# mourisl/T1K

Hardware: AMD Instinct MI355X
Metric: genotyped reads/sec (end-to-end genotyper stage, 2x150 bp HLA) (higher is better)
Workload: dtype u64

## Files before the change

### include/t1k_gpu.h

```cpp
#ifndef T1K_GPU_H
#define T1K_GPU_H

#include <stddef.h>
#include <stdint.h>

#ifdef __cplusplus
extern "C" {
#endif

typedef enum {
  T1K_OK = 0,
  T1K_ERR_ARG = -1,
  T1K_ERR_DEVICE = -2,
  T1K_ERR_CAPACITY = -3,
  T1K_ERR_IO = -4,
  T1K_ERR_STATE = -5,
  T1K_ERR_INTERNAL = -6,
  T1K_ERR_COMMITTED = -7
} t1k_status;

typedef struct t1k_ctx t1k_ctx;
typedef struct t1k_job t1k_job;
typedef struct t1k_rowset t1k_rowset;
typedef struct t1k_comm t1k_comm;

typedef struct {
  int32_t kmer_length;
  int32_t radius;
  int32_t hit_len_required;
  double ref_seq_similarity;
  int32_t relax_intron_align;
  int32_t max_assign_cnt;
  int32_t max_read_len;
  int32_t workgroups;
  int64_t group_cap;
  int64_t cand_cap;
  int64_t ovl_cap;
  int64_t row_cap;
  int32_t n_base_code;
  int32_t store_chunk_mb;
} t1k_params;

void t1k_params_default(t1k_params *p);

int t1k_ctx_create(int device, const t1k_params *params, t1k_ctx **out);
void t1k_ctx_destroy(t1k_ctx *ctx);
const char *t1k_last_error(const t1k_ctx *ctx);
int t1k_device_count(void);
int t1k_device_memory(int device, uint64_t *freeBytes, uint64_t *totalBytes);

int t1k_ref_upload(t1k_ctx *ctx, const char *seqs, const uint64_t *offsets, const uint8_t *exon, uint32_t nAlleles);

int t1k_reads_upload(t1k_ctx *ctx, const char *seqs, const uint64_t *offsets, const uint32_t *weights, uint32_t nReadEnds);
int t1k_reads_upload_begin(t1k_ctx *ctx, uint32_t nReadEnds, uint64_t textBytes, int maxReadLen);
int t1k_reads_upload_piece(t1k_ctx *ctx, int what, const void *src, uint64_t byteOffset, uint64_t bytes, int slot);
int t1k_reads_upload_wait(t1k_ctx *ctx, int slot);
int t1k_reads_upload_end(t1k_ctx *ctx);

int t1k_reads_dedupe(t1k_ctx *ctx, uint32_t *distinctOf, uint32_t *nDistinct);

typedef struct {
  int32_t seq_idx, read_start, read_end, seq_start, seq_end, strand;
  int32_t match_cnt, left_clip, right_clip, relaxed_match_cnt;
  double similarity;
} t1k_overlap;

int t1k_assign_batch(t1k_ctx *ctx);
int t1k_assign_range(t1k_ctx *ctx, uint64_t first, uint32_t count);
int t1k_overlaps_download(t1k_ctx *ctx, uint32_t *counts, t1k_overlap *ovl, uint64_t cap, uint64_t *total);

int t1k_overlaps_upload(t1k_ctx *ctx, const uint32_t *counts, const t1k_overlap *ovl);
void t1k_pair_limits(uint32_t out[4]);
uint32_t t1k_pair_direct_cap(void);

typedef struct {
  int32_t allele_idx, start, end;
  float weight, qual, adjust_weight;
} t1k_row_entry;

int t1k_pair_batch(t1k_ctx *ctx, const uint32_t *end1, const uint32_t *end2, const uint8_t *hasN, uint32_t nFragments);
int t1k_rows_download(t1k_ctx *ctx, uint32_t *rowCounts, uint8_t *fragAssigned, t1k_row_entry *rows, uint64_t cap, uint64_t *total);

typedef struct {
  int32_t allele, start, end;
  float weight, adjust_weight;
} t1k_group_entry;
int t1k_rowset_create(t1k_ctx *owner, uint64_t nFragments, const uint8_t *whitelist , t1k_rowset **out);
int t1k_rowset_trim(t1k_rowset *rs, uint64_t n_fragments);
void t1k_rowset_destroy(t1k_rowset *rs);
int t1k_rowset_set_raw(t1k_rowset *rs, int raw);
int t1k_rowset_device_bytes(t1k_rowset *rs, uint64_t *bytes, uint64_t *rowEntries);
const char *t1k_rowset_last_error(const t1k_rowset *rs);
int t1k_pair_into(t1k_ctx *ctx, t1k_rowset *rs, const uint32_t *end1, const uint32_t *end2, const uint8_t *hasN, uint32_t nFragments, uint64_t fragBase);
int t1k_rowset_coalesce(t1k_rowset *rs, uint64_t *nGroups, uint64_t *nEntries, uint64_t *assignedFragments);
int t1k_rowset_coalesce_sized(t1k_rowset *rs, uint64_t *nGroups, uint64_t *nEntries, uint64_t *assignedFragments, void (*sized)(uint64_t nGroups, uint64_t nEntries, void *user), void *user);
int t1k_rowset_groups_download(t1k_rowset *rs, uint64_t *groupPtr, t1k_group_entry *entries, uint32_t *firstFragment);
int t1k_rowset_assigned_download(t1k_rowset *rs, uint8_t *fragAssigned);
int t1k_rowset_assigned_range(t1k_rowset *rs, uint64_t first, uint64_t count, uint8_t *fragAssigned);
int t1k_rowset_rows_download(t1k_rowset *rs, uint64_t first, uint32_t count, uint32_t *rowCounts, t1k_row_entry *rows, uint64_t cap, uint64_t *total);
void t1k_coalesce_limits(uint32_t out[3]);

typedef struct t1k_comm_group t1k_comm_group;
int t1k_comm_unique_id(void *id128);
t1k_comm_group *t1k_comm_group_create(int nRanks);
void t1k_comm_group_destroy(t1k_comm_group *g);
int t1k_comm_init(t1k_ctx *ctx, int nRanks, int rank, const void *id128, t1k_comm_group *group, int transport , t1k_comm **out);
int t1k_comm_bind(t1k_comm *c, t1k_ctx *ctx);
int t1k_comm_abort(t1k_comm *c);
void t1k_comm_destroy(t1k_comm *c);
const char *t1k_comm_last_error(const t1k_comm *c);
int t1k_comm_rank(const t1k_comm *c);
int t1k_comm_size(const t1k_comm *c);
int t1k_comm_is_rccl(const t1k_comm *c);
int t1k_comm_allreduce(t1k_comm *c, void *dev, uint64_t count, int kind);
int t1k_comm_allgather_u64(t1k_comm *c, const uint64_t *mine, uint32_t k, uint64_t *all);
int t1k_comm_alltoallv(t1k_comm *c, const void *sendbuf, const uint64_t *sendOff, void *recvbuf, const uint64_t *recvOff);
int t1k_comm_allgatherv(t1k_comm *c, const void *mine, const uint64_t *bytes, const uint64_t *displ, void *out);
int t1k_comm_allgatherv_host(t1k_comm *c, void *host, const uint64_t *bytes, const uint64_t *displ, uint64_t total);
int t1k_rowset_exchange(t1k_rowset *rs, t1k_comm *comm, uint64_t fragBase);
int t1k_rowset_groups_gather(t1k_rowset *rs, t1k_comm *comm, uint64_t *totalGroups, uint64_t *totalEntries, uint64_t *totalAssigned);
int t1k_rowset_groups_download_all(t1k_rowset *rs, uint32_t *sizes, t1k_group_entry *entries, uint32_t *firstFragment);
int t1k_em_shard(t1k_ctx *ctx, uint32_t rowBegin, uint32_t rowEnd, t1k_comm *comm);

int t1k_coverage_get(t1k_ctx *ctx, int32_t *out, uint64_t cap);
int t1k_coverage_reset(t1k_ctx *ctx);
int t1k_missing_coverage(t1k_ctx *ctx, int32_t *missing);
typedef struct t1k_readset t1k_readset;
int t1k_ctx_set_coverage_mode(t1k_ctx *ctx, int deferred);
int t1k_readset_detach(t1k_ctx *reader, t1k_readset **out);
int t1k_readset_take_store(t1k_readset *rs, t1k_ctx *pipe, int slot);
uint64_t t1k_readset_bytes(const t1k_readset *rs);
uint32_t t1k_readset_size(const t1k_readset *rs);
const char *t1k_readset_last_error(const t1k_readset *rs);
void t1k_readset_destroy(t1k_readset *rs);
int t1k_coverage_selected(t1k_ctx *ctx, t1k_readset *rs, const uint8_t *selected, uint64_t *nRecords);
typedef struct t1k_xwin t1k_xwin;
int t1k_xwin_create(t1k_ctx *owner, uint64_t maxReadEnds, uint32_t maxWindows, t1k_xwin **out);
void t1k_xwin_destroy(t1k_xwin *x);
const char *t1k_xwin_last_error(const t1k_xwin *x);
int t1k_xwin_link(t1k_xwin *x, t1k_ctx *reader, uint32_t window, uint32_t *nExternal);
int t1k_xwin_resolve(t1k_xwin *x, t1k_ctx *ctx, uint32_t window);

int t1k_ref_share(t1k_ctx *dst, const t1k_ctx *src);
uint64_t t1k_pool_release(void);
void *t1k_pinned_alloc(uint64_t bytes);
void t1k_pinned_free(void *p);
int t1k_reads_share(t1k_ctx *dst, const t1k_ctx *src);
int t1k_reads_attach(t1k_ctx *dst, const t1k_ctx *src, int storeSlot, int resetStore);
int t1k_coverage_absorb(t1k_ctx *dst, t1k_ctx *src);

int t1k_extract_batch(t1k_ctx *ctx, uint32_t endsPerFragment, uint8_t *good, uint64_t *stats);

int t1k_align_count_batch(t1k_ctx *ctx, const char *text, const uint32_t *tOff, const char *pat, const uint32_t *pOff, const uint32_t *len, uint32_t nJobs,
                          int32_t *nMatch);
int t1k_gap_count_batch(t1k_ctx *ctx, const char *text, const uint32_t *tOff, const uint32_t *tLen, const char *pat, const uint32_t *pOff,
                        const uint32_t *pLen, uint32_t nJobs, int32_t *nMatch);
int t1k_align_batch(t1k_ctx *ctx, const char *text, const uint32_t *tOff, const uint32_t *tLen, const char *pat, const uint32_t *pOff,
                    const uint32_t *pLen, uint32_t nJobs, int32_t *score, int32_t *nMatch, int32_t *nMismatch, int32_t *nIndel, int8_t *ops,
                    const uint32_t *opsOff, uint32_t *nOps);

typedef void (*t1k_allreduce_fn)(void *dev_f64, uint64_t n, void *user);
int t1k_em_setup(t1k_ctx *ctx, const uint64_t *rowPtr, const uint32_t *ecIdx, const double *count, const int32_t *ecLen, uint32_t nGroups,
                 uint32_t nEc, t1k_allreduce_fn allreduce, void *user);
int t1k_em_update(t1k_ctx *ctx, const double *x0, double *x1, double *ecReadCount, double *diff);
void t1k_em_limits(uint32_t out[2]);

int t1k_barcode_em(t1k_ctx *ctx, uint32_t nBarcodes, const uint64_t *bcAllelePtr, const uint32_t *bcAllele, const uint64_t *bcGroupPtr,
                   const double *groupCount, const uint64_t *groupEntryPtr, const uint32_t *entryLocal, const double *rho, uint32_t nAlleles,
                   double alpha, double tol, int32_t maxIter, double *nOut, int32_t *itersOut, double *kernelMs);

typedef struct {
  uint64_t distinct;
  uint64_t keys;
  uint64_t corrected;
  uint64_t split;
  uint64_t no_umi;
  double kernel_ms;
} t1k_umi_stats;
int t1k_umi_collapse(t1k_ctx *ctx, uint32_t nFrag, const uint32_t *fragRow, const uint64_t *fragUmi, const uint64_t *listPtr, const uint32_t *listAllele,
                     uint32_t nRows, const uint32_t *alleleGene, uint32_t nAlleles, uint32_t nGenes, int32_t mismatch, uint32_t *fragMol, uint32_t *nMol,
                     uint32_t *molRow, uint32_t *molFrags, uint64_t *molListPtr, uint32_t *molList, double *frac, int32_t *uniq, t1k_umi_stats *stats);

typedef struct {
  uint32_t allele, seq_start;
  uint64_t read_at, ops_at;
  uint32_t n_ops, w_all, w_uniq, reserved;
} t1k_pileup_aln;
int t1k_pileup_begin(t1k_ctx *ctx, uint32_t nAlleles, const uint64_t *alleleOff );
int t1k_pileup_add(t1k_ctx *ctx, const t1k_pileup_aln *aln, uint32_t n, const char *text, uint64_t textBytes, const int8_t *ops, uint64_t opsBytes,
                   double *kernelMs);
int t1k_pileup_get(t1k_ctx *ctx, int32_t *counts );
int t1k_pileup_end(t1k_ctx *ctx);

int t1k_sitepile_begin(t1k_ctx *ctx, uint32_t nAlleles, const uint64_t *alleleOff , uint64_t nSites, const uint32_t *siteAllele, const uint32_t *sitePos,
                       uint64_t nBarcodes);
int t1k_sitepile_add(t1k_ctx *ctx, const t1k_pileup_aln *aln, uint32_t n, const uint64_t *bookPtr , const uint32_t *book, const char *text, uint64_t textBytes,
                     const int8_t *ops, uint64_t opsBytes, double *kernelMs);
int t1k_sitepile_get(t1k_ctx *ctx, uint64_t *keys, int32_t *counts, uint64_t cap, uint64_t *nRuns);
int t1k_sitepile_stats(t1k_ctx *ctx, uint64_t *keysEmitted, uint64_t *folds, double *foldMs);
int t1k_sitepile_end(t1k_ctx *ctx);

int t1k_phase_begin(t1k_ctx *ctx, uint32_t nAlleles, const uint64_t *alleleOff , uint64_t nSites, const uint32_t *siteAllele, const uint32_t *sitePos);
int t1k_phase_add(t1k_ctx *ctx, const t1k_pileup_aln *aln, uint32_t n, uint32_t nBook, const uint32_t *bookRec , const uint8_t *bookUniq ,
                  const char *text, uint64_t textBytes, const int8_t *ops, uint64_t opsBytes, double *kernelMs);
int t1k_phase_get(t1k_ctx *ctx, uint64_t *keys, int32_t *counts, uint64_t cap, uint64_t *nRuns);
int t1k_phase_stats(t1k_ctx *ctx, uint64_t *observations, uint64_t *bookings, uint64_t *keysEmitted, uint64_t *discordant, uint64_t *folds, double *foldMs);
int t1k_phase_end(t1k_ctx *ctx);

typedef struct { uint32_t read_len, clip_front, strand; } t1k_support_rec;
typedef struct { uint32_t flags, t_start, t_end; } t1k_support_book;
int t1k_support_begin(t1k_ctx *ctx, uint32_t nAlleles, const uint64_t *alleleOff , uint64_t nSites, const uint32_t *siteAllele, const uint32_t *sitePos);
int t1k_support_add(t1k_ctx *ctx, const t1k_pileup_aln *aln, uint32_t n, const t1k_support_rec *rec , const uint64_t *bookPtr ,
                    const t1k_support_book *book, const char *text, uint64_t textBytes, const int8_t *ops, uint64_t opsBytes, double *kernelMs);
int t1k_support_get(t1k_ctx *ctx, uint64_t *keys, int32_t *counts, uint64_t cap, uint64_t *nRuns);
int t1k_support_stats(t1k_ctx *ctx, uint64_t *keysEmitted, uint64_t *folds, double *foldMs);
int t1k_support_end(t1k_ctx *ctx);

int t1k_indel_begin(t1k_ctx *ctx, uint32_t nAlleles, const uint64_t *alleleOff , const char *alleleText );
int t1k_indel_add(t1k_ctx *ctx, const t1k_pileup_aln *aln, uint32_t n, const uint8_t *strand , const uint64_t *bookPtr , const uint8_t *bookUniq,
                  const char *text, uint64_t textBytes, const int8_t *ops, uint64_t opsBytes, double *kernelMs);
int t1k_indel_get(t1k_ctx *ctx, uint64_t *keys, int32_t *counts, uint64_t cap, uint64_t *nRuns);
int t1k_indel_stats(t1k_ctx *ctx, uint64_t *events, uint64_t *shifted, uint64_t *edgeDelBooked, uint64_t *edgeInsBooked, uint64_t *keysEmitted, uint64_t *folds, double *foldMs);
int t1k_indel_end(t1k_ctx *ctx);

int t1k_cigar_batch(t1k_ctx *ctx, const t1k_pileup_aln *aln, uint32_t n, const uint32_t *clip ,
                    const int8_t *ops, uint64_t opsBytes, uint32_t nAlleles, const uint64_t *alleleOff , const char *alleleText ,
                    uint64_t *cigarPtr , char *cigar, uint64_t cigarCap, uint64_t *mdPtr , char *md, uint64_t mdCap,
                    uint32_t *nm , uint32_t *refSpan , double *kernelMs );

typedef struct {
  uint64_t read_ends, lookups, postings, hits, groups, candidates, extended, near_best, dp_calls, rows, batches;
  double ms_seed, ms_chain, ms_extend, ms_select, ms_fullalign, ms_pair, ms_em, ms_total;
  uint64_t read_ends_total, pair_overlaps, dp_cells;
  double ms_load, ms_device, ms_coalesce, ms_write;
} t1k_stats;
int t1k_stats_get(t1k_ctx *ctx, t1k_stats *out);

enum { T1K_ROUTE_GENERAL_LANE = 0,
       T1K_ROUTE_WAVE_SMALL = 1,
       T1K_ROUTE_WAVE_LARGE = 2,
       T1K_ROUTE_BIG_BY_SIZE = 3,
       T1K_ROUTE_BIG_BY_SCRATCH = 4,
       T1K_ROUTE_KINDS = 5 };
typedef struct {
  uint64_t ranges, ranges_nw5, ranges_nw10, ranges_xlong;
  uint64_t groups, fast, slow, jobs, retry, finish, general, wave, genjobs, big, eq, band, wide, extjobs, extretry;
} t1k_route_totals;
typedef struct {
  uint32_t read_end, allele, n;
  uint8_t strand;
  uint8_t near_done, simple;
  uint8_t route;
  uint8_t nw, xlong, reserved[2];
} t1k_route_rec;
int t1k_route_report_enable(t1k_ctx *ctx, int on);
int t1k_route_report_get(t1k_ctx *ctx, t1k_route_totals *totals , t1k_route_rec *recs , uint64_t cap, uint64_t *nRecs);

double t1k_alloc_ms(t1k_ctx *ctx, uint64_t *bytes);
uint64_t t1k_ctx_mem_report(t1k_ctx *ctx, const char *tag, int print);

int t1k_genotyper_main(int argc, char **argv);
int t1k_extractor_main(int argc, char **argv);
int t1k_bam_extractor_main(int argc, char **argv);
int t1k_analyzer_main(int argc, char **argv);

typedef struct {
  t1k_params dev;
  double filter_frac, filter_cov, cross_gene_rate, squarem_min_alpha;
  int32_t allele_digit_units;
  char allele_delimiter;
  int32_t threads;
  int32_t device;
  int32_t output_read_assignment;
  int32_t batch_fragments;
} t1k_job_params;
void t1k_job_params_default(t1k_job_params *p);

int t1k_job_create(const t1k_job_params *p, const char *refFasta, t1k_job **out);
void t1k_job_destroy(t1k_job *job);
const char *t1k_job_last_error(const t1k_job *job);
int t1k_job_load_reads(t1k_job *job, const char *file1, const char *file2, const char *barcodeFile);
int t1k_job_load_reads_multi(t1k_job *job, const char *const *files1, uint32_t n1, const char *const *files2, uint32_t n2, const char *barcodeFile);
typedef struct t1k_reads t1k_reads;
int t1k_reads_open(const char *const *files1, uint32_t n1, const char *const *files2, uint32_t n2, const char *barcodeFile, int threads, t1k_reads **out);
int t1k_reads_open_stream(const char *const *files1, uint32_t n1, const char *const *files2, uint32_t n2, const char *barcodeFile, int threads, t1k_reads **out);
const char *t1k_reads_last_error(const t1k_reads *reads);
int t1k_reads_fragments(const t1k_reads *reads, uint64_t *nFragments);
void t1k_reads_close(t1k_reads *reads);
int t1k_job_attach_reads(t1k_job *job, t1k_reads *reads);
int t1k_job_set_reads(t1k_job *job, const char *seq1, const uint64_t *off1, const char *seq2, const uint64_t *off2, uint32_t nFragments);
int t1k_job_run(t1k_job *job);
int t1k_job_set_output_prefix(t1k_job *job, const char *prefix);
int t1k_job_write_outputs(t1k_job *job, const char *prefix);
int t1k_job_genotype_text(t1k_job *job, char *buf, uint64_t cap, uint64_t *needed);
int t1k_job_counts(t1k_job *job, uint64_t *fragments, uint64_t *assignedFragments, uint64_t *groups, uint64_t *ecs, int32_t *emIterations);
int t1k_job_stats(t1k_job *job, t1k_stats *out);
t1k_ctx *t1k_job_ctx(t1k_job *job);
int t1k_job_set_shard(t1k_job *job, int rank, int nRanks, t1k_comm *comm);
int t1k_job_share_reads(t1k_job *dst, t1k_job *src);
int t1k_job_run_local(t1k_job *job);
int t1k_job_finish(t1k_job *job);
int t1k_job_groups_serialize(t1k_job *job, void *buf, uint64_t cap, uint64_t *needed);
int t1k_job_groups_merge(t1k_job *job, const void *const *bufs, const uint64_t *lens, uint32_t n);
int t1k_job_coalesce_rows(t1k_job *job, const t1k_row_entry *rows, const uint32_t *rowCounts, const uint32_t *fragments, uint32_t nFragments);
int t1k_coverage_device(t1k_ctx *ctx, void **devPtr, uint64_t *count);

typedef struct {
  int32_t allele_idx;
  int32_t has_mate_pair, o1_from_r2;
  t1k_overlap o1, o2;
  uint64_t ops1, ops2;
  uint32_t n_ops1, n_ops2;
} t1k_frag_assignment;
int t1k_fragment_details(const t1k_overlap *l1, uint32_t n1, const t1k_overlap *l2, uint32_t n2, int paired, const int32_t *alleles, uint32_t nAlleles,
                         t1k_frag_assignment *out);
typedef struct {
  int32_t allele_idx, ref_pos, exon_pos;
// ... 19 lines not shown
```

### t1k_amd/capi.py

```python
import ctypes as C
import gzip
import os

import numpy as np

_HERE = os.path.dirname(os.path.abspath(__file__))


def lib_path():
    return os.environ.get("T1K_GPU_LIB") or os.path.join(_HERE, "lib", "libt1k_gpu.so")


class T1kError(RuntimeError):
    pass


class Params(C.Structure):
    _fields_ = [("kmer_length", C.c_int32), ("radius", C.c_int32), ("hit_len_required", C.c_int32),
                ("ref_seq_similarity", C.c_double), ("relax_intron_align", C.c_int32), ("max_assign_cnt", C.c_int32),
                ("max_read_len", C.c_int32), ("workgroups", C.c_int32), ("group_cap", C.c_int64),
                ("cand_cap", C.c_int64), ("ovl_cap", C.c_int64), ("row_cap", C.c_int64), ("n_base_code", C.c_int32), ("store_chunk_mb", C.c_int32)]


class JobParams(C.Structure):
    _fields_ = [("dev", Params), ("filter_frac", C.c_double), ("filter_cov", C.c_double),
                ("cross_gene_rate", C.c_double), ("squarem_min_alpha", C.c_double), ("allele_digit_units", C.c_int32),
                ("allele_delimiter", C.c_char), ("threads", C.c_int32), ("device", C.c_int32),
                ("output_read_assignment", C.c_int32), ("batch_fragments", C.c_int32)]


class Stats(C.Structure):
    _fields_ = [(n, C.c_uint64) for n in ("read_ends", "lookups", "postings", "hits", "groups", "candidates", "extended",
                                          "near_best", "dp_calls", "rows", "batches")] + \
               [(n, C.c_double) for n in ("ms_seed", "ms_chain", "ms_extend", "ms_select", "ms_fullalign", "ms_pair", "ms_em", "ms_total")] + \
               [(n, C.c_uint64) for n in ("read_ends_total", "pair_overlaps", "dp_cells")] + \
               [(n, C.c_double) for n in ("ms_load", "ms_device", "ms_coalesce", "ms_write")]

    def as_dict(self):
        return {n: getattr(self, n) for n, _ in self._fields_}


class UmiStats(C.Structure):
    _fields_ = [(n, C.c_uint64) for n in ("distinct", "keys", "corrected", "split", "no_umi")] + [("kernel_ms", C.c_double)]


OVERLAP_DTYPE = np.dtype([("seq_idx", "<i4"), ("read_start", "<i4"), ("read_end", "<i4"), ("seq_start", "<i4"),
                          ("seq_end", "<i4"), ("strand", "<i4"), ("match_cnt", "<i4"), ("left_clip", "<i4"),
                          ("right_clip", "<i4"), ("relaxed_match_cnt", "<i4"), ("similarity", "<f8")])
ROW_DTYPE = np.dtype([("allele_idx", "<i4"), ("start", "<i4"), ("end", "<i4"), ("weight", "<f4"), ("qual", "<f4"),
                      ("adjust_weight", "<f4")])
GROUP_DTYPE = np.dtype([("allele", "<i4"), ("start", "<i4"), ("end", "<i4"), ("weight", "<f4"), ("adjust_weight", "<f4")])
assert OVERLAP_DTYPE.itemsize == 48 and ROW_DTYPE.itemsize == 24 and GROUP_DTYPE.itemsize == 20
FRAG_ASG_DTYPE = np.dtype([("allele_idx", "<i4"), ("has_mate_pair", "<i4"), ("o1_from_r2", "<i4"), ("_pad", "<i4"), ("o1", OVERLAP_DTYPE), ("o2", OVERLAP_DTYPE),
                           ("ops1", "<u8"), ("ops2", "<u8"), ("n_ops1", "<u4"), ("n_ops2", "<u4")])
VARIANT_DTYPE = np.dtype([("allele_idx", "<i4"), ("ref_pos", "<i4"), ("exon_pos", "<i4"), ("ref", "S1"), ("var", "S1"), ("_pad", "S2"), ("qual", "<i4"), ("group", "<i4"),
                          ("output_group", "<i4"), ("_pad2", "<i4"), ("var_support", "<f8"), ("all_support", "<f8"), ("var_uniq_support", "<f8")])
assert FRAG_ASG_DTYPE.itemsize == 136 and VARIANT_DTYPE.itemsize == 56

PILEUP_ALN_DTYPE = np.dtype([("allele", "<u4"), ("seq_start", "<u4"), ("read_at", "<u8"), ("ops_at", "<u8"), ("n_ops", "<u4"), ("w_all", "<u4"), ("w_uniq", "<u4"),
                             ("reserved", "<u4")])
PHASE_NO_MATE = 0xFFFFFFFF
PHASE_STATES = ("A", "C", "G", "T", "N", "-")
PILEUP_COUNTERS = ("A", "C", "G", "T", "N", "del", "ins", "A_uniq", "C_uniq", "G_uniq", "T_uniq", "N_uniq", "del_uniq", "ins_uniq")
assert PILEUP_ALN_DTYPE.itemsize == 40
SUPPORT_REC_DTYPE = np.dtype([("read_len", "<u4"), ("clip_front", "<u4"), ("strand", "<u4")])
SUPPORT_BOOK_DTYPE = np.dtype([("flags", "<u4"), ("t_start", "<u4"), ("t_end", "<u4")])
SUPPORT_STATES = ("A", "C", "G", "T", "N", "-", "+")
SUPPORT_FAMILY_B = 1 << 57
assert SUPPORT_REC_DTYPE.itemsize == 12 and SUPPORT_BOOK_DTYPE.itemsize == 12
ROUTE_TOTALS = ("ranges", "ranges_nw5", "ranges_nw10", "ranges_xlong", "groups", "fast", "slow", "jobs", "retry", "finish", "general", "wave", "genjobs", "big",
                "eq", "band", "wide", "extjobs", "extretry")
ROUTE_REC_DTYPE = np.dtype([("read_end", "<u4"), ("allele", "<u4"), ("n", "<u4"), ("strand", "u1"), ("near_done", "u1"), ("simple", "u1"), ("route", "u1"),
                            ("nw", "u1"), ("xlong", "u1"), ("reserved", "u1", (2,))])
ROUTE_NAMES = ("general_lane", "wave_small", "wave_large", "big_by_size", "big_by_scratch")
assert ROUTE_REC_DTYPE.itemsize == 20
CIGAR_FILL = 0xAB

ALLREDUCE_FN = C.CFUNCTYPE(None, C.c_void_p, C.c_uint64, C.c_void_p)

_lib = None


def lib():
    global _lib
    if _lib is not None:
        return _lib
    p = lib_path()
    if not os.path.exists(p):
        raise T1kError("%s not found: run `python -c 'import __graft_entry__ as g; g.build()'` first" % p)
    L = C.CDLL(p)
    vp, u64p, u32p, u8p, i32p = C.c_void_p, C.POINTER(C.c_uint64), C.POINTER(C.c_uint32), C.POINTER(C.c_uint8), C.POINTER(C.c_int32)
    L.t1k_params_default.argtypes = [C.POINTER(Params)]
    L.t1k_ctx_create.argtypes = [C.c_int, C.POINTER(Params), C.POINTER(vp)]
    L.t1k_ctx_destroy.argtypes = [vp]
    L.t1k_last_error.argtypes = [vp]
    L.t1k_last_error.restype = C.c_char_p
    L.t1k_device_count.restype = C.c_int
    L.t1k_ref_upload.argtypes = [vp, C.c_char_p, vp, vp, C.c_uint32]
    L.t1k_reads_upload.argtypes = [vp, C.c_char_p, vp, vp, C.c_uint32]
    L.t1k_assign_batch.argtypes = [vp]
    L.t1k_assign_range.argtypes = [vp, C.c_uint64, C.c_uint32]
    L.t1k_overlaps_download.argtypes = [vp, vp, vp, C.c_uint64, u64p]
    L.t1k_pair_batch.argtypes = [vp, vp, vp, vp, C.c_uint32]
    L.t1k_rows_download.argtypes = [vp, vp, vp, vp, C.c_uint64, u64p]
    L.t1k_coverage_get.argtypes = [vp, vp, C.c_uint64]
    L.t1k_coverage_reset.argtypes = [vp]
    L.t1k_missing_coverage.argtypes = [vp, vp]
    L.t1k_coverage_absorb.argtypes = [vp, vp]
    L.t1k_align_batch.argtypes = [vp, C.c_char_p, vp, vp, C.c_char_p, vp, vp, C.c_uint32, vp, vp, vp, vp, vp, vp, vp]
    L.t1k_align_count_batch.argtypes = [vp, C.c_char_p, vp, C.c_char_p, vp, vp, C.c_uint32, vp]
    L.t1k_gap_count_batch.argtypes = [vp, C.c_char_p, vp, vp, C.c_char_p, vp, vp, C.c_uint32, vp]
    L.t1k_em_setup.argtypes = [vp, vp, vp, vp, vp, C.c_uint32, C.c_uint32, ALLREDUCE_FN, vp]
    L.t1k_em_update.argtypes = [vp, vp, vp, vp, vp]
    L.t1k_em_shard.argtypes = [vp, C.c_uint32, C.c_uint32, vp]
    L.t1k_em_limits.argtypes = [vp]
    L.t1k_em_limits.restype = None
    L.t1k_barcode_em.argtypes = [vp, C.c_uint32, vp, vp, vp, vp, vp, vp, vp, C.c_uint32, C.c_double, C.c_double, C.c_int32, vp, vp, C.POINTER(C.c_double)]
    L.t1k_umi_collapse.argtypes = [vp, C.c_uint32, vp, vp, vp, vp, C.c_uint32, vp, C.c_uint32, C.c_uint32, C.c_int32, vp, C.POINTER(C.c_uint32), vp, vp, vp, vp, vp, vp,
                                   C.POINTER(UmiStats)]
# ... 4 lines not shown
    L.t1k_sitepile_begin.argtypes = [vp, C.c_uint32, vp, C.c_uint64, vp, vp, C.c_uint64]
    L.t1k_sitepile_add.argtypes = [vp, vp, C.c_uint32, vp, vp, vp, C.c_uint64, vp, C.c_uint64, C.POINTER(C.c_double)]
    L.t1k_sitepile_get.argtypes = [vp, vp, vp, C.c_uint64, u64p]
    L.t1k_sitepile_stats.argtypes = [vp, u64p, u64p, C.POINTER(C.c_double)]
    L.t1k_sitepile_end.argtypes = [vp]
    L.t1k_support_begin.argtypes = [vp, C.c_uint32, vp, C.c_uint64, vp, vp]
    L.t1k_support_add.argtypes = [vp, vp, C.c_uint32, vp, vp, vp, vp, C.c_uint64, vp, C.c_uint64, C.POINTER(C.c_double)]
    L.t1k_support_get.argtypes = [vp, vp, vp, C.c_uint64, u64p]
    L.t1k_support_stats.argtypes = [vp, u64p, u64p, C.POINTER(C.c_double)]
    L.t1k_support_end.argtypes = [vp]
    L.t1k_indel_begin.argtypes = [vp, C.c_uint32, vp, vp]
    L.t1k_indel_add.argtypes = [vp, vp, C.c_uint32, vp, vp, vp, vp, C.c_uint64, vp, C.c_uint64, C.POINTER(C.c_double)]
    L.t1k_indel_get.argtypes = [vp, vp, vp, C.c_uint64, u64p]
    L.t1k_indel_stats.argtypes = [vp, u64p, u64p, u64p, u64p, u64p, u64p, C.POINTER(C.c_double)]
    L.t1k_indel_end.argtypes = [vp]
    L.t1k_phase_begin.argtypes = [vp, C.c_uint32, vp, C.c_uint64, vp, vp]
    L.t1k_phase_add.argtypes = [vp, vp, C.c_uint32, C.c_uint32, vp, vp, vp, C.c_uint64, vp, C.c_uint64, C.POINTER(C.c_double)]
    L.t1k_phase_get.argtypes = [vp, vp, vp, C.c_uint64, u64p]
    L.t1k_phase_stats.argtypes = [vp, u64p, u64p, u64p, u64p, u64p, C.POINTER(C.c_double)]
    L.t1k_phase_end.argtypes = [vp]
    L.t1k_cigar_batch.argtypes = [vp, vp, C.c_uint32, vp, vp, C.c_uint64, C.c_uint32, vp, vp, vp, vp, C.c_uint64, vp, vp, C.c_uint64, vp, vp, C.POINTER(C.c_double)]
    L.t1k_extract_batch.argtypes = [vp, C.c_uint32, vp, vp]
    L.t1k_extractor_main.argtypes = [C.c_int, C.POINTER(C.c_char_p)]
    L.t1k_stats_get.argtypes = [vp, C.POINTER(Stats)]
    L.t1k_route_report_enable.argtypes = [vp, C.c_int]
    L.t1k_route_report_get.argtypes = [vp, vp, vp, C.c_uint64, u64p]
    L.t1k_genotyper_main.argtypes = [C.c_int, C.POINTER(C.c_char_p)]
    L.t1k_job_params_default.argtypes = [C.POINTER(JobParams)]
    L.t1k_job_create.argtypes = [C.POINTER(JobParams), C.c_char_p, C.POINTER(vp)]
    L.t1k_job_destroy.argtypes = [vp]
    L.t1k_job_last_error.argtypes = [vp]
    L.t1k_job_last_error.restype = C.c_char_p
    L.t1k_job_load_reads.argtypes = [vp, C.c_char_p, C.c_char_p, C.c_char_p]
    L.t1k_job_set_reads.argtypes = [vp, C.c_char_p, vp, C.c_char_p, vp, C.c_uint32]
    L.t1k_job_run.argtypes = [vp]
    L.t1k_job_write_outputs.argtypes = [vp, C.c_char_p]
    L.t1k_pool_release.restype = C.c_uint64
    L.t1k_pool_release.argtypes = []
    L.t1k_job_load_reads_multi.argtypes = [vp, C.POINTER(C.c_char_p), C.c_uint32, C.POINTER(C.c_char_p), C.c_uint32, C.c_char_p]
    L.t1k_reads_open.argtypes = [C.POINTER(C.c_char_p), C.c_uint32, C.POINTER(C.c_char_p), C.c_uint32, C.c_char_p, C.c_int, C.POINTER(vp)]
    L.t1k_reads_open_stream.argtypes = [C.POINTER(C.c_char_p), C.c_uint32, C.POINTER(C.c_char_p), C.c_uint32, C.c_char_p, C.c_int, C.POINTER(vp)]
    L.t1k_reads_last_error.argtypes = [vp]
    L.t1k_reads_last_error.restype = C.c_char_p
    L.t1k_reads_fragments.argtypes = [vp, u64p]
    L.t1k_reads_close.argtypes = [vp]
    L.t1k_reads_close.restype = None
    L.t1k_job_attach_reads.argtypes = [vp, vp]
    L.t1k_job_genotype_text.argtypes = [vp, C.c_char_p, C.c_uint64, u64p]
    L.t1k_job_counts.argtypes = [vp, u64p, u64p, u64p, u64p, i32p]
    L.t1k_job_stats.argtypes = [vp, C.POINTER(Stats)]
    L.t1k_job_ctx.argtypes = [vp]
    L.t1k_job_ctx.restype = vp
    L.t1k_job_run_local.argtypes = [vp]
    L.t1k_job_finish.argtypes = [vp]
    L.t1k_job_groups_serialize.argtypes = [vp, vp, C.c_uint64, u64p]
    L.t1k_reads_dedupe.argtypes = [vp, vp, u32p]
    L.t1k_job_groups_merge.argtypes = [vp, vp, vp, C.c_uint32]
    L.t1k_job_coalesce_rows.argtypes = [vp, vp, vp, vp, C.c_uint32]
    L.t1k_variants_call.argtypes = [vp, vp, C.c_int32, C.c_uint32, vp, vp, vp, vp, vp, vp, vp, C.POINTER(vp)]
    L.t1k_fragment_details.argtypes = [vp, C.c_uint32, vp, C.c_uint32, C.c_int, vp, C.c_uint32, vp]
    L.t1k_variants_count.argtypes = [vp]
    L.t1k_variants_count.restype = C.c_uint32
    L.t1k_variants_get.argtypes = [vp, vp]
    L.t1k_variants_vcf.argtypes = [vp, vp, C.c_uint64, u64p]
    L.t1k_variants_adjust.argtypes = [vp, vp, C.c_uint32, vp, C.c_char_p, C.c_uint32, C.c_char_p, C.c_uint32, vp]
    L.t1k_variants_destroy.argtypes = [vp]
    L.t1k_job_set_shard.argtypes = [vp, C.c_int, C.c_int, vp]
    L.t1k_job_share_reads.argtypes = [vp, vp]
    L.t1k_job_ctx.restype = vp
    L.t1k_job_ctx.argtypes = [vp]
    L.t1k_comm_unique_id.argtypes = [vp]
    L.t1k_comm_init.argtypes = [vp, C.c_int, C.c_int, vp, vp, C.c_int, C.POINTER(vp)]
    L.t1k_comm_bind.argtypes = [vp, vp]
    L.t1k_comm_destroy.argtypes = [vp]
    L.t1k_comm_last_error.restype = C.c_char_p
    L.t1k_comm_last_error.argtypes = [vp]
    L.t1k_comm_is_rccl.argtypes = [vp]
    L.t1k_comm_group_create.restype = vp
    L.t1k_comm_group_create.argtypes = [C.c_int]
    L.t1k_comm_group_destroy.argtypes = [vp]
    L.t1k_coverage_device.argtypes = [vp, C.POINTER(vp), u64p]
    L.t1k_device_memory.argtypes = [C.c_int, u64p, u64p]
    L.t1k_ctx_set_coverage_mode.argtypes = [vp, C.c_int]
    L.t1k_readset_detach.argtypes = [vp, C.POINTER(vp)]
    L.t1k_readset_take_store.argtypes = [vp, vp, C.c_int]
    L.t1k_readset_bytes.argtypes = [vp]
    L.t1k_readset_bytes.restype = C.c_uint64
    L.t1k_readset_size.argtypes = [vp]
    L.t1k_readset_size.restype = C.c_uint32
    L.t1k_readset_destroy.argtypes = [vp]
    L.t1k_coverage_selected.argtypes = [vp, vp, vp, u64p]
    L.t1k_overlaps_upload.argtypes = [vp, vp, vp]
    L.t1k_pair_limits.argtypes = [vp]
    L.t1k_pair_limits.restype = None
    L.t1k_pair_direct_cap.argtypes = []
    L.t1k_pair_direct_cap.restype = C.c_uint32
    L.t1k_rowset_create.argtypes = [vp, C.c_uint64, vp, C.POINTER(vp)]
    L.t1k_rowset_destroy.argtypes = [vp]
    L.t1k_rowset_destroy.restype = None
    L.t1k_rowset_set_raw.argtypes = [vp, C.c_int]
    L.t1k_rowset_last_error.argtypes = [vp]
    L.t1k_rowset_last_error.restype = C.c_char_p
    L.t1k_pair_into.argtypes = [vp, vp, vp, vp, vp, C.c_uint32, C.c_uint64]
    L.t1k_rowset_rows_download.argtypes = [vp, C.c_uint64, C.c_uint32, vp, vp, C.c_uint64, u64p]
    L.t1k_rowset_assigned_range.argtypes = [vp, C.c_uint64, C.c_uint64, vp]
    L.t1k_rowset_coalesce.argtypes = [vp, u64p, u64p, u64p]
    L.t1k_rowset_groups_download.argtypes = [vp, vp, vp, vp]
    L.t1k_rowset_device_bytes.argtypes = [vp, u64p, u64p]
    L.t1k_coalesce_limits.argtypes = [vp]
    L.t1k_coalesce_limits.restype = None
    L.t1k_rowset_exchange.argtypes = [vp, vp, C.c_uint64]
    L.t1k_rowset_groups_gather.argtypes = [vp, vp, u64p, u64p, u64p]
    L.t1k_rowset_groups_download_all.argtypes = [vp, vp, vp, vp]
    L.t1k_comm_abort.argtypes = [vp]
    L.t1k_ref_share.argtypes = [vp, vp]
    _lib = L
    return L


def _ptr(a):
    return a.ctypes.data_as(C.c_void_p) if a is not None else None


def _concat(seqs):
    offs = np.zeros(len(seqs) + 1, dtype=np.uint64)
    if len(seqs):
        offs[1:] = np.cumsum([len(s) for s in seqs], dtype=np.uint64)
    blob = "".join(seqs).encode("ascii")
    return blob, offs


class Context:

    def __init__(self, device=0, **kw):
        L = lib()
        p = Params()
        L.t1k_params_default(C.byref(p))
        for k, v in kw.items():
            setattr(p, k, v)
        self.params = p
        h = C.c_void_p()
        rc = L.t1k_ctx_create(device, C.byref(p), C.byref(h))
        if rc != 0:
            raise T1kError("t1k_ctx_create failed (%d): no usable GPU / bad parameters" % rc)
        self.h = h
        self.n_read_ends = 0
        self.allele_len = None

    def _check(self, rc, what):
        if rc != 0:
            raise T1kError("%s failed (%d): %s" % (what, rc, lib().t1k_last_error(self.h).decode()))

    def close(self):
        if self.h:
            lib().t1k_ctx_destroy(self.h)
            self.h = None

    def __del__(self):
        try:
            self.close()
        except Exception:
            pass

    def ref_upload(self, seqs, exon_masks=None):
        blob, offs = _concat(seqs)
        ex = None
        if exon_masks is not None:
            ex = np.concatenate([np.asarray(m, dtype=np.uint8) for m in exon_masks]) if len(seqs) else np.zeros(0, np.uint8)
        self.allele_len = np.array([len(s) for s in seqs], dtype=np.int64)
        self._check(lib().t1k_ref_upload(self.h, blob, _ptr(offs), _ptr(ex), len(seqs)), "t1k_ref_upload")

    def ref_share(self, src):
        self.allele_len = src.allele_len
        self._check(lib().t1k_ref_share(self.h, src.h), "t1k_ref_share")

    def reads_upload(self, seqs, weights=None):
        blob, offs = _concat(seqs)
        w = None if weights is None else np.asarray(weights, dtype=np.uint32)
        self.n_read_ends = len(seqs)
        self._check(lib().t1k_reads_upload(self.h, blob, _ptr(offs), _ptr(w), len(seqs)), "t1k_reads_upload")

    def reads_dedupe(self):
        out = np.zeros(self.n_read_ends, dtype=np.uint32)
        nd = C.c_uint32()
        self._check(lib().t1k_reads_dedupe(self.h, _ptr(out), C.byref(nd)), "t1k_reads_dedupe")
        self.n_uploaded, self.n_read_ends = self.n_read_ends, nd.value
        return out

    def assign(self):
        self._check(lib().t1k_assign_batch(self.h), "t1k_assign_batch")

    def extract(self, ends_per_fragment=1):
        good = np.zeros(self.n_read_ends // ends_per_fragment, dtype=np.uint8)
        st = np.zeros(8, dtype=np.uint64)
        self._check(lib().t1k_extract_batch(self.h, ends_per_fragment, _ptr(good), _ptr(st)), "t1k_extract_batch")
        return good, dict(zip(("read_ends", "lookups", "postings", "read_ends_with_hits", "read_ends_chained", "screen_ns", "main_ns", "big_shape"), (int(x) for x in st)))

    def overlaps(self):
        n = self.n_read_ends
        counts = np.zeros(n, dtype=np.uint32)
        tot = C.c_uint64()
        self._check(lib().t1k_overlaps_download(self.h, _ptr(counts), None, 0, C.byref(tot)), "t1k_overlaps_download")
        out = np.zeros(tot.value, dtype=OVERLAP_DTYPE)
        self._check(lib().t1k_overlaps_download(self.h, _ptr(counts), _ptr(out), tot.value, C.byref(tot)), "t1k_overlaps_download")
        return counts, out

    def overlaps_upload(self, counts, ovl):
        c = np.ascontiguousarray(counts, dtype=np.uint32)
        o = np.ascontiguousarray(ovl, dtype=OVERLAP_DTYPE)
        assert len(c) == self.n_read_ends and int(c.sum()) == len(o)
        self._check(lib().t1k_overlaps_upload(self.h, _ptr(c), _ptr(o)), "t1k_overlaps_upload")

    def pair(self, end1, end2, has_n):
        e1 = np.asarray(end1, dtype=np.uint32)
        e2 = None if end2 is None else np.asarray(end2, dtype=np.uint32)
        hn = np.asarray(has_n, dtype=np.uint8)
        self.n_fragments = len(e1)
        self._check(lib().t1k_pair_batch(self.h, _ptr(e1), _ptr(e2), _ptr(hn), len(e1)), "t1k_pair_batch")

    def rows(self):
        n = self.n_fragments
        counts = np.zeros(n, dtype=np.uint32)
        assigned = np.zeros(n, dtype=np.uint8)
        tot = C.c_uint64()
        self._check(lib().t1k_rows_download(self.h, _ptr(counts), _ptr(assigned), None, 0, C.byref(tot)), "t1k_rows_download")
        out = np.zeros(tot.value, dtype=ROW_DTYPE)
        self._check(lib().t1k_rows_download(self.h, _ptr(counts), _ptr(assigned), _ptr(out), tot.value, C.byref(tot)), "t1k_rows_download")
        return counts, assigned, out

    def coverage(self):
        tot = int(self.allele_len.sum())
        out = np.zeros(tot, dtype=np.int32)
        self._check(lib().t1k_coverage_get(self.h, _ptr(out), tot), "t1k_coverage_get")
        return out

    def set_coverage_mode(self, deferred):
        self._check(lib().t1k_ctx_set_coverage_mode(self.h, 1 if deferred else 0), "t1k_ctx_set_coverage_mode")

    def detach_readset(self, slot=0):
        h = C.c_void_p()
        self._check(lib().t1k_readset_detach(self.h, C.byref(h)), "t1k_readset_detach")
        rs = Readset(h)
        self._check(lib().t1k_readset_take_store(rs.h, self.h, slot), "t1k_readset_take_store")
        return rs

    def coverage_selected(self, readset, selected):
        sel = np.ascontiguousarray(selected, dtype=np.uint8)
        n = C.c_uint64()
        self._check(lib().t1k_coverage_selected(self.h, readset.h, _ptr(sel), C.byref(n)), "t1k_coverage_selected")
        return n.value

    def coverage_reset(self):
        self._check(lib().t1k_coverage_reset(self.h), "t1k_coverage_reset")

    def missing_coverage(self):
        out = np.zeros(len(self.allele_len), dtype=np.int32)
        self._check(lib().t1k_missing_coverage(self.h, _ptr(out)), "t1k_missing_coverage")
        return out

    def stats(self):
        s = Stats()
        lib().t1k_stats_get(self.h, C.byref(s))
        return s.as_dict()

    def route_report_enable(self, on=True):
        self._check(lib().t1k_route_report_enable(self.h, 1 if on else 0), "t1k_route_report_enable")

    def route_report(self):
        n = C.c_uint64()
        self._check(lib().t1k_route_report_get(self.h, None, None, 0, C.byref(n)), "t1k_route_report_get")
        tot = np.zeros(len(ROUTE_TOTALS), np.uint64)
        recs = np.zeros(n.value, ROUTE_REC_DTYPE)
        self._check(lib().t1k_route_report_get(self.h, _ptr(tot), _ptr(recs), n.value, C.byref(n)), "t1k_route_report_get")
        return dict(zip(ROUTE_TOTALS, (int(x) for x in tot))), recs

    def align_batch(self, texts, pats, want_ops=True):
        n = len(texts)
        tb, toff = _concat(texts)
        pb, poff = _concat(pats)
        tlen = np.array([len(t) for t in texts], dtype=np.uint32)
        plen = np.array([len(p) for p in pats], dtype=np.uint32)
        toff32, poff32 = toff[:-1].astype(np.uint32), poff[:-1].astype(np.uint32)
        score = np.zeros(n, np.int32); nm = np.zeros(n, np.int32); nx = np.zeros(n, np.int32); ni = np.zeros(n, np.int32)
        ops_off = np.zeros(n, np.uint32)
        if n:
            ops_off[1:] = np.cumsum((tlen + plen + 2)[:-1], dtype=np.uint64).astype(np.uint32)
        ops = np.zeros(int((tlen + plen + 2).sum()) + 8, np.int8)
        nops = np.zeros(n, np.uint32)
        self._check(lib().t1k_align_batch(self.h, tb, _ptr(toff32), _ptr(tlen), pb, _ptr(poff32), _ptr(plen), n, _ptr(score), _ptr(nm),
                                          _ptr(nx), _ptr(ni), _ptr(ops) if want_ops else None, _ptr(ops_off), _ptr(nops)), "t1k_align_batch")
        op_list = [ops[ops_off[i]:ops_off[i] + nops[i]].copy() for i in range(n)] if want_ops else None
        return score, nm, nx, ni, op_list

    def align_count_batch(self, texts, pats):
        n = len(texts)
        tb, toff = _concat(texts)
        pb, poff = _concat(pats)
        ln = np.array([len(t) for t in texts], dtype=np.uint32)
        out = np.zeros(n, np.int32)
        self._check(lib().t1k_align_count_batch(self.h, tb, _ptr(toff[:-1].astype(np.uint32)), pb, _ptr(poff[:-1].astype(np.uint32)), _ptr(ln), n,
                                                _ptr(out)), "t1k_align_count_batch")
        return out

    def gap_count_batch(self, texts, pats, lead=""):
        n = len(texts)
        tb, toff = _concat([lead] + list(texts))
        pb, poff = _concat(pats)
        tlen = np.array([len(t) for t in texts], dtype=np.uint32)
        plen = np.array([len(p) for p in pats], dtype=np.uint32)
        out = np.zeros(n, np.int32)
        self._check(lib().t1k_gap_count_batch(self.h, tb, _ptr(toff[1:-1].astype(np.uint32)), _ptr(tlen), pb, _ptr(poff[:-1].astype(np.uint32)), _ptr(plen), n,
                                              _ptr(out)), "t1k_gap_count_batch")
        return out

    def em_setup(self, row_ptr, ec_idx, count, ec_len, allreduce=None, raw=False):
        self._em_keep = (np.ascontiguousarray(row_ptr, np.uint64), np.ascontiguousarray(ec_idx, np.uint32), np.ascontiguousarray(count, np.float64),
                         np.ascontiguousarray(ec_len, np.int32))
        rp, ei, ct, el = self._em_keep
        assert len(rp) == len(ct) + 1 and int(rp[-1]) == len(ei)
        self._em_cb = ALLREDUCE_FN(allreduce) if allreduce else C.cast(None, ALLREDUCE_FN)
        self._em_nec = len(el)
# ... 860 lines not shown
```

### t1k_amd/csrc/host/job.cpp

```cpp
#include "job_internal.h"

extern "C" {


void t1k_job_params_default(t1k_job_params *p) {
  memset(p, 0, sizeof(*p));
  t1k_params_default(&p->dev);
  p->filter_frac = 0.15;
  p->filter_cov = 1.0;
  p->cross_gene_rate = 0.04;
  p->squarem_min_alpha = 0;
  p->allele_digit_units = -1;
  p->allele_delimiter = 0;
  p->threads = 1;
  p->device = 0;
  p->output_read_assignment = 0;
  p->batch_fragments = 0;
}

int t1k_job_create(const t1k_job_params *p, const char *refFasta, t1k_job **out) { return jobCreate(p, refFasta, nullptr, out); }

}
namespace t1k {
int jobCreate(const t1k_job_params *p, const char *refFasta, const std::set<std::string> *selected, t1k_job **out) {
// ... 411 lines not shown
  const bool traceTasks = getenv("T1K_DEBUG_TASKS") != nullptr;
  auto prepare = [&] {
    struct Raw {
      void *p = nullptr; size_t cap = 0; bool pinned = false;
      ~Raw() { drop(); }
      void drop() { if (pinned) t1k_pinned_free(p); else free(p); p = nullptr; cap = 0; }
      void *need(size_t bytes) {
        if (bytes <= cap) return p;
        drop();
        static const bool noPin = getenv("T1K_NO_PINNED_TEXT") != nullptr;
        p = noPin ? nullptr : t1k_pinned_alloc(bytes);
        pinned = p != nullptr;
        if (!p) p = malloc(bytes);
        cap = p ? bytes : 0;
        return p;
      }
    } offs[2], stage;
    auto windowSize = [&](uint32_t w) -> uint64_t {
      uint64_t size = firstWindow;
      if (w > 0) {
        const Window &prev = win[w - 1];
        const double tp = prev.msPrep / std::max<double>(1, prev.f1 - prev.f0);
        double tg = 0;
        for (uint32_t v = w; v-- > 0;)
          if (win[v].done && win[v].tDone > win[v].tReady) { tg = (win[v].tDone - win[v].tReady) / std::max<double>(1, win[v].f1 - win[v].f0); break; }
        uint64_t waiting = 0;
        for (uint32_t v = sh.oldest; v < w; ++v) waiting += win[v].f1 - win[v].f0;
        double factor = fixedGrowth > 0 ? fixedGrowth : (tg > 0 && tp > 0 ? 0.85 * tg / tp : 6.0);
        factor = std::min(16.0, std::max(1.0, factor));
        size = (uint64_t)(factor * (double)std::max<uint64_t>(waiting, firstWindow / 2));
        size = std::min<uint64_t>(windowFrags, std::max<uint64_t>(size, firstWindow));
      }
      return size;
    };
    uint64_t fNext = 0;
    uint64_t have = F;
    bool ended = !gzStream;
    for (uint32_t w = 0; gzStream ? true : fNext < F; ++w) {
      if (gzStream) {
        const uint64_t least = fNext + (w == 0 ? firstWindow : std::max<uint32_t>(16384u, firstWindow / 4));
        for (;;) {
          const int st = in.streamState();
          have = in.streamAvail();
          if (st < 0) { std::string e; (void)job->in->streamFinish(e); fail(T1K_ERR_IO, e.empty() ? "cannot read the .gz input" : e); return; }
          if (st == 1) { have = in.streamAvail(); ended = true; break; }
          bool idle;
          uint64_t want;
          { std::lock_guard<std::mutex> g(sh.m); if (sh.err != T1K_OK) return; idle = sh.oldest >= sh.created; want = fNext + windowSize(w); }
          if (w + 8 >= maxWindows) { std::this_thread::sleep_for(std::chrono::milliseconds(1)); continue; }
          if (have >= want || (have >= least && idle)) break;
          std::this_thread::sleep_for(std::chrono::microseconds(300));
        }
        if (ended && fNext >= have) {
          std::lock_guard<std::mutex> g(sh.m);
          sh.allCreated = true;
          sh.cv.notify_all();
          break;
        }
      }
      {
        std::unique_lock<std::mutex> lk(sh.m);
        sh.cv.wait(lk, [&] { return sh.err != T1K_OK || w < 2 || win[w - 2].done; });
        if (sh.err != T1K_OK) return;
        if (gzStream && !ended) { const int st = in.streamState(); have = in.streamAvail(); if (st == 1) { have = in.streamAvail(); ended = true; } }
        const uint64_t size = windowSize(w);
        Window N;
        N.f0 = (uint32_t)fNext; N.f1 = (uint32_t)std::min<uint64_t>(have, fNext + size);
        if (ended && (have - N.f1 < size / 4 || w + 1 >= maxWindows)) N.f1 = (uint32_t)have;
        N.slot = (int)(w & 1);
        N.touched.assign(P, 0);
        if (!eagerFromNowOn) {
          const double perFrag = archivedFrags ? 1.25 * (double)archivedNeed / (double)archivedFrags : 0.0;
          const uint64_t slack = (uint64_t)P * (uint64_t)std::max(1, job->prm.dev.store_chunk_mb) << 20;
          auto estimate = [&](const Window &X) { return archivedFrags ? (uint64_t)(perFrag * (double)(X.f1 - X.f0)) + slack : 0ull; };
          uint64_t open = 0;
          for (uint32_t v = sh.oldest; v < w; ++v)
            if (win[v].deferred && !win[v].done) open += estimate(win[v]);
          bool fits = archivedBytes + open + estimate(N) <= archiveBudget;
          static const char *testHeadroom = getenv("T1K_TEST_ARCHIVE_HEADROOM_MB");
          if (fits && sh.pairedFrags >= (testHeadroom ? 1u : 65536u) && !getenv("T1K_ARCHIVE_GB")) {
            uint64_t freeNow = 0, totalNow = 0, rowsNow = 0, entriesNow = 0;
            if (t1k_device_memory(job->prm.device, &freeNow, &totalNow) == T1K_OK && t1k_rowset_device_bytes(job->rows, &rowsNow, &entriesNow) == T1K_OK && totalNow) {
              if (testHeadroom) { const uint64_t used = totalNow - std::min(freeNow, totalNow); totalNow = used + ((uint64_t)atoll(testHeadroom) << 20); freeNow = totalNow - used; }
              const double projectedRows = (double)entriesNow / (double)sh.pairedFrags * (double)F * sizeof(t1k_row_entry) * 1.1 + 32.0 * (double)F + std::min(4e9, 0.015 * (double)totalNow);
              const uint64_t usedNow = totalNow - std::min(freeNow, totalNow);
              const uint64_t other = usedNow > archivedBytes + rowsNow ? usedNow - archivedBytes - rowsNow : 0;
              const double coalesceWork = 48.0 * (double)F + std::min(8e9, 0.03 * (double)totalNow);
              const double transient = perFrag * (double)std::min<uint64_t>(windowFrags, F - N.f1);
              static const double reserve = [] { const char *e = getenv("T1K_ARCHIVE_RESERVE_GB"); return e ? atof(e) * 1073741824.0 : -1.0; }();
              const double keepFree = reserve >= 0 ? reserve : std::max(8e9, 0.04 * (double)totalNow);
              fits = (double)other + (double)(archivedBytes + open + estimate(N)) + std::max(projectedRows, (double)rowsNow) + coalesceWork + transient + keepFree <= (double)totalNow;
              if (getenv("T1K_DEBUG_ARCHIVE"))
                fprintf(stderr, "[t1k job] window %u (%u fragments): %llu row entries in the chunks, %llu fragments paired, stats.rows %llu, rows %.1f GB, kept %.1f + open %.1f + this %.1f GB, other %.1f GB, transient %.1f GB -> %s\n",
                        w, N.f1 - N.f0, (unsigned long long)entriesNow, (unsigned long long)sh.pairedFrags, (unsigned long long)job->stats.rows, rowsNow / 1e9, archivedBytes / 1e9, open / 1e9,
                        estimate(N) / 1e9, other / 1e9, transient / 1e9, fits ? "kept" : "not kept");
              if (!fits && getenv("T1K_DEBUG_PHASES"))
                fprintf(stderr, "[t1k job] window %u: read sets are not kept from here on: %.1f GB of rows projected for the job (%.1f GB so far), %.1f GB kept, %.1f GB other, device %.1f GB\n",
                        w, projectedRows / 1e9, rowsNow / 1e9, archivedBytes / 1e9, other / 1e9, totalNow / 1e9);
            }
          }
          if (fits) N.deferred = true;
          else eagerFromNowOn = true;
        }
        fNext = N.f1;
        win.push_back(std::move(N));
        sh.created = w + 1;
        if (ended && fNext >= have) sh.allCreated = true;
      }
      Window &W = win[w];
      const double t0 = nowMs();
      const uint32_t nf = W.f1 - W.f0, ne = nf * per;
      uint64_t *off = (uint64_t *)offs[W.slot].need(((size_t)ne + 1) * 8);
      if (!off) { fail(T1K_ERR_DEVICE, "window preparation: out of host memory"); return; }
      W.hasN.resize(nf);
      std::vector<uint64_t> pieceBytes(T + 2, 0);
      std::vector<uint32_t> pieceMax(T + 1, 0);
      auto setAside = [&](uint32_t r) {
        if (!dropLong) return false;
        for (uint32_t m = 0; m < per; ++m) if (in.side[m].seqL[r] > lenLimit) return true;
        return false;
      };
      parallelRanges(nf, T, [&](int t, size_t b, size_t e) {
        uint64_t run = 0, aside = 0;
        uint32_t mx = 0;
        for (size_t i = b; i < e; ++i) {
          const uint32_t r = in.frag[fBeg - inBase + W.f0 + i];
          const bool skip = setAside(r);
          aside += skip ? 1 : 0;
          for (uint32_t m = 0; m < per; ++m) {
            const uint32_t len = skip ? 0 : in.side[m].seqL[r];
            off[i * per + m] = run; run += len; mx = std::max(mx, len);
          }
        }
        pieceBytes[t + 1] = run; pieceMax[t] = mx;
        if (aside) droppedFragments += aside;
      });
      for (int t = 0; t < T; ++t) pieceBytes[t + 1] += pieceBytes[t];
      const uint64_t total = pieceBytes[T];
      uint32_t maxLen = 0;
      for (int t = 0; t < T; ++t) maxLen = std::max(maxLen, pieceMax[t]);
      if (gzStream && maxLen > lenLimit) {
        fail(T1K_ERR_ARG, "a read of " + std::to_string(maxLen) + " bases is longer than this build handles (" + std::to_string(job->prm.dev.max_read_len) +
                              "); T1K_LONG_READS=drop sets the fragments of such reads aside instead of stopping");
        return;
      }
      parallelRanges(nf, T, [&](int t, size_t b, size_t e) {
        const uint64_t carry = pieceBytes[t];
        for (size_t i = b; i < e; ++i)
          for (uint32_t m = 0; m < per; ++m) off[i * per + m] += carry;
      });
      off[ne] = total;
      static const size_t slotBytes = [] { const char *e = getenv("T1K_STAGE_MB"); return (size_t)std::max(1, e ? atoi(e) : 96) << 20; }();
      const int nSlots = 3;
      char *ring = (char *)stage.need(nSlots * slotBytes);
      if (!ring) { fail(T1K_ERR_DEVICE, "window preparation: out of host memory"); return; }
      t1k_ctx *rd = job->reader[W.slot];
      int r = t1k_reads_upload_begin(rd, ne, total, (int)maxLen);
      if (r == T1K_OK) r = t1k_reads_upload_piece(rd, 1, off, 0, ((uint64_t)ne + 1) * 8, 3);
      double msGather = 0;
      uint32_t nPieces = 0;
      for (size_t i0 = 0; i0 < nf && r == T1K_OK; ++nPieces) {
        const uint64_t base = off[i0 * per];
        size_t lo = i0 + 1, hi = nf;
        while (lo < hi) {
          const size_t mid = lo + (hi - lo + 1) / 2;
          if (off[mid * per] - base <= slotBytes) lo = mid; else hi = mid - 1;
        }
// ... 48 lines not shown
          }
        });
        for (uint32_t q = 1; q < W.nPair; ++q) W.pairNeed[q] = std::max(W.pairNeed[q], W.pairNeed[q - 1]);
        for (uint32_t q = 0; q < W.nPair; ++q) W.pairNeed[q] = std::min(W.pairNeed[q], W.nAssign);
      }
      if (traceTasks) fprintf(stderr, "[t1k task] prep window %u: %.1f .. %.1f ms (text %.1f ms, upload %.1f, resize %.1f, dedupe %.1f, pairing needs %.1f)\n", w, t0 - tStart, nowMs() - tStart, tText - t0, tUp - tText, tRes - tUp, tDd - tRes, nowMs() - tDd);
      {
        std::lock_guard<std::mutex> g(sh.m);
        job->distinctReadEnds += W.nDistinct - W.nExternal;
        job->stats.read_ends -= W.nExternal;
        msPrep += nowMs() - t0;
        W.msPrep = nowMs() - t0; W.tReady = nowMs();
        W.ready = true;
      }
      sh.cv.notify_all();
    }
  };
  std::function<int(t1k_ctx *, Window &, uint32_t, uint32_t, std::string &)> assignRange = [&](t1k_ctx *ctx, Window &Wn, uint32_t b0, uint32_t nb, std::string &msg) -> int {
    int r = t1k_assign_range(ctx, b0, nb);
    if (r == T1K_ERR_CAPACITY && nb > 64) {
      if ((r = assignRange(ctx, Wn, b0, nb / 2, msg)) != T1K_OK) return r;
      return assignRange(ctx, Wn, b0 + nb / 2, nb - nb / 2, msg);
    }
    if (r != T1K_OK) { msg = t1k_last_error(ctx); return r; }
    t1k_stats st;
    t1k_stats_get(ctx, &st);
    if (traceTasks) fprintf(stderr, "[t1k task]   range of %u read-ends at %u: kernels by HIP events: seed %.1f chain %.1f extend %.1f select %.1f align+truncate %.1f ms\n", nb, b0, st.ms_seed, st.ms_chain, st.ms_extend, st.ms_select, st.ms_fullalign);
    std::lock_guard<std::mutex> g(sh.m);
    Wn.ovlRecords += st.extended;
    job->stats.read_ends += st.read_ends; job->stats.lookups += st.lookups; job->stats.postings += st.postings; job->stats.hits += st.hits;
    job->stats.groups += st.groups; job->stats.candidates += st.candidates; job->stats.extended += st.extended; job->stats.near_best += st.near_best;
    job->stats.dp_calls += st.dp_calls; job->stats.ms_chain += st.ms_chain; job->stats.ms_extend += st.ms_extend; job->stats.ms_select += st.ms_select;
    job->stats.ms_fullalign += st.ms_fullalign; job->stats.ms_seed += st.ms_seed; job->stats.batches += 1; job->stats.dp_cells += st.dp_cells;
    return T1K_OK;
  };
  auto worker = [&](int pi) {
    t1k_ctx *ctx = pipes[pi];
    int attached = -1;
    std::vector<uint32_t> e1, e2;
    for (;;) {
      uint32_t w = 0, item = 0;
      int kind = -1;
      {
        std::unique_lock<std::mutex> lk(sh.m);
        for (;;) {
          if (sh.err != T1K_OK) return;
          if (sh.allCreated && sh.oldest >= sh.created) return;
          for (w = sh.oldest; w < sh.created && w < sh.oldest + 2 && win[w].ready && kind < 0; ++w) {
            Window &W = win[w];
            if (W.nextPair < W.nPair && W.assignPrefix >= W.pairNeed[W.nextPair]) {
              if (W.linked) { kind = 1; item = W.nextPair++; }
              else if (!W.linking) {
                bool srcDone = true;
                for (uint32_t v = sh.oldest; v < w; ++v) srcDone = srcDone && win[v].ready && win[v].doneAssign == win[v].nAssign;
                if (srcDone) { kind = 2; W.linking = true; }
              }
            }
            if (kind < 0 && W.nextAssign < W.nAssign) { kind = 0; item = W.nextAssign++; }
            if (kind >= 0) break;
          }
          if (kind >= 0) break;
          sh.cv.wait(lk);
        }
      }
      Window &W = win[w];
      int r = T1K_OK;
      std::string msg;
      const double tTask = nowMs();
      if (kind == 2) {
        r = t1k_xwin_resolve(xw.x, ctx, w);
        if (r != T1K_OK) { fail(r, t1k_xwin_last_error(xw.x)); return; }
        if (traceTasks) fprintf(stderr, "[t1k task] pipe %d window %u: %u read-ends linked to earlier windows: %.1f .. %.1f ms\n", pi, w, W.nExternal, tTask - tStart, nowMs() - tStart);
        { std::lock_guard<std::mutex> g(sh.m); W.linked = true; }
        sh.cv.notify_all();
        continue;
      }
      if (attached != (int)w) {
        r = t1k_reads_attach(ctx, job->reader[W.slot], W.slot, W.touched[pi] ? 0 : 1);
        if (r != T1K_OK) msg = t1k_last_error(ctx);
        W.touched[pi] = 1;
        attached = (int)w;
      }
      if (r == T1K_OK) (void)t1k_ctx_set_coverage_mode(ctx, (W.deferred || job->analyzer) ? 1 : 0);
      if (r == T1K_OK && kind == 0) {
        const uint32_t b0 = item * W.assignBatch, nb = std::min(W.assignBatch, W.nDistinct - b0);
        r = assignRange(ctx, W, b0, nb, msg);
      } else if (r == T1K_OK) {
        const uint32_t q0 = item * W.pairBatch, nq = std::min(W.pairBatch, (W.f1 - W.f0) - q0);
        e1.resize(nq); e2.resize(nq);
        for (uint32_t i = 0; i < nq; ++i) { e1[i] = W.distinctOf[(size_t)(q0 + i) * per]; if (per == 2) e2[i] = W.distinctOf[(size_t)(q0 + i) * per + 1]; }
        r = t1k_pair_into(ctx, job->rows, e1.data(), per == 2 ? e2.data() : nullptr, W.hasN.data() + q0, nq, (uint64_t)W.f0 + q0);
        if (r != T1K_OK) msg = t1k_last_error(ctx);
        else {
          t1k_stats st;
          t1k_stats_get(ctx, &st);
          std::lock_guard<std::mutex> g(sh.m);
          job->stats.ms_pair += st.ms_pair; job->stats.pair_overlaps += st.pair_overlaps; job->stats.rows += st.rows;
          sh.pairedFrags += nq;
        }
      }
      if (r != T1K_OK) { fail(r, msg); return; }
      if (traceTasks) fprintf(stderr, "[t1k task] pipe %d window %u %s %u: %.1f .. %.1f ms\n", pi, w, kind == 0 ? "assign" : "pair", item, tTask - tStart, nowMs() - tStart);
      {
        std::lock_guard<std::mutex> g(sh.m);
        if (kind == 0) {
          ++W.doneAssign; W.assignDone[item] = 1;
          while (W.assignPrefix < W.nAssign && W.assignDone[W.assignPrefix]) ++W.assignPrefix;
        } else { ++W.donePair; W.pairDone[item] = 1; }
        if (W.doneAssign == W.nAssign && W.donePair == W.nPair) {
          if (W.deferred) {
            t1k_readset *rs = nullptr;
            if (t1k_readset_detach(job->reader[W.slot], &rs) == T1K_OK) {
              for (int q = 0; q < P; ++q)
                if (W.touched[q]) (void)t1k_readset_take_store(rs, pipes[q], W.slot);
              archivedBytes += t1k_readset_bytes(rs); archivedFrags += W.f1 - W.f0;
              archivedNeed += W.ovlRecords * 16 + (uint64_t)W.nDistinct * 220;
              job->archive.push_back(rs);
            } else if (sh.err == T1K_OK) { sh.err = T1K_ERR_INTERNAL; sh.errMsg = std::string("keeping the window's read set: ") + t1k_last_error(job->reader[W.slot]); }
          }
          W.done = true; W.tDone = nowMs();
          if (traceTasks) fprintf(stderr, "[t1k task] window %u done: fragments %u .. %u, %u distinct read-ends (%u of them assigned by earlier windows), %u + %u ranges, ready at %.1f ms, done at %.1f ms%s\n", w, W.f0, W.f1,
                                  W.nDistinct, W.nExternal, W.nAssign, W.nPair, W.tReady - tStart, W.tDone - tStart, W.deferred ? ", read set kept" : "");
          std::vector<uint32_t>().swap(W.distinctOf);
          while (sh.oldest < sh.created && win[sh.oldest].done) ++sh.oldest;
        }
      }
      sh.cv.notify_all();
    }
  };
  job->streamDone = 0;
  const bool streaming = !job->outPrefix.empty() && job->nRanks == 1 && !in.sharded && !job->analyzer && F > 0 && !getenv("T1K_NO_STREAM_OUTPUT");
  bool loopEnded = false;
  auto follow = [&] {
    if (!streamOpen(job, job->outPrefix)) { fail(T1K_ERR_IO, job->err); return; }
    for (uint32_t w = 0;; ++w) {
      {
        std::unique_lock<std::mutex> lk(sh.m);
        sh.cv.wait(lk, [&] { return sh.err != T1K_OK || loopEnded || w < sh.created || sh.allCreated; });
        if (sh.err != T1K_OK || w >= sh.created) return;
      }
      Window &W = win[w];
      uint32_t next = 0;
      for (;;) {
        uint32_t upto = next;
        {
          std::unique_lock<std::mutex> lk(sh.m);
          sh.cv.wait(lk, [&] { return sh.err != T1K_OK || loopEnded || (W.ready && (next >= W.nPair || W.pairDone[next])); });
          if (sh.err != T1K_OK) return;
          if (!W.ready) return;
          while (upto < W.nPair && W.pairDone[upto]) ++upto;
          if (upto == next && next < W.nPair) return;
        }
        if (upto == next) break;
        const uint32_t fLo = W.f0 + next * W.pairBatch, fHi = (uint32_t)std::min<uint64_t>(W.f1, (uint64_t)W.f0 + (uint64_t)upto * W.pairBatch);
        int r = t1k_rowset_assigned_range(job->rows, fLo, fHi - fLo, job->fragAssigned.data() + fBeg + fLo);
        if (r != T1K_OK) { fail(r, t1k_rowset_last_error(job->rows)); return; }
        if (!streamAppend(job, fLo, fHi, true)) { fail(T1K_ERR_IO, job->err); return; }
        job->streamDone = fHi;
        if (!job->prm.output_read_assignment && fHi > fLo) job->in->release(in.frag[fLo], (size_t)in.frag[fHi - 1] + 1);
        next = upto;
      }
    }
  };
  {
    std::thread prep(prepare);
    std::thread writer;
    if (streaming) writer = std::thread(follow);
    std::vector<std::thread> others;
    for (int i = 1; i < P; ++i) others.emplace_back(worker, i);
    worker(0);
    for (auto &t : others) t.join();
    { std::lock_guard<std::mutex> g(sh.m); if (sh.err == T1K_OK && (!sh.allCreated || sh.oldest < sh.created) && F > 0) { sh.err = T1K_ERR_INTERNAL; sh.errMsg = "window loop ended early"; } loopEnded = true; }
    sh.cv.notify_all();
    prep.join();
    if (writer.joinable()) writer.join();
  }
  if (sh.err != T1K_OK) { streamClose(job, true); return jobFail(job, sh.err, sh.errMsg); }
  if (gzStream) {
    if (!job->in->streamFinish(job->err)) { streamClose(job, true); return jobFail(job, T1K_ERR_IO, job->err); }
    F = (uint32_t)in.nFrag();
// ... 64 lines not shown
      if (!job->assignText.empty()) memcpy(&all[displ[job->rank]], job->assignText.data(), job->assignText.size());
      if ((rc = t1k_comm_allgatherv_host(job->comm, total ? &all[0] : nullptr, sizes.data(), displ.data(), total)) != T1K_OK) return jobFail(job, rc, t1k_comm_last_error(job->comm));
      job->assignText.swap(all);
    }
  }
  uint64_t G = 0, N = 0, assigned = 0;
  static_assert(sizeof(GroupEntry) == sizeof(t1k_group_entry), "group entry layouts differ");
  const double tEx0 = nowMs();
  if (getenv("T1K_DEBUG_ARCHIVE")) {
    uint64_t b = 0, e = 0;
    if (t1k_rowset_device_bytes(job->rows, &b, &e) == T1K_OK)
      fprintf(stderr, "[t1k job] after the loop: %llu row entries in the chunks (%.1f GB allocated for rows), %llu fragments paired, stats.rows %llu\n",
              (unsigned long long)e, b / 1e9, (unsigned long long)sh.pairedFrags, (unsigned long long)job->stats.rows);
  }
  if (sharded && (rc = t1k_rowset_exchange(job->rows, job->comm, fBeg)) != T1K_OK) return jobFail(job, rc, t1k_rowset_last_error(job->rows));
  const double tEx1 = nowMs();
  struct Sizer { Genotyper *gt; int T; bool on; } sizer{&gt, T, !sharded};
  auto sizeTables = [](uint64_t g, uint64_t n, void *u) {
    Sizer &z = *(Sizer *)u;
    if (!z.on) return;
    z.gt->groupPtr.assign(g + 1, 0);
    z.gt->groupEnt.resize(n);
    z.gt->groupFirst.resize(g);
    parallelRanges(n * sizeof(GroupEntry) / 4096 + 1, z.T, [&](int, size_t b, size_t e) {
      volatile char *base = (volatile char *)z.gt->groupEnt.data();
      const size_t bytes = n * sizeof(GroupEntry);
      for (size_t pg = b; pg < e; ++pg) if (pg * 4096 < bytes) base[pg * 4096] = 0;
    });
  };
  if ((rc = t1k_rowset_coalesce_sized(job->rows, &G, &N, &assigned, sizeTables, &sizer)) != T1K_OK) return jobFail(job, rc, t1k_rowset_last_error(job->rows));
  const double tCo = nowMs();
  if (!sharded) {
    if (gt.groupPtr.size() != G + 1) { gt.groupPtr.assign(G + 1, 0); gt.groupEnt.resize(N); gt.groupFirst.resize(G); }
    const double tRes = nowMs();
    if ((rc = t1k_rowset_groups_download(job->rows, gt.groupPtr.data(), (t1k_group_entry *)gt.groupEnt.data(), gt.groupFirst.data())) != T1K_OK)
      return jobFail(job, rc, t1k_rowset_last_error(job->rows));
    const double tDl = nowMs();
    if ((rc = t1k_rowset_assigned_download(job->rows, job->fragAssigned.data())) != T1K_OK) return jobFail(job, rc, t1k_rowset_last_error(job->rows));
    if (getenv("T1K_DEBUG_PHASES"))
      fprintf(stderr, "[t1k job] after the loop: coverage of the pipelines + coalescing on the device %.1f ms, host tables sized %.1f ms, groups downloaded %.1f ms, flags %.1f ms\n",
              tCo - tDev, tRes - tCo, tDl - tRes, nowMs() - tDl);
  } else {
    const uint64_t Gl = G, Nl = N;
    if ((rc = t1k_rowset_groups_gather(job->rows, job->comm, &G, &N, &assigned)) != T1K_OK) return jobFail(job, rc, t1k_rowset_last_error(job->rows));
    std::vector<uint32_t> sizes(G), first(G);
    GroupVec ents;
    ents.resize(N);
    parallelRanges(N * sizeof(GroupEntry) / 4096 + 1, T, [&](int, size_t b, size_t e) {
      volatile char *base = (volatile char *)ents.data();
      const size_t bytes = N * sizeof(GroupEntry);
      for (size_t pg = b; pg < e; ++pg) if (pg * 4096 < bytes) base[pg * 4096] = 0;
    });
    if ((rc = t1k_rowset_groups_download_all(job->rows, sizes.data(), (t1k_group_entry *)ents.data(), first.data())) != T1K_OK)
      return jobFail(job, rc, t1k_rowset_last_error(job->rows));
    const double tGa = nowMs();
    gt.setGroupsMerged(sizes, ents, first);
    if (getenv("T1K_DEBUG_PHASES"))
      fprintf(stderr, "[t1k job] rank %d of %d after the loop (waits for the slowest rank included): rows to their pattern owners %.1f ms, coalescing of the owned patterns %.1f ms "
                      "(%llu groups, %llu entries on this rank), group tables gathered + downloaded %.1f ms (%llu groups, %llu entries in all), merged by first fragment %.1f ms\n",
              job->rank, job->nRanks, tEx1 - tEx0, tCo - tEx1, (unsigned long long)Gl, (unsigned long long)Nl, tGa - tCo,
              (unsigned long long)G, (unsigned long long)N, nowMs() - tGa);
    if ((rc = t1k_rowset_assigned_download(job->rows, job->fragAssigned.data() + fBeg)) != T1K_OK) return jobFail(job, rc, t1k_rowset_last_error(job->rows));
    if (!in.sharded) {
      std::vector<uint64_t> bytes(job->nRanks), displ(job->nRanks);
      for (int r = 0; r < job->nRanks; ++r) { displ[r] = (uint64_t)Fall * r / job->nRanks; bytes[r] = (uint64_t)Fall * (r + 1) / job->nRanks - displ[r]; }
      if ((rc = t1k_comm_allgatherv_host(job->comm, job->fragAssigned.data(), bytes.data(), displ.data(), Fall)) != T1K_OK) return jobFail(job, rc, t1k_comm_last_error(job->comm));
    }
  }
  gt.assignedFragments = assigned;
  job->stats.read_ends_total = job->readEnds;
  t1k_rowset_destroy(job->rows);
  job->rows = nullptr;
  job->msDevice = tDev - tStart; job->msCoalesce = nowMs() - tDev; job->msHost = 0;
  job->stats.ms_load = job->msLoad; job->stats.ms_device = job->msDevice; job->stats.ms_coalesce = job->msCoalesce;
  if (getenv("T1K_DEBUG_PHASES")) {
    double ms = 0; uint64_t by = 0, b1 = 0;
    for (t1k_ctx *c : pipes) { ms += t1k_alloc_ms(c, &b1); by += b1; }
    for (t1k_ctx *c : job->reader) { ms += t1k_alloc_ms(c, &b1); by += b1; }
    fprintf(stderr, "[t1k job] device memory: %.1f GB allocated by the contexts in %.1f ms of hipMalloc (summed over threads)\n", by / 1073741824.0, ms);
  }
  if (getenv("T1K_DEBUG_PHASES"))
    fprintf(stderr, "[t1k job] %u windows, %llu read-ends -> %llu distinct; window preparation %.1f ms (overlapped), device loop %.1f ms, coalesce + download %.1f ms (%llu groups, %llu entries)\n",
            sh.created, (unsigned long long)job->readEnds, (unsigned long long)job->distinctReadEnds, msPrep, job->msDevice, job->msCoalesce, (unsigned long long)G, (unsigned long long)N);
  if (getenv("T1K_DEBUG_PHASES") && job->covDeferred)
    fprintf(stderr, "[t1k job] coverage deferred to selection: read sets of %zu of %u windows kept (%.2f GB of device memory)\n", job->archive.size(), sh.created, archivedBytes / 1073741824.0);
  job->localDone = true;
  return T1K_OK;
}

int t1k_job_run_local(t1k_job *job) {
  int rc = runLocalOnce(job);
  if (rc != T1K_OK && job && job->in && job->in->streamGaveUp.load() && job->nRanks == 1) {
    fprintf(stderr, "[t1k] %s -- the read files are opened whole and the job starts over\n", job->err.c_str());
    std::unique_ptr<ReadInput> whole(new ReadInput());
    const std::vector<std::string> f1 = job->in->streamFiles1, f2 = job->in->streamFiles2;
    const std::string bc = job->in->streamBarcodeFile;
    const bool drop = job->in->dropInflatedText;
    job->in.reset();
    const double t0 = nowMs();
    std::string err;
    if (!whole->open(f1, f2, bc, hostThreads(job), err)) return jobFail(job, T1K_ERR_IO, err);
    whole->dropInflatedText = drop;
    job->in = std::move(whole);
    job->ran = false; job->localDone = false;
    job->msLoad = nowMs() - t0;
    rc = runLocalOnce(job);
  }
  return rc;
}


}
```

### t1k_amd/csrc/t1k_capi.hip

```cpp
#include <sys/mman.h>
#include <map>
#include <mutex>
#include <unordered_map>
#include <algorithm>
#include <memory>
#include <thread>
#include <chrono>
#include <cstring>
#include <cstdio>
#include <cstdlib>
#include "t1k_dev.h"
#include "t1k_launch.h"

namespace {
struct DevPool {
  std::mutex m;
  std::map<int, std::multimap<size_t, void *>> freeBlocks;
  std::unordered_map<void *, std::pair<size_t, int>> live;
  size_t pooled = 0;
};
DevPool &devPool() { static DevPool *p = new DevPool(); return *p; }
}

hipError_t t1k_dev_malloc(void **out, size_t bytes) {
// ... 180 lines not shown
  if (g >= nOvl) return;
  T1kOvlP p;
  if (!t1k_ovl_pack(work[g], p)) atomicOr(&counters[2], 1024ull);
  store[g] = p;
}
static void t1k_launch_publish_lists(t1k_ctx *ctx, unsigned long long *listPtr, uint32_t *listCount, const T1kOvl *work, T1kOvlP *store, uint64_t nOvl,
                                     const uint32_t *ovlStart, const uint32_t *ovlCount, uint32_t n, unsigned long long *counters, const uint8_t *skip) {
  if (nOvl) hipLaunchKernelGGL(k_pack_overlaps, dim3((unsigned)((nOvl + 255) / 256)), dim3(256), 0, ctx->stream, work, store, nOvl, counters);
  if (n) hipLaunchKernelGGL(k_publish_lists, dim3((n + 255) / 256), dim3(256), 0, ctx->stream, listPtr, listCount, store, ovlStart, ovlCount, n, skip);
}


extern "C" {

void t1k_params_default(t1k_params *p) {
  memset(p, 0, sizeof(*p));
  p->kmer_length = 11;
  p->radius = 10;
  p->hit_len_required = 31;
  p->ref_seq_similarity = 0.8;
  p->relax_intron_align = 0;
  p->max_assign_cnt = 2000;
  p->max_read_len = T1K_LONG_READ_LEN;
  p->workgroups = 2048;
  p->n_base_code = 3;
  p->store_chunk_mb = 1536;
  p->group_cap = 160ll << 20;
  p->cand_cap = 128ll << 20;
  p->ovl_cap = 96ll << 20;
  p->row_cap = 48ll << 20;
}

int t1k_device_count(void) {
  int n = 0;
  if (hipGetDeviceCount(&n) != hipSuccess) return 0;
  return n;
}

int t1k_ctx_create(int device, const t1k_params *params, t1k_ctx **out) {
  if (!out) return T1K_ERR_ARG;
  *out = nullptr;
  int n = 0;
  if (hipGetDeviceCount(&n) != hipSuccess || n <= 0 || device < 0 || device >= n) return T1K_ERR_DEVICE;
  if (hipSetDevice(device) != hipSuccess) return T1K_ERR_DEVICE;
  t1k_ctx *ctx = new t1k_ctx();
  ctx->device = device;
  if (params) ctx->prm = *params; else t1k_params_default(&ctx->prm);
  t1k_params d;
  t1k_params_default(&d);
  if (ctx->prm.kmer_length <= 0) ctx->prm.kmer_length = d.kmer_length;
  if (ctx->prm.radius <= 0) ctx->prm.radius = d.radius;
  if (ctx->prm.hit_len_required <= 0) ctx->prm.hit_len_required = d.hit_len_required;
  if (ctx->prm.max_assign_cnt == 0) ctx->prm.max_assign_cnt = d.max_assign_cnt;
  if (ctx->prm.max_read_len <= 0) ctx->prm.max_read_len = d.max_read_len;
  if (ctx->prm.workgroups <= 0) ctx->prm.workgroups = d.workgroups;
  if (ctx->prm.group_cap <= 0) ctx->prm.group_cap = d.group_cap;

  if (ctx->prm.cand_cap <= 0) ctx->prm.cand_cap = d.cand_cap;
  if (ctx->prm.ovl_cap <= 0) ctx->prm.ovl_cap = d.ovl_cap;
  if (ctx->prm.row_cap <= 0) ctx->prm.row_cap = d.row_cap;
  if (ctx->prm.store_chunk_mb <= 0) ctx->prm.store_chunk_mb = d.store_chunk_mb;
  if (ctx->prm.kmer_length > 15 || ctx->prm.max_read_len > T1K_LONG_READ_LEN) { delete ctx; return T1K_ERR_ARG; }
  if (hipStreamCreate(&ctx->stream) != hipSuccess) { delete ctx; return T1K_ERR_DEVICE; }
  for (auto &e : ctx->ev) if (hipEventCreate(&e) != hipSuccess) { delete ctx; return T1K_ERR_DEVICE; }
  *out = ctx;
  return T1K_OK;
}

static void freeBuf(T1kDevBuf &b) {
  if (b.p) (void)t1k_dev_free(b.p);
  b.p = nullptr; b.bytes = 0;
}

void t1k_ctx_destroy(t1k_ctx *ctx) {
  if (ctx && ctx->emPinned) { (void)hipHostFree(ctx->emPinned); ctx->emPinned = nullptr; }
  if (ctx && ctx->countersPinned) { (void)hipHostFree(ctx->countersPinned); ctx->countersPinned = nullptr; }
  if (!ctx) return;
  (void)hipSetDevice(ctx->device);
  if (ctx->stream) (void)hipStreamSynchronize(ctx->stream);
  for (auto &b : ctx->refBufs) freeBuf(b);
  T1kDevBuf *all[] = {&ctx->bReadAscii, &ctx->bReadOffs, &ctx->bReadBases, &ctx->bReadN, &ctx->bReadLen, &ctx->bReadWeight, &ctx->bWgHits, &ctx->bWgGroups,
                      &ctx->bWgStage, &ctx->bWgBig, &ctx->bWgCache, &ctx->bLists, &ctx->bCand, &ctx->bExt, &ctx->bCandStart, &ctx->bCandCount, &ctx->bListPtr, &ctx->bListCount,
                      &ctx->bOvlWork, &ctx->bOvlUpload, &ctx->bDedupScratch, &ctx->bDedupBases, &ctx->bDedupN, &ctx->bDedupLen, &ctx->bDedupWeight, &ctx->bOvlStart, &ctx->bOvlCount, &ctx->bCounters, &ctx->bSlowQueue, &ctx->bSlowScratch, &ctx->bSortScratch, &ctx->bSelClass, &ctx->bEqTrace, &ctx->bSortTmp, &ctx->bJobSort, &ctx->bEnd1, &ctx->bEnd2,
                      &ctx->bHasN, &ctx->bRows, &ctx->bRowStart, &ctx->bRowCount, &ctx->bFragAssigned, &ctx->bPairScratch, &ctx->bPairOverflow, &ctx->bPairBig, &ctx->bExtractHuge, &ctx->bEmRowPtr, &ctx->bEmEc,
                      &ctx->bEmCount, &ctx->bEmLen, &ctx->bEmX0, &ctx->bEmN, &ctx->bEmPsum, &ctx->bEmColPtr, &ctx->bEmRowOf, &ctx->bExtract, &ctx->bPileup, &ctx->bPileupIn, &ctx->spMap.buf, &ctx->spTab.keys, &ctx->spTab.vals, &ctx->spTab.work, &ctx->bSpIn,
                      &ctx->phMap.buf, &ctx->phTab.keys, &ctx->phTab.vals, &ctx->phTab.work, &ctx->bPhIn, &ctx->bPhObs, &ctx->bPhArena,
                      &ctx->supMap.buf, &ctx->supTab.keys, &ctx->supTab.vals, &ctx->supTab.work, &ctx->bSupIn,
                      &ctx->indTab.keys, &ctx->indTab.vals, &ctx->indTab.work, &ctx->bIndRef, &ctx->bIndIn};
  for (auto *b : all) freeBuf(*b);
  for (auto &slot : ctx->storeChunks)
    for (auto &b : slot) freeBuf(b);
  for (auto &b : ctx->bAlign) freeBuf(b);
  for (auto &e : ctx->ev) if (e) (void)hipEventDestroy(e);
  for (auto &e : ctx->upEv) if (e) (void)hipEventDestroy(e);
  if (ctx->stream) (void)hipStreamDestroy(ctx->stream);
  delete ctx;
}

const char *t1k_last_error(const t1k_ctx *ctx) { return ctx ? ctx->err.c_str() : "no context"; }

uint64_t t1k_ctx_mem_report(t1k_ctx *ctx, const char *tag, int print) {
  if (!ctx) return 0;
#define B(x) {#x, &ctx->x}
  const struct { const char *name; T1kDevBuf *b; } all[] = {B(bReadAscii), B(bReadOffs), B(bReadBases), B(bReadN), B(bReadLen), B(bReadWeight), B(bWgHits), B(bWgGroups),
    B(bWgStage), B(bWgBig), B(bWgCache), B(bLists), B(bCand), B(bExt), B(bCandStart), B(bCandCount), B(bListPtr), B(bListCount), B(bOvlWork), B(bOvlUpload), B(bDedupScratch), B(bDedupBases), B(bDedupN),
    B(bDedupLen), B(bDedupWeight), B(bOvlStart), B(bOvlCount), B(bCounters), B(bSlowQueue), B(bSlowScratch), B(bSortScratch), B(bSelClass), B(bEqTrace), B(bSortTmp), B(bJobSort), B(bEnd1),
    B(bEnd2), B(bHasN), B(bRows), B(bRowStart), B(bRowCount), B(bFragAssigned), B(bPairScratch), B(bPairOverflow), B(bPairBig), B(bExtractHuge), B(bEmRowPtr), B(bEmEc), B(bEmCount),
    B(bEmLen), B(bEmX0), B(bEmN), B(bEmPsum), B(bEmColPtr), B(bEmRowOf), B(bExtract), B(bPileup), B(bPileupIn), B(bSpIn), B(bPhIn), B(bPhObs), B(bPhArena), B(bSupIn), B(bIndRef), B(bIndIn),
    {"bIndKeys", &ctx->indTab.keys}, {"bIndVals", &ctx->indTab.vals}, {"bIndWork", &ctx->indTab.work},
    {"bSupSites", &ctx->supMap.buf}, {"bSupKeys", &ctx->supTab.keys}, {"bSupVals", &ctx->supTab.vals}, {"bSupWork", &ctx->supTab.work},
    {"bSpSites", &ctx->spMap.buf}, {"bSpKeys", &ctx->spTab.keys}, {"bSpVals", &ctx->spTab.vals}, {"bSpWork", &ctx->spTab.work},
    {"bPhSites", &ctx->phMap.buf}, {"bPhKeys", &ctx->phTab.keys}, {"bPhVals", &ctx->phTab.vals}, {"bPhWork", &ctx->phTab.work}};
#undef B
  uint64_t tot = 0, ref = 0, store = 0, align = 0;
  std::string line;
  for (auto &e : all) if (e.b->p) { tot += e.b->bytes; if (e.b->bytes >= (64u << 20)) { char t[96]; snprintf(t, sizeof t, " %s %.0f", e.name + 1, e.b->bytes / 1048576.0); line += t; } }
  for (auto &b : ctx->refBufs) if (b.p) ref += b.bytes;
  for (auto &slot : ctx->storeChunks) for (auto &b : slot) if (b.p) store += b.bytes;
  for (auto &b : ctx->bAlign) if (b.p) align += b.bytes;
  if (print)
    fprintf(stderr, "[t1k mem] %s: %.2f GB in named blocks + reference %.2f + overlap store %.2f + alignment phase %.2f GB; blocks of 64 MB and more (MB):%s\n", tag ? tag : "context",
            tot / 1073741824.0, ref / 1073741824.0, store / 1073741824.0, align / 1073741824.0, line.c_str());
  return tot + ref + store + align;
}

int t1k_missing_coverage(t1k_ctx *ctx, int32_t *missing) {
  if (!ctx || !ctx->ref.covDiff || !missing) return t1k_fail(ctx, T1K_ERR_STATE, "no reference");
  T1K_HIP(ctx, hipSetDevice(ctx->device));
  const uint32_t A = ctx->ref.nAlleles;
  T1kDevBuf dScratch, dMiss;
  int rc;
  const double t0 = nowMs();
  if ((rc = t1k_ensure(ctx, dScratch, (ctx->ref.totalBases + 2) * 4))) return rc;
  if ((rc = t1k_ensure(ctx, dMiss, (size_t)A * 4))) { freeBuf(dScratch); return rc; }
  const double t1 = nowMs();
  if ((rc = t1k_coverage_fold(ctx))) { freeBuf(dScratch); freeBuf(dMiss); return rc; }
  t1k_launch_missing_coverage(ctx, ctx->ref, (int32_t *)dScratch.p, (int32_t *)dMiss.p);
  hipMemcpyAsync(missing, dMiss.p, (size_t)A * 4, hipMemcpyDeviceToHost, ctx->stream);
  hipError_t e = hipStreamSynchronize(ctx->stream);
  if (getenv("T1K_DEBUG_PHASES")) fprintf(stderr, "[t1k] missing coverage: buffers %.1f ms, kernel + copy %.1f ms\n", t1 - t0, nowMs() - t1);
  freeBuf(dScratch); freeBuf(dMiss);
  if (e != hipSuccess) return t1k_fail(ctx, T1K_ERR_DEVICE, hipGetErrorString(e));
  return T1K_OK;
}
int t1k_coverage_device(t1k_ctx *ctx, void **devPtr, uint64_t *count) {
  if (!ctx || !ctx->ref.covDiff || !devPtr || !count) return t1k_fail(ctx, T1K_ERR_STATE, "no reference");
  T1K_HIP(ctx, hipSetDevice(ctx->device));
  if (int rc = t1k_coverage_fold(ctx)) return rc;
  T1K_HIP(ctx, hipStreamSynchronize(ctx->stream));
  *devPtr = ctx->ref.covDiff;
  *count = 2 * ctx->ref.covStride;
  return T1K_OK;
}

int t1k_ref_share(t1k_ctx *dst, const t1k_ctx *src) {
  if (!dst || !src || dst == src || !src->ref.bases || dst->device != src->device) return t1k_fail(dst, T1K_ERR_ARG, "t1k_ref_share: contexts do not match");
  if (dst->prm.kmer_length != src->prm.kmer_length) return t1k_fail(dst, T1K_ERR_ARG, "t1k_ref_share: different k-mer length");
  T1K_HIP(dst, hipSetDevice(dst->device));
  for (auto &b : dst->refBufs) freeBuf(b);
  dst->refBufs.clear();
  dst->ref = src->ref;
  dst->hAlleleOff = src->hAlleleOff;
  dst->hAlleleLen = src->hAlleleLen;
  T1kDevBuf cov;
  int rc;
  if ((rc = t1k_ensure(dst, cov, 3 * src->ref.covStride * sizeof(int32_t)))) return rc;
  T1K_HIP(dst, hipMemsetAsync(cov.p, 0, 3 * src->ref.covStride * sizeof(int32_t), dst->stream));
  T1K_HIP(dst, hipStreamSynchronize(dst->stream));
  dst->refBufs.push_back(cov);
  dst->ref.covDiff = (int32_t *)cov.p;
  dst->covFullLen = 0; dst->covFullDirty = false;
  return T1K_OK;
}
int t1k_reads_attach(t1k_ctx *dst, const t1k_ctx *src, int storeSlot, int resetStore) {
  if (!dst || !src || dst == src || dst->device != src->device || storeSlot < 0 || storeSlot > 1) return t1k_fail(dst, T1K_ERR_ARG, "t1k_reads_attach: contexts do not match");
  dst->reads = src->reads;
  dst->readsShared = true;
  dst->batchMaxLen = src->batchMaxLen; dst->batchFastMaxLen = src->batchFastMaxLen;
  dst->nCand = dst->nOvl = 0;
  dst->rangeCount = 0;
  dst->storeSlot = storeSlot;
  if (resetStore) { dst->storeChunk[storeSlot] = 0; dst->storeUsed[storeSlot] = 0; }
  return T1K_OK;
}
int t1k_reads_share(t1k_ctx *dst, const t1k_ctx *src) { return t1k_reads_attach(dst, src, 0, 1); }
int t1k_coverage_absorb(t1k_ctx *dst, t1k_ctx *src) {
  if (!dst || !src || !dst->ref.covDiff || !src->ref.covDiff || dst->device != src->device || dst->ref.totalBases != src->ref.totalBases)
    return t1k_fail(dst, T1K_ERR_ARG, "t1k_coverage_absorb: contexts do not match");
  T1K_HIP(dst, hipSetDevice(dst->device));
  if (int rc = t1k_coverage_fold(src)) return t1k_fail(dst, rc, "t1k_coverage_absorb: fold");
// ... 739 lines not shown
```

### t1k_amd/csrc/t1k_coalesce.hip

```cpp
#include <algorithm>
#include <thread>
#include <chrono>
#include <cstdio>
#include <cstdlib>
#include <cstring>
#include "t1k_dev.h"
#include "t1k_launch.h"

struct T1kGroupEnt { int32_t allele, start, end; float weight, adjustWeight; };

__global__ void k_co_flag(const uint32_t *rowCount, uint32_t *flag, uint32_t n) {
  const uint32_t f = blockIdx.x * blockDim.x + threadIdx.x;
  if (f < n) flag[f] = rowCount[f] ? 1u : 0u;
}
__global__ void k_co_compact(const uint32_t *flag, const uint32_t *pos, const unsigned long long *h2, uint32_t *idx, unsigned long long *key, uint32_t n) {
  const uint32_t f = blockIdx.x * blockDim.x + threadIdx.x;
  if (f < n && flag[f]) { idx[pos[f] - 1] = f; key[pos[f] - 1] = h2[f]; }
}
__global__ void k_co_gather_key(const uint32_t *idx, const unsigned long long *h, unsigned long long *key, uint32_t m) {
  const uint32_t j = blockIdx.x * blockDim.x + threadIdx.x;
  if (j < m) key[j] = h[idx[j]];
}
__global__ void k_co_mark(const uint32_t *idx, const unsigned long long *k1, const unsigned long long *h2, const unsigned long long *rowPtr, const uint32_t *rowCount,
                          uint32_t *flag, uint32_t m) {
// ... 171 lines not shown
          if (u < cnt) {
            if (e[u].x < a.x) a.x = e[u].x;
            if (e[u].y < a.y) a.y = e[u].x;
            wt += __int_as_float(e[u].z);
            aw += __int_as_float(e[u].w);
          }
        }
      }
      a.z = __float_as_int(wt); a.w = __float_as_int(aw);
      sAcc[lane] = a;
    }
    meet();
    loadRows();
    loadPtrs(min(b + 8, nBatches - 1));
    for (int t = ws + 1; t < 4; ++t) meet();
  }
  if (w == 0 && act) {
    const int4 a = sAcc[lane];
    out[groupPtr[g] + q] = T1kGroupEnt{allele, a.x, a.y, __int_as_float(a.z), __int_as_float(a.w)};
  }
}

__global__ void k_co_unsort(const unsigned long long *rowPtr, const uint32_t *rowCount, const unsigned long long *outOff, t1k_row_entry *out, uint64_t f0, uint32_t n) {
  const uint32_t i = blockIdx.x * 4 + (threadIdx.x >> 6);
  if (i >= n) return;
  const int lane = threadIdx.x & 63;
  const t1k_row_entry *r = (const t1k_row_entry *)rowPtr[f0 + i];
  const uint32_t c = rowCount[f0 + i];
  for (uint32_t q = lane; q < c; q += 64) {
    t1k_row_entry e = r[q];
    const uint32_t at = __float_as_uint(e.qual);
    e.qual = 1.0f;
    out[outOff[i] + at] = e;
  }
}

static uint32_t coLongRun() {
  static const uint32_t longRun = getenv("T1K_CO_LONG_RUN") ? (uint32_t)std::max(2 * CO_B + 2, atoi(getenv("T1K_CO_LONG_RUN"))) : (uint32_t)CO_LONG_RUN;
  return longRun;
}

static int rsFail(t1k_rowset *rs, int code, const std::string &m) { if (rs) rs->err = m; return code; }
#define RS_HIP(call) do { hipError_t e_ = (call); if (e_ != hipSuccess) return rsFail(rs, T1K_ERR_DEVICE, std::string(#call) + ": " + hipGetErrorString(e_)); } while (0)

int t1k_rowset_chunk(t1k_rowset *rs, t1k_ctx *ctx, size_t *chunk, t1k_row_entry **rows, uint64_t *cap, unsigned long long **cursor) {
  std::lock_guard<std::mutex> g(rs->m);
  if (rs->cur >= 1024) return t1k_fail(ctx, T1K_ERR_CAPACITY, "rowset: more than 1024 row chunks");
  if (rs->cur >= rs->chunks.size()) rs->chunks.resize(rs->cur + 1);
  T1kDevBuf &b = rs->chunks[rs->cur];
  if (!b.p) {
    hipError_t e = t1k_dev_malloc(&b.p, rs->chunkEntries * sizeof(t1k_row_entry));
    if (e != hipSuccess) { b.p = nullptr; return t1k_fail(ctx, T1K_ERR_DEVICE, std::string("rowset: hipMalloc of a row chunk failed: ") + hipGetErrorString(e)); }
    b.bytes = rs->chunkEntries * sizeof(t1k_row_entry);
  }
  *chunk = rs->cur; *rows = (t1k_row_entry *)b.p; *cap = rs->chunkEntries; *cursor = (unsigned long long *)rs->bCursors.p + rs->cur;
  return T1K_OK;
}
int t1k_rowset_chunk_full(t1k_rowset *rs, t1k_ctx *, size_t chunk) {
  std::lock_guard<std::mutex> g(rs->m);
  if (rs->cur == chunk) ++rs->cur;
  return T1K_OK;
}

extern "C" {

void t1k_coalesce_limits(uint32_t out[3]) {
  out[0] = CO_B; out[1] = coLongRun(); out[2] = 64;
}

int t1k_rowset_create(t1k_ctx *owner, uint64_t nFragments, const uint8_t *whitelist, t1k_rowset **out) {
  if (!owner || !out) return T1K_ERR_ARG;
  *out = nullptr;
  if (nFragments >= 0xFFFFFFF0ull) return t1k_fail(owner, T1K_ERR_ARG, "t1k_rowset_create: more than 2^32 fragments on one GPU");
  T1K_HIP(owner, hipSetDevice(owner->device));
  t1k_rowset *rs = new t1k_rowset();
  rs->device = owner->device; rs->owner = owner; rs->nFrag = nFragments;
  const uint64_t F = std::max<uint64_t>(nFragments, 1);
  int rc;
  if ((rc = t1k_ensure(owner, rs->bFrag, F * (8 * 3 + 4 + 1) + 256)) || (rc = t1k_ensure(owner, rs->bCursors, 1024 * 8))) { delete rs; return rc; }
  rs->rowPtr = (unsigned long long *)rs->bFrag.p; rs->h1 = rs->rowPtr + F; rs->h2 = rs->h1 + F;
  rs->rowCount = (uint32_t *)(rs->h2 + F); rs->assigned = (uint8_t *)(rs->rowCount + F);
  T1K_HIP(owner, hipMemsetAsync(rs->bFrag.p, 0, rs->bFrag.bytes, owner->stream));
  T1K_HIP(owner, hipMemsetAsync(rs->bCursors.p, 0, 1024 * 8, owner->stream));
  const char *ce = getenv("T1K_ROW_CHUNK");
  rs->chunkEntries = ce ? std::max<uint64_t>(1u << 16, strtoull(ce, nullptr, 10)) : std::max<uint64_t>((uint64_t)owner->prm.row_cap, 64ull << 20);
  if (whitelist) {
    const uint32_t A = owner->ref.nAlleles;
    if ((rc = t1k_ensure(owner, rs->bWhitelist, A))) { delete rs; return rc; }
    T1K_HIP(owner, hipMemcpyAsync(rs->bWhitelist.p, whitelist, A, hipMemcpyHostToDevice, owner->stream));
    rs->whitelist = (const uint8_t *)rs->bWhitelist.p;
  }
  T1K_HIP(owner, hipStreamSynchronize(owner->stream));
  *out = rs;
  return T1K_OK;
}

int t1k_rowset_trim(t1k_rowset *rs, uint64_t nFragments) {
  if (!rs || rs->exchanged || nFragments > rs->nFrag) return T1K_ERR_ARG;
  rs->nFrag = nFragments;
  return T1K_OK;
}

void t1k_rowset_destroy(t1k_rowset *rs) {
  if (!rs) return;
  (void)hipSetDevice(rs->device);
  T1kDevBuf *all[] = {&rs->bFrag, &rs->bCursors, &rs->bWhitelist, &rs->bWork, &rs->bGroupPtr, &rs->bGroupEnt, &rs->bGroupFirst, &rs->bSend, &rs->bRecv, &rs->bFrag2, &rs->bAll};
  for (auto *b : all) if (b->p) (void)t1k_dev_free(b->p);
  for (auto &b : rs->chunks) if (b.p) (void)t1k_dev_free(b.p);
  if (rs->copyStream) (void)hipStreamDestroy(rs->copyStream);
  delete rs;
}

int t1k_rowset_set_raw(t1k_rowset *rs, int raw) { if (!rs) return T1K_ERR_ARG; rs->rawKept = raw != 0; return T1K_OK; }
int t1k_rowset_device_bytes(t1k_rowset *rs, uint64_t *bytes, uint64_t *rowEntries) {
  if (!rs || !bytes) return T1K_ERR_ARG;
  size_t nChunks;
  {
    std::lock_guard<std::mutex> g(rs->m);
    uint64_t b = rs->bFrag.bytes;
    for (const T1kDevBuf &c : rs->chunks) if (c.p) b += c.bytes;
    *bytes = b;
    nChunks = std::min<size_t>(rs->chunks.size(), 1024);
  }
  if (rowEntries) {
    *rowEntries = 0;
    if (nChunks) {
      RS_HIP(hipSetDevice(rs->device));
      std::vector<unsigned long long> cur(nChunks);
      hipStream_t st = nullptr;
      RS_HIP(hipStreamCreateWithFlags(&st, hipStreamNonBlocking));
      hipError_t e = hipMemcpyAsync(cur.data(), rs->bCursors.p, nChunks * 8, hipMemcpyDeviceToHost, st);
      if (e == hipSuccess) e = hipStreamSynchronize(st);
      (void)hipStreamDestroy(st);
      RS_HIP(e);
      for (unsigned long long c : cur) *rowEntries += std::min<unsigned long long>(c, rs->chunkEntries);
    }
  }
  return T1K_OK;
}
const char *t1k_rowset_last_error(const t1k_rowset *rs) { return rs ? rs->err.c_str() : "no rowset"; }

int t1k_rowset_coalesce(t1k_rowset *rs, uint64_t *nGroups, uint64_t *nEntries, uint64_t *assignedFragments) {
  return t1k_rowset_coalesce_sized(rs, nGroups, nEntries, assignedFragments, nullptr, nullptr);
}

int t1k_rowset_coalesce_sized(t1k_rowset *rs, uint64_t *nGroups, uint64_t *nEntries, uint64_t *assignedFragments, void (*sized)(uint64_t, uint64_t, void *), void *user) {
  if (!rs) return T1K_ERR_ARG;
  t1k_ctx *ctx = rs->owner;
  RS_HIP(hipSetDevice(rs->device));
  hipStream_t st = ctx->stream;
  const uint32_t F = (uint32_t)rs->nFrag;
  rs->nGroups = rs->nEntries = 0;
  if (!rs->exchanged) rs->nAssigned = 0;
  rs->coalesced = true;
  if (nGroups) *nGroups = 0;
  if (nEntries) *nEntries = 0;
  if (assignedFragments) *assignedFragments = rs->exchanged ? rs->nAssigned : 0;
  if (F == 0) return T1K_OK;
  int rc;
  auto fail = [&](int code) { rs->err = ctx->err; return code; };
  const bool dbg = getenv("T1K_DEBUG_PHASES") != nullptr;
  auto tLap = std::chrono::steady_clock::now();
  auto lap = [&](const char *what) {
    if (!dbg) return;
    (void)hipStreamSynchronize(st);
    const auto now = std::chrono::steady_clock::now();
    fprintf(stderr, "[t1k] coalesce %s: %.1f ms\n", what, std::chrono::duration<double, std::milli>(now - tLap).count());
    tLap = now;
  };
  const size_t n4 = ((size_t)(F + 2) * 4 + 255) & ~(size_t)255, n8 = ((size_t)(F + 2) * 8 + 255) & ~(size_t)255;
  if ((rc = t1k_ensure(ctx, rs->bWork, 8 * n4 + 3 * n8))) return fail(rc);
  char *wp = (char *)rs->bWork.p;
  uint32_t *a0 = (uint32_t *)wp, *a1 = (uint32_t *)(wp + n4), *a2 = (uint32_t *)(wp + 2 * n4), *a3 = (uint32_t *)(wp + 3 * n4), *a4 = (uint32_t *)(wp + 4 * n4),
           *a5 = (uint32_t *)(wp + 5 * n4), *a6 = (uint32_t *)(wp + 6 * n4), *a7 = (uint32_t *)(wp + 7 * n4);
  unsigned long long *k0 = (unsigned long long *)(wp + 8 * n4), *k1 = (unsigned long long *)(wp + 8 * n4 + n8), *k2 = (unsigned long long *)(wp + 8 * n4 + 2 * n8);
  const unsigned nbF = (F + 255) / 256;
  hipLaunchKernelGGL(k_co_flag, dim3(nbF), dim3(256), 0, st, rs->rowCount, a0, F);
  if ((rc = t1k_inclusive_sum(ctx, a0, a1, F))) return fail(rc);
  uint32_t M = 0;
  RS_HIP(hipMemcpyAsync(&M, a1 + (F - 1), 4, hipMemcpyDeviceToHost, st));
  RS_HIP(hipStreamSynchronize(st));
  if (!rs->exchanged) rs->nAssigned = M;
  if (assignedFragments) *assignedFragments = rs->nAssigned;
  if (M == 0) return T1K_OK;
  hipLaunchKernelGGL(k_co_compact, dim3(nbF), dim3(256), 0, st, a0, a1, rs->h2, a2, k0, F);
  const unsigned nbM = (M + 255) / 256;
  if ((rc = t1k_sort_pairs(ctx, k0, k1, a2, a3, M))) return fail(rc);
  hipLaunchKernelGGL(k_co_gather_key, dim3(nbM), dim3(256), 0, st, a3, rs->h1, k0, M);
  if ((rc = t1k_sort_pairs(ctx, k0, k1, a3, a2, M))) return fail(rc);
  uint32_t *idx = a2;
  lap("compaction + two radix sorts");
  hipLaunchKernelGGL(k_co_mark, dim3(nbM), dim3(256), 0, st, idx, k1, rs->h2, rs->rowPtr, rs->rowCount, a0, M);
  if ((rc = t1k_inclusive_sum(ctx, a0, a1, M))) return fail(rc);
  uint32_t G = 0;
  RS_HIP(hipMemcpyAsync(&G, a1 + (M - 1), 4, hipMemcpyDeviceToHost, st));
  RS_HIP(hipStreamSynchronize(st));
  uint32_t *runStart = a3, *headVal = a4, *order = a5;
  hipLaunchKernelGGL(k_co_heads, dim3(nbM), dim3(256), 0, st, idx, a0, a1, runStart, k0, headVal, M);
  if ((rc = t1k_sort_pairs(ctx, k0, k2, headVal, order, G, 32))) return fail(rc);
  uint32_t *gSize = a0, *gTiles = a1, *gFirst = a6;
  const unsigned nbG = (G + 255) / 256;
  hipLaunchKernelGGL(k_co_sizes, dim3(nbG), dim3(256), 0, st, order, runStart, idx, rs->rowCount, rs->gid, gSize, gTiles, gFirst, G);
// ... 280 lines not shown
```

### t1k_amd/csrc/t1k_dev.h

```cpp
#pragma once
#include <hip/hip_runtime.h>
#include <stdint.h>
#include <string>
#include <type_traits>
#include <vector>
#include "../../include/t1k_gpu.h"

#define T1K_MAX_READ_LEN 320
#define T1K_LONG_READ_LEN 1000
#define T1K_EVEN 0x5555555555555555ull
#define T1K_NEG_BIG (-(1 << 28))

struct T1kPosting { uint32_t allele, offset; };

struct T1kCand {
  uint32_t allele;
  uint32_t readSE;
  int32_t seqStart, seqEnd;
  uint32_t match;
  uint32_t re;
};

struct T1kExt {
  int32_t seqStart, seqEnd;
// ... 716 lines not shown
}
__device__ __forceinline__ uint32_t t1k_block_scan_exclusive(uint32_t v, uint32_t *warpSums, uint32_t *total) {
  return t1k_block_scan_exclusive_n<4>(v, warpSums, total);
}

struct T1kDevBuf {
  void *p = nullptr;
  size_t bytes = 0;
};

struct T1kSiteMap {
  T1kDevBuf buf;
  size_t at[3] = {0, 0, 0};
  uint64_t nSites = 0;
  std::vector<uint64_t> off;
};
struct T1kCountTable {
  T1kDevBuf keys, vals, work;
  uint64_t runs = 0, pending = 0, cap = 0, bound = 0, emitted = 0, folds = 0;
  int endBit = 64;
  double foldMs = 0;
};

struct t1k_ctx {
  int device = 0;
  std::vector<unsigned long long> hRaw;
  hipStream_t stream = nullptr;
  hipEvent_t ev[12] = {};
  t1k_params prm;
  std::string err;
  T1kRefDev ref{};
  std::vector<uint64_t> hAlleleOff;
  std::vector<uint32_t> hAlleleLen;
  std::vector<T1kDevBuf> refBufs;
  T1kReadsDev reads{};
  T1kDevBuf bReadAscii, bReadOffs, bReadBases, bReadN, bReadLen, bReadWeight, bListPtr, bListCount;
  T1kDevBuf bDedupScratch, bDedupBases, bDedupN, bDedupLen, bDedupWeight;
  bool readsShared = false;
  int batchMaxLen = 0;
  int batchFastMaxLen = 0;
  int covFullLen = 0;
  bool covFullDirty = false;
  uint32_t rangeCount = 0;
  T1kDevBuf bWgHits, bWgGroups, bWgStage, bWgBig, bWgCache, bLists;
  std::vector<T1kDevBuf> storeChunks[2];
  int storeSlot = 0;
  size_t storeChunk[2] = {0, 0};
  uint64_t storeUsed[2] = {0, 0};
  T1kOvl *ovlBase = nullptr;
  T1kDevBuf bOvlWork;
  bool ovlPacked = false;
  T1kDevBuf bOvlUpload;
  T1kOvlP *storeBase = nullptr;
  uint64_t wGroup = 0, wList = 0, wRare = 0, wCand = 0, wOvl = 0, wJob = 0, wGenJob = 0, wGenHit = 0;
  uint64_t needGroup = 0, needList = 0, needRare = 0, needCand = 0, needOvl = 0, needJob = 0, needGenJob = 0, needGenHit = 0;
  unsigned long long lastCapFlags = 0;
  bool scaledOnce = false;
  bool covCommitted = false;
  uint32_t queueBoost = 1;
  int covMode = 0;
  double msAlloc = 0;
  uint64_t bytesAlloc = 0;
  T1kDevBuf bCand, bExt, bCandStart, bCandCount, bOvlStart, bOvlCount, bCounters, bSlowQueue, bSlowScratch, bSortScratch, bSelClass, bEqTrace, bSortTmp, bJobSort;
  uint64_t nCand = 0, nOvl = 0;
  T1kDevBuf bEnd1, bEnd2, bHasN, bRows, bRowStart, bRowCount, bFragAssigned, bPairScratch, bPairOverflow, bPairBig, bExtractHuge;
  uint32_t nFragments = 0;
  uint64_t nRows = 0;
  T1kDevBuf bEmRowPtr, bEmEc, bEmCount, bEmLen, bEmX0, bEmN, bEmPsum, bEmColPtr, bEmRowOf;
  std::vector<uint64_t> emPieceBytes, emPieceDispl;
  uint32_t emGroups = 0, emEc = 0, emRowBegin = 0, emRowEnd = 0;
  struct t1k_comm *emComm = nullptr;
  bool emReduceMode = false;
  uint64_t emNnz = 0;
  std::vector<int32_t> hEmLen;
  int traceFetch = 0;
  uint32_t upN = 0; int upS = 0, upMaxLen = 0; uint64_t upBytes = 0; bool upOpen = false;
  hipEvent_t upEv[4] = {nullptr, nullptr, nullptr, nullptr}; bool upEvSet[4] = {false, false, false, false};
  uint64_t lastSlowGroups = 0;
  uint64_t estTotal[T1K_NARENA] = {};
  bool estValid = false;
  struct { bool on = false; t1k_route_totals kept{}; std::vector<t1k_route_rec> keptRecs, passRecs; bool passLong = false, passXlong = false; } route;
  uint64_t pairEpoch = 0;
  uint64_t pairBigCap = 0;
  unsigned long long *countersPinned = nullptr;
  double *emPinned = nullptr;
  size_t emPinnedN = 0;
  double emMs[4] = {0, 0, 0, 0};
  t1k_allreduce_fn emAllreduce = nullptr;
  void *emUser = nullptr;
  T1kDevBuf bAlign[12];
  T1kDevBuf bExtract;
  T1kDevBuf bPileup, bPileupIn;
  bool pileupOpen = false;
  std::vector<uint64_t> pileupOff, pileupLoad;
  T1kSiteMap spMap;
  T1kCountTable spTab;
  T1kDevBuf bSpIn;
  bool spOpen = false;
  uint64_t spBarcodes = 0;
  T1kSiteMap supMap;
  T1kCountTable supTab;
  T1kDevBuf bSupIn;
  bool supOpen = false;
  T1kCountTable indTab;
  T1kDevBuf bIndRef, bIndIn;
  bool indOpen = false;
  size_t indTextAt = 0;
  std::vector<uint64_t> indOff;
  uint64_t indEvents = 0, indShifted = 0, indEdgeDel = 0, indEdgeIns = 0;
  T1kSiteMap phMap;
  T1kCountTable phTab;
  T1kDevBuf bPhIn, bPhObs, bPhArena;
  bool phOpen = false;
  uint64_t phObs = 0, phBookings = 0, phDiscordant = 0;
  t1k_stats stats{};
};

hipError_t t1k_dev_malloc(void **out, size_t bytes);
hipError_t t1k_dev_free(void *p);
uint64_t t1k_pool_cached_bytes(int device);
int t1k_fail(t1k_ctx *ctx, int code, const std::string &msg);
int t1k_ensure(t1k_ctx *ctx, T1kDevBuf &b, size_t bytes);
#define T1K_HIP(ctx, call)                                                                              \
  do {                                                                                                  \
    hipError_t e_ = (call);                                                                             \
    if (e_ != hipSuccess) return t1k_fail(ctx, T1K_ERR_DEVICE, std::string(#call) + ": " + hipGetErrorString(e_)); \
  } while (0)
```

### t1k_amd/csrc/t1k_launch.h

```cpp
#pragma once
#include <algorithm>
#include <mutex>
#include "t1k_dev.h"

#define T1K_USED_MASK_WORDS 10
struct ChainArgs {
  T1kRefDev ref;
  T1kReadsDev reads;
  int k, radius, hitLenRequired;
  double sim;
  uint32_t *recs; uint32_t recStride; uint64_t groupCap;
  uint32_t *chunkStart, *chunkCount; int maxChunks;
  uint32_t *usedMask;
  uint32_t *usedOut, *usedCount;
  unsigned long long *memo;
  uint32_t *jobList; uint32_t jobCap;
  uint32_t *retryList, *generalList, *bigList;
  uint32_t *jobStr, *retryStr, *generalStr, *bigStr, *finishStr, *waveStr, *waveList, *slowStr, *slowList;
  uint32_t groupSegCap, jobSegCap, listSegCap, rareSegCap, genCandSegCap, genHitSegCap;
  uint32_t maxK;
  uint32_t maxKFast;
  uint32_t *genJobStr, *genJobList; uint32_t genJobSegCap;
  uint32_t *genHits;
  uint32_t *genCand; uint32_t genCandCap;
// ... 17 lines not shown
  unsigned long long *counters;
  unsigned long long *memo;
  uint32_t *jobStr; uint32_t jobSegCap;
  uint32_t *retryStr; uint32_t retrySegCap;
};

struct SelectArgs {
  T1kReadsDev reads;
  const T1kCand *cand;
  const T1kExt *ext;
  const uint32_t *candStart, *candCount;
  T1kOvl *ovl; uint64_t ovlCap;
  uint32_t *ovlStart, *ovlCount;
  T1kOvlP *store;
  unsigned long long *listPtr;
  uint32_t *listCount;
  uint64_t *sortScratch;
  uint32_t sortCap;
  int alleleBits;
  int relax;
  int xl;
  unsigned long long *counters;
  uint32_t *classList;
  int lenWord, hoWord;
};

struct FullArgs {
  T1kRefDev ref;
  T1kReadsDev reads;
  int relax;
  int noCov;
  int fullLen;
  int undo;
  T1kOvl *ovl;
  uint64_t nOvl;
  uint32_t *eqStr, *bandStr, *wideStr; uint32_t segCap;
  unsigned long long *eqKeyStr, *bandKeyStr;
  unsigned long long *counters;
};

struct SlowArgs {
  T1kRefDev ref;
  T1kReadsDev reads;
  int relax;
  int noCov;
  T1kOvl *ovl;
  const uint32_t *slowQueue;
  uint32_t nSlow;
  const uint32_t *runOf, *rep; uint32_t nRuns; uint64_t traceStride;
  uint8_t *scratch; uint64_t perThread;
  int maxCells;
  unsigned long long *counters;
};

struct TruncArgs {
  T1kReadsDev reads;
  T1kOvl *ovl;
  const uint32_t *ovlStart;
  uint32_t *ovlCount;
  uint64_t *sortScratch; uint32_t sortCap;
  int alleleBits;
  int xl;
  unsigned long long *counters;
};

struct t1k_rowset {
  int device = 0;
  t1k_ctx *owner = nullptr;
  uint64_t nFrag = 0;
  T1kDevBuf bFrag;
  unsigned long long *rowPtr = nullptr, *h1 = nullptr, *h2 = nullptr;
  uint32_t *rowCount = nullptr;
  uint8_t *assigned = nullptr;
  uint32_t *gid = nullptr;
  bool exchanged = false;
  uint64_t nFragLocal = 0;
  T1kDevBuf bSend, bRecv, bFrag2, bAll;
  uint64_t allGroups = 0, allEntries = 0;
  T1kDevBuf bCursors;
  std::vector<T1kDevBuf> chunks;
  size_t cur = 0;
  uint64_t chunkEntries = 0;
  std::mutex m;
  T1kDevBuf bWhitelist;
  const uint8_t *whitelist = nullptr;
  bool rawKept = false;
  T1kDevBuf bWork, bGroupPtr, bGroupEnt, bGroupFirst;
  uint64_t nGroups = 0, nEntries = 0, nAssigned = 0;
  bool coalesced = false;
  hipStream_t copyStream = nullptr;
  std::string err;
};
struct T1kCarve {
  size_t off = 0;
  size_t operator()(size_t bytes) { const size_t o = off; off += (bytes + 255) / 256 * 256 + 256; return o; }
};
struct T1kCallBlock {
  T1kDevBuf buf;
  hipStream_t stream = nullptr;
  T1kCallBlock() = default;
  T1kCallBlock(const T1kCallBlock &) = delete;
  T1kCallBlock &operator=(const T1kCallBlock &) = delete;
  int alloc(t1k_ctx *ctx, size_t bytes) { stream = ctx->stream; return t1k_ensure(ctx, buf, bytes); }
  ~T1kCallBlock() {
    if (!buf.p) return;
    (void)hipStreamSynchronize(stream);
    (void)t1k_dev_free(buf.p);
  }
};
inline unsigned t1k_grid(t1k_ctx *ctx, uint64_t items, uint32_t perBlock, uint32_t blocksPerCu = 16) {
  int cus = 256;
  (void)hipDeviceGetAttribute(&cus, hipDeviceAttributeMultiprocessorCount, ctx->device);
  return (unsigned)std::max<uint64_t>(1, std::min<uint64_t>((uint64_t)cus * blocksPerCu, (items + perBlock - 1) / perBlock));
}
inline int t1k_bits(unsigned long long v) {
  int b = 1;
  while (b < 64 && (v >> b)) ++b;
  return b;
}

int t1k_rowset_chunk(t1k_rowset *rs, t1k_ctx *ctx, size_t *chunk, t1k_row_entry **rows, uint64_t *cap, unsigned long long **cursor);
int t1k_rowset_chunk_full(t1k_rowset *rs, t1k_ctx *ctx, size_t chunk);
int t1k_exclusive_sum64(t1k_ctx *ctx, const uint32_t *in, unsigned long long *out, uint32_t n);
int t1k_exclusive_sum32(t1k_ctx *ctx, const uint32_t *in, uint32_t *out, uint64_t n);
int t1k_exclusive_sum_u64(t1k_ctx *ctx, const unsigned long long *in, unsigned long long *out, uint64_t n);

int t1k_launch_pack(t1k_ctx *ctx, const char *dAscii, const uint64_t *dOffs, uint32_t n, int S, uint64_t *bases, uint64_t *nmask, uint16_t *lens, int nCode);
size_t t1k_slow_per_thread(int maxCells);
size_t t1k_chain_big_scratch_u32();
int t1k_chain_max_chunks(uint32_t nAlleles);
int t1k_chain_memo_entries();
int t1k_chain_rec_stride(int maxLen);
int t1k_chain_max_kmers(int maxLen, int k);
int t1k_chain_used_u32(int maxK);
int t1k_launch_seed(t1k_ctx *ctx, const ChainArgs &a, bool longReads, bool xlong);
int t1k_run_chain(t1k_ctx *ctx, const ChainArgs &a, int nWg, int bigBlocks, bool longReads, unsigned long long *hc);
void t1k_launch_extend(t1k_ctx *ctx, const ExtendArgs &a);
void t1k_launch_select(t1k_ctx *ctx, const SelectArgs &a, int nWg, bool packed);
void t1k_launch_fullalign(t1k_ctx *ctx, const FullArgs &a);
void t1k_launch_fullalign_slow(t1k_ctx *ctx, const SlowArgs &a, int nBlocks);
void t1k_launch_align_flags(t1k_ctx *ctx, const SlowArgs &a, uint32_t *flags);
void t1k_launch_align_reps(t1k_ctx *ctx, const uint32_t *flags, const uint32_t *runOf, uint32_t *rep, uint32_t n);
void t1k_launch_align_fill_apply(t1k_ctx *ctx, const SlowArgs &a, bool eq);
int t1k_inclusive_sum(t1k_ctx *ctx, const uint32_t *in, uint32_t *out, uint64_t n);
void t1k_launch_truncate(t1k_ctx *ctx, const TruncArgs &a, int nWg);
void t1k_launch_coverage_scan(t1k_ctx *ctx, const T1kRefDev &ref, int32_t *out, const uint64_t *outOff);
int t1k_fetch_counters(t1k_ctx *ctx, unsigned long long *h);
int t1k_fullalign_phase(t1k_ctx *ctx, const T1kReadsDev &rd, T1kOvl *ovl, uint64_t nOvl, int relaxFlag, int noCov, int maxLen, bool exactQueues, unsigned long long *hc);
struct T1kArenaCounts { uint64_t total; uint32_t maxSeg; bool overflow; };
T1kArenaCounts t1k_arena_counts(const t1k_ctx *ctx, int arena, uint32_t segCap);
void t1k_launch_coverage_add(t1k_ctx *ctx, int32_t *dst, int32_t *src, uint64_t n);
int t1k_coverage_fold(t1k_ctx *ctx);
void t1k_launch_missing_coverage(t1k_ctx *ctx, const T1kRefDev &ref, int32_t *scratch, int32_t *missing);
void t1k_arena_compact_dev(t1k_ctx *ctx, int arena, const uint32_t *src, uint32_t segCap, uint32_t *dst, uint64_t estTotal);
void t1k_launch_dp_dense_dev(t1k_ctx *ctx, const ChainArgs &a, const uint32_t *jobs, int arena, uint32_t cap, uint64_t est);
uint64_t t1k_arena_estimate(const t1k_ctx *ctx, int arena, uint64_t cap, uint32_t nRe);
void t1k_arena_estimate_set(t1k_ctx *ctx, int arena, uint64_t total, uint32_t nRe);
void t1k_launch_extend_retry_dev(t1k_ctx *ctx, const ExtendArgs &a, const uint32_t *list, int arena, uint64_t est);
void t1k_arena_compact64(t1k_ctx *ctx, int arena, const unsigned long long *src, uint32_t segCap, unsigned long long *dst, uint32_t maxSeg);
int t1k_run_table(t1k_ctx *ctx, const unsigned long long *keys, uint32_t n, const unsigned long long *lone,
                  uint32_t *flag, uint32_t *scan, uint32_t *runStart, unsigned long long *runKey, uint32_t *runs);
int t1k_sort_pairs(t1k_ctx *ctx, const unsigned long long *keysIn, unsigned long long *keysOut, const uint32_t *valsIn, uint32_t *valsOut, uint32_t n, int endBit = 64);
void t1k_arena_compact(t1k_ctx *ctx, int arena, const uint32_t *src, uint32_t segCap, uint32_t *dst, uint32_t maxSeg);

void t1k_launch_extract(t1k_ctx *ctx, const T1kRefDev &ref, const T1kReadsDev &reads, int k, int radius, int hitLenRequired, double oneMinusSim, uint32_t nFragments,
                        uint32_t epf, uint32_t maxK, uint8_t *good, uint8_t *state, unsigned long long *err, unsigned long long *stats, int nWg);
void t1k_launch_extract_huge(t1k_ctx *ctx, const T1kRefDev &ref, const T1kReadsDev &reads, int k, int radius, int hitLenRequired, double oneMinusSim,
                             uint32_t nFragments, uint32_t epf, uint32_t maxK, uint8_t *good, uint8_t *state, unsigned long long *err, unsigned long long *stats, int nWg,
                             uint32_t *scratch, uint32_t cap);
void t1k_launch_extract_big(t1k_ctx *ctx, const T1kRefDev &ref, const T1kReadsDev &reads, int k, int radius, int hitLenRequired, double oneMinusSim,
                            uint32_t nFragments, uint32_t epf, uint32_t maxK, uint8_t *good, uint8_t *state, unsigned long long *err, unsigned long long *stats, int nWg);
```

### t1k_amd/csrc/t1k_pair.hip

```cpp
#include <algorithm>
#include <chrono>
#include <cstring>
#include "t1k_dev.h"
#include "t1k_launch.h"

#ifdef T1K_PAIR_PROFILE
#define PP(i) do { if (tid == 0) { const uint64_t tn_ = __builtin_amdgcn_s_memtime(); tp_[i] += tn_ - tl_; tl_ = tn_; } } while (0)
#else
#define PP(i) do { } while (0)
#endif
#ifdef T1K_PAIR_ROUTES
#define T1K_ROUTE_COUNT() do { if (tid == 0) { const int r_ = 2 * ((jt.direct() ? 2 : jt.lds() ? 0 : 1) + (P.only ? 3 : 0)); \
  atomicAdd(&P.counters[40 + r_], 1ull); atomicAdd(&P.counters[41 + r_], (unsigned long long)(n1 + n2)); } } while (0)
#else
#define T1K_ROUTE_COUNT() do { } while (0)
#endif
#define SORT_TILE 2048
constexpr uint32_t ljCapacity(uint32_t slots) { return slots * 17 / 25; }
template <int LJ_SLOTS>
__device__ __forceinline__ uint32_t ljHash(uint32_t allele) { return (allele * 2654435761u) >> (LJ_SLOTS == 4096 ? 20 : 21); }
template <int LJ_SLOTS>
__device__ __forceinline__ uint32_t ljInsert(uint32_t *hKey, uint32_t allele) {
  const uint32_t key = allele + 1;
  uint32_t h = ljHash<LJ_SLOTS>(allele);
  for (;;) {
    const uint32_t k = hKey[h];
    if (k == key) return h;
    if (k == 0) {
      const uint32_t old = atomicCAS(&hKey[h], 0u, key);
      if (old == 0 || old == key) return h;
    }
    h = (h + 1) & (LJ_SLOTS - 1);
  }
}
template <int LJ_SLOTS>
__device__ __forceinline__ int ljFind(const uint32_t *hKey, uint32_t allele) {
  const uint32_t key = allele + 1;
  uint32_t h = ljHash<LJ_SLOTS>(allele);
  for (;;) {
    const uint32_t k = hKey[h];
    if (k == key) return (int)h;
    if (k == 0) return -1;
    h = (h + 1) & (LJ_SLOTS - 1);
  }
}

constexpr uint32_t directCapacity(uint32_t slots) { return 2 * slots; }
static int pairDirectOn() {
  static const int on = [] { const char *e = getenv("T1K_PAIR_DIRECT"); return e && !strcmp(e, "0") ? 0 : 1; }();
  return on;
}

enum { JT_HASH = 0, JT_DIRECT = 1, JT_HBM = 2, JT_HBM_DUP = 3 };
template <int LJ_SLOTS>
struct JoinTab {
  uint32_t *mem;
  uint64_t *tab2, *tabSlot;
  uint32_t ep;
  uint32_t lo, range;
  int kind;
  __device__ __forceinline__ bool lds() const { return kind <= JT_DIRECT; }
  __device__ __forceinline__ bool direct() const { return kind == JT_DIRECT; }
  __device__ __forceinline__ uint32_t words() const { return direct() ? range : 2u * LJ_SLOTS; }
  __device__ __forceinline__ void toHbm(bool dup) { kind = dup ? JT_HBM_DUP : JT_HBM; }
  __device__ __forceinline__ bool stamped(uint64_t e) const { return (uint32_t)(e >> 32) == ep; }
  __device__ __forceinline__ int word(uint32_t allele) const {
    if (direct()) { const uint32_t d = allele - lo; return d < range ? (int)d : -1; }
    const int s = ljFind<LJ_SLOTS>(mem, allele);
    return s >= 0 ? LJ_SLOTS + s : -1;
  }
  __device__ __forceinline__ bool insert1(uint32_t allele, uint32_t i) {
    if (!lds()) return stamped(atomicExch((unsigned long long *)&tabSlot[allele], (unsigned long long)((uint64_t)ep << 32 | i)));
    const uint32_t w = direct() ? allele - lo : LJ_SLOTS + ljInsert<LJ_SLOTS>(mem, allele);
    return (atomicOr(&mem[w], i + 1) & 0x7FFFu) != 0;
  }
  __device__ __forceinline__ bool insert2(uint32_t allele, uint32_t j) {
    if (!lds()) return stamped(atomicExch((unsigned long long *)&tab2[allele], (unsigned long long)((uint64_t)ep << 32 | j)));
    const uint32_t w = direct() ? allele - lo : LJ_SLOTS + ljInsert<LJ_SLOTS>(mem, allele);
    return (atomicOr(&mem[w], (j + 1) << 16) >> 16) != 0;
  }
  __device__ __forceinline__ int mate(uint32_t allele, int &w) const {
    if (lds()) { w = word(allele); return w >= 0 ? (int)(mem[w] >> 16) - 1 : -1; }
    const uint64_t e = tab2[allele];
    return stamped(e) ? (int)(e & 0x3FFFFFFFu) : -1;
  }
  __device__ __forceinline__ int mate(uint32_t allele) const { int w = -1; return mate(allele, w); }
  __device__ __forceinline__ void mark(int w, uint32_t allele) { if (lds()) atomicOr(&mem[w], 0x8000u); else tab2[allele] |= 0x80000000ull; }
  __device__ __forceinline__ bool member(uint32_t allele) const {
    if (lds()) { const int w = word(allele); return w >= 0 && (mem[w] & 0x8000u) != 0; }
    if (kind != JT_HBM_DUP) { const uint64_t e = tab2[allele]; return stamped(e) && (e & 0x80000000ull); }
    const uint64_t e = tabSlot[allele]; return stamped(e) && (e & 0x40000000ull);
  }
};

__device__ __forceinline__ unsigned long long t1k_pattern_mix(uint32_t allele, uint32_t r, unsigned long long k) {
  unsigned long long x = ((unsigned long long)allele << 32 | r) * k;
  x ^= x >> 31; x *= 0xD6E8FEB86659FD93ull; x ^= x >> 29;
  return x;
}

#ifndef T1K_PAIR_UNROLL
#define T1K_PAIR_UNROLL 2
#endif
#ifndef T1K_PAIR_HANDOUT
#define T1K_PAIR_HANDOUT 4
#endif
#ifndef T1K_ROW_RESERVE
#define T1K_ROW_RESERVE 32
#endif
#ifndef T1K_PAIR_WAVES
#define T1K_PAIR_WAVES 4
#endif
struct Frag {
  uint32_t allele;
  int32_t i, j;
  int32_t matchCnt, relaxed, seqStart, seqEnd;
  int32_t slot;
  double sim;
};

struct PairArgs {
  T1kRefDev ref;
  const unsigned long long *listPtr;
  const uint32_t *listCount;
  const uint32_t *end1, *end2;
  const uint8_t *hasN;
  uint32_t nFragments;
  double sim; int relax; int maxAssign; int hitLenRequired;
  t1k_row_entry *rows; uint64_t rowCap;
  uint32_t *rowStart, *rowCount; uint8_t *fragAssigned;
  uint64_t *tab2, *tabSlot;
  uint32_t epochBase;
  Frag *frags; uint32_t fragCap;
  uint32_t *keep;
  unsigned long long *counters;
  const uint32_t *only;
  Frag *bigFrags; uint32_t *bigKeep; uint64_t bigCap;
  uint32_t *overflowList;
  int direct;
  const uint8_t *whitelist;
  int listForm;
  int rawKept;
  unsigned long long *rsRowPtr; uint32_t *rsRowCount; unsigned long long *rsH1, *rsH2; uint8_t *rsAssigned;
  t1k_row_entry *rsRows; uint64_t rsCap; unsigned long long *rsCursor; uint64_t fragBase;
};

struct OvlList {
  const T1kOvlP *p;
  __device__ __forceinline__ T1kOvl operator[](uint32_t i) const { return t1k_ovl_unpack(p[i]); }
};

__device__ __forceinline__ double ovlSim(const T1kOvl &o) {
  return (double)o.matchCnt / (double)(o.readEnd - o.readStart + 1 + o.seqEnd - o.seqStart + 1 + 2 * o.leftClip + 2 * o.rightClip);
}
__device__ __forceinline__ int ovlStrand(const T1kOvl &o) { return (o.flags & 2) ? -1 : 1; }

__device__ __forceinline__ bool sepInRangeP(const T1kRefDev &ref, uint32_t allele, int s, int e) {
  int len = (int)ref.alleleLen[allele];
  if (s <= -1 && e >= -1) return true;
  if (s <= len && e >= len) return true;
  uint32_t b = ref.sepStart[allele], en = ref.sepStart[allele + 1];
  for (uint32_t i = b; i < en; ++i) {
    int p = ref.sepPos[i];
    if (p >= s && p <= e) return true;
  }
  return false;
}

__device__ inline void makeFrag(Frag &f, const T1kOvl *o1, int i, const T1kOvl *o2, int j) {
  const T1kOvl &o = o1 ? *o1 : *o2;
  f.allele = o.allele; f.i = o1 ? i : -1; f.j = o2 ? j : -1; f.slot = -1;
  f.matchCnt = o.matchCnt; f.relaxed = o.relaxed; f.seqStart = o.seqStart; f.seqEnd = o.seqEnd; f.sim = ovlSim(o);
  if (o1 && o2) {
    f.matchCnt += o2->matchCnt;
    f.relaxed += o2->relaxed;
    if (ovlStrand(o) == 1) f.seqEnd = o2->seqEnd; else f.seqStart = o2->seqStart;
    f.sim = (double)f.matchCnt / (double)(o.readEnd - o.readStart + 1 + o2->readEnd - o2->readStart + 1 + o.seqEnd - o.seqStart + 1 + o2->seqEnd -
                                          o2->seqStart + 1 + 2 * o.leftClip + 2 * o.rightClip + 2 * o2->leftClip + 2 * o2->rightClip);
  }
}

__device__ inline bool fragBefore(const Frag &a, const T1kOvl &a1, const Frag &b, const T1kOvl &b1) {
  if (a.matchCnt != b.matchCnt) return a.matchCnt > b.matchCnt;
  if (a.sim != b.sim) return a.sim > b.sim;
  if (a1.matchCnt != b1.matchCnt) return a1.matchCnt > b1.matchCnt;
  double sa = ovlSim(a1), sb = ovlSim(b1);
  if (sa != sb) return sa > sb;
  if (a1.readEnd - a1.readStart != b1.readEnd - b1.readStart) return a1.readEnd - a1.readStart > b1.readEnd - b1.readStart;
  if (a1.allele != b1.allele) return a1.allele < b1.allele;
  if (ovlStrand(a1) != ovlStrand(b1)) return ovlStrand(a1) < ovlStrand(b1);
  if (a1.readStart != b1.readStart) return a1.readStart < b1.readStart;
  if (a1.readEnd != b1.readEnd) return a1.readEnd < b1.readEnd;
  if (a1.seqStart != b1.seqStart) return a1.seqStart < b1.seqStart;
  return a1.seqEnd < b1.seqEnd;
}

__device__ inline bool truncatedMate(const T1kRefDev &ref, const T1kOvl &o, const T1kOvl &c1, const T1kOvl &c2) {
  if (ovlStrand(o) == 1) {
    if ((int)ref.alleleLen[o.allele] - 1 < o.seqEnd + c2.seqEnd - c1.seqEnd || sepInRangeP(ref, o.allele, o.seqEnd, o.seqEnd + c2.seqEnd - c1.seqEnd + 1))
      return true;
  } else {
    if (o.seqStart - (c1.seqStart - c2.seqStart) < 0 || sepInRangeP(ref, o.allele, o.seqStart - (c1.seqStart - c2.seqStart) - 1, o.seqStart)) return true;
  }
  return false;
}

__device__ __forceinline__ float rowWeight(double sim, double s, bool hasN) {
  double ret = 1;
  double segment = (1 - s) / 4.0;
  if (segment < 0.01) segment = 0.01;
  if (sim < 1 - 3 * segment) ret = 0.01;
  else if (sim < 1 - 2 * segment) ret = 0.1;
  else if (sim < 1 - segment) ret = 0.5;
  if (hasN) ret /= 10.0;
  return (float)ret;
}

template <int NWAVE>
__device__ __forceinline__ uint32_t scanExcl(uint32_t v, uint32_t *warpSums, uint32_t *total) {
  int lane = threadIdx.x & 63, wave = threadIdx.x >> 6;
  uint32_t x = v;
#pragma unroll
  for (int o = 1; o < 64; o <<= 1) {
    uint32_t y = __shfl_up(x, o, 64);
    if (lane >= o) x += y;
  }
  if (NWAVE == 1) {
    *total = __shfl(x, 63, 64);
    return x - v;
  }
  if (lane == 63) warpSums[wave] = x;
  __syncthreads();
  uint32_t base = 0, tot = 0;
#pragma unroll
  for (int w = 0; w < NWAVE; ++w) { if (w < wave) base += warpSums[w]; tot += warpSums[w]; }
  __syncthreads();
  *total = tot;
  return base + x - v;
}

template <int WG, int LJ_SLOTS>
__global__ __launch_bounds__(WG) __attribute__((amdgpu_waves_per_eu(T1K_PAIR_WAVES, T1K_PAIR_WAVES))) void k_pair(PairArgs P) {
  constexpr int NWAVE = WG / 64;
  constexpr int PU = T1K_PAIR_UNROLL;
  constexpr uint32_t LJ_CAP = ljCapacity(LJ_SLOTS);
  constexpr uint32_t DIRECT_CAP = directCapacity(LJ_SLOTS);
  static_assert(DIRECT_CAP <= 32766, "a list of the direct route numbers its records in 15 bits");
  __shared__ uint32_t warpSums[NWAVE];
  __shared__ int sDup, sFail, sBestM, sBestIdx, sAnySep, sNotOne;
  __shared__ double sBestSim;
  __shared__ uint32_t sN, sBase;
  __shared__ uint32_t sLo, sHi;
  __shared__ uint32_t ljMem[2 * LJ_SLOTS];
  const int tid = threadIdx.x;
  const uint32_t A = P.ref.nAlleles;
  uint64_t *tab2 = P.tab2 + (uint64_t)blockIdx.x * A;
  uint64_t *tabSlot = P.tabSlot + (uint64_t)blockIdx.x * A;
  Frag *frags = P.frags + (uint64_t)blockIdx.x * P.fragCap;
  uint32_t *keep = P.keep + (uint64_t)blockIdx.x * P.fragCap;
  uint32_t fragCap = P.fragCap;
#ifdef T1K_PAIR_PROFILE
  uint64_t tp_[8] = {0, 0, 0, 0, 0, 0, 0, 0}, tl_ = __builtin_amdgcn_s_memtime();
#endif
  const uint32_t nItems = P.only ? (uint32_t)P.counters[23] : P.nFragments;
  __shared__ uint32_t sItem;
  uint32_t hoNext = 0, hoLeft = 0;
  __shared__ unsigned long long sStatOvl, sStatRows;
  if (tid == 0) { sStatOvl = 0; sStatRows = 0; }
  unsigned long long rowNext = 0; uint32_t rowLeft = 0;
  for (;;) {
    if (tid == 0) {
      if (hoLeft == 0) { hoNext = (uint32_t)atomicAdd(&P.counters[P.only ? 26 : 25], (unsigned long long)T1K_PAIR_HANDOUT); hoLeft = T1K_PAIR_HANDOUT; }
      sItem = hoNext++; --hoLeft;
      sDup = 0; sFail = 0; sBestM = -1; sBestIdx = 0x7FFFFFFF; sAnySep = 0; sNotOne = 0; sN = 0; sLo = 0xFFFFFFFFu; sHi = 0;
    }
    __syncthreads();
    const uint32_t it = sItem;
    if (it >= nItems) break;
    const uint32_t f = P.only ? P.only[2 * it] : it;
    const uint64_t epoch = (uint64_t)(P.epochBase + f + 1) << 32;
    const bool paired = P.end2 != nullptr;
    const uint32_t e1 = P.end1[f];
    const uint32_t e2 = paired ? P.end2[f] : 0u;
    const bool hasN = P.hasN ? P.hasN[f] != 0 : false;
    const uint32_t n1 = P.listCount[e1];
    const OvlList L1{(const T1kOvlP *)P.listPtr[e1]};
    uint32_t n2 = 0;
    OvlList L2{nullptr};
    if (paired) { n2 = P.listCount[e2]; L2.p = (const T1kOvlP *)P.listPtr[e2]; }
    const bool dangling = paired && (n1 == 0 || n2 == 0);
    const bool both = paired && !dangling;
    uint32_t nFrag = 0;
    if (P.only) {
      const uint64_t off = P.only[2 * it + 1];
      fragCap = off + n1 + n2 <= P.bigCap ? n1 + n2 : 0u;
      frags = P.bigFrags + off; keep = P.bigKeep + off;
    }
    if (n1 + n2 > fragCap) {
      if (P.overflowList) {
        if (tid == 0) {
          const unsigned long long q = atomicAdd(&P.counters[23], 1ull);
          const unsigned long long off = atomicAdd(&P.counters[24], (unsigned long long)(n1 + n2));
          P.overflowList[2 * q] = f; P.overflowList[2 * q + 1] = (uint32_t)min(off, 0xFFFFFFFFull);
        }
        __syncthreads();
        continue;
      }
      if (tid == 0) {
        atomicOr(&P.counters[2], P.only ? 1024ull : 128ull);
        if (P.rsRowPtr) { P.rsRowCount[P.fragBase + f] = 0; P.rsAssigned[P.fragBase + f] = 0; }
        else { P.rowStart[f] = 0; P.rowCount[f] = 0; P.fragAssigned[f] = 0; }
      }
      __syncthreads();
      continue;
    }
    if (tid == 0) sStatOvl += n1 + n2;
    JoinTab<LJ_SLOTS> jt{ljMem, tab2, tabSlot, (uint32_t)(epoch >> 32), 0u, 0u, n1 + n2 <= LJ_CAP ? JT_HASH : JT_HBM};
    if (P.direct && !jt.lds()) {
      uint32_t lo = 0xFFFFFFFFu, hi = 0;
      for (uint32_t i0 = tid; i0 < n1; i0 += 4 * WG) {
        uint32_t al[4];
#pragma unroll
        for (int r = 0; r < 4; ++r) al[r] = i0 + r * WG < n1 ? (uint32_t)(L1.p[i0 + r * WG].lo & 0xFFFFFFu) : 0u;
#pragma unroll
        for (int r = 0; r < 4; ++r)
          if (i0 + r * WG < n1) { lo = min(lo, al[r]); hi = max(hi, al[r]); }
      }
      for (uint32_t j0 = tid; j0 < n2; j0 += 4 * WG) {
        uint32_t al[4];
#pragma unroll
        for (int r = 0; r < 4; ++r) al[r] = j0 + r * WG < n2 ? (uint32_t)(L2.p[j0 + r * WG].lo & 0xFFFFFFu) : 0u;
#pragma unroll
        for (int r = 0; r < 4; ++r)
          if (j0 + r * WG < n2) { lo = min(lo, al[r]); hi = max(hi, al[r]); }
      }
#pragma unroll
      for (int o = 32; o > 0; o >>= 1) { lo = min(lo, (uint32_t)__shfl_xor((int)lo, o, 64)); hi = max(hi, (uint32_t)__shfl_xor((int)hi, o, 64)); }
      if ((tid & 63) == 0 && lo <= hi) { atomicMin(&sLo, lo); atomicMax(&sHi, hi); }
      __syncthreads();
      lo = sLo; hi = sHi;
      if (lo <= hi && hi - lo < DIRECT_CAP && n1 <= hi - lo + 1 && n2 <= hi - lo + 1) { jt.kind = JT_DIRECT; jt.lo = lo; jt.range = hi - lo + 1; }
    }
    if (jt.lds()) {
      for (uint32_t q = tid, nq = jt.words(); q < nq; q += WG) ljMem[q] = 0;
      __syncthreads();
      for (uint32_t i0 = tid; i0 < n1; i0 += 4 * WG) {
        uint32_t al[4];
#pragma unroll
        for (int r = 0; r < 4; ++r) al[r] = i0 + r * WG < n1 ? (uint32_t)(L1.p[i0 + r * WG].lo & 0xFFFFFFu) : 0u;
#pragma unroll
        for (int r = 0; r < 4; ++r) {
          const uint32_t i = i0 + r * WG;
          if (i < n1 && jt.insert1(al[r], i)) sDup = 1;
        }
      }
      for (uint32_t j0 = tid; j0 < n2; j0 += 4 * WG) {
        uint32_t al[4];
#pragma unroll
        for (int r = 0; r < 4; ++r) al[r] = j0 + r * WG < n2 ? (uint32_t)(L2.p[j0 + r * WG].lo & 0xFFFFFFu) : 0u;
#pragma unroll
        for (int r = 0; r < 4; ++r) {
          const uint32_t j = j0 + r * WG;
// ... 366 lines not shown
        }
      }
      __syncthreads();
      continue;
    }
    PP(5);
    __shared__ unsigned long long sRowBase;
    uint32_t *sAllele = ljMem;
    static_assert(SORT_TILE <= LJ_SLOTS, "the rank-sort tile lives in the join table's first words");
    __shared__ unsigned long long sHash[2][NWAVE];
    if (tid == 0) {
      unsigned long long b = 0;
      bool fitsChunk = true;
      if (nRow) {
        if (T1K_ROW_RESERVE > 0 && nRow <= rowLeft) { b = rowNext; rowNext += nRow; rowLeft -= nRow; }
        else {
          const unsigned long long take = (unsigned long long)(T1K_ROW_RESERVE > 0 && nRow < (uint32_t)T1K_ROW_RESERVE ? (uint32_t)T1K_ROW_RESERVE : nRow);
          b = atomicAdd(P.rsCursor, take);
          if (b + take > P.rsCap) fitsChunk = false; else { rowNext = b + nRow; rowLeft = (uint32_t)(take - nRow); }
        }
      }
      if (!fitsChunk) { atomicOr(&P.counters[2], 128ull); sRowBase = ~0ull; }
      else { sRowBase = b; sStatRows += nRow; }
    }
    for (uint32_t q = tid; q < nRow; q += WG) frags[keep[q]].slot = 0;
    for (uint32_t t0 = 0; t0 < nRow; t0 += SORT_TILE) {
      const uint32_t tn = min(nRow - t0, (uint32_t)SORT_TILE);
      __syncthreads();
      for (uint32_t i = tid; i < tn; i += WG) sAllele[i] = frags[keep[t0 + i]].allele;
      __syncthreads();
      for (uint32_t q = tid; q < nRow; q += WG) {
        Frag &fr = frags[keep[q]];
        const uint32_t a = fr.allele;
        int c = 0;
        for (uint32_t i = 0; i < tn; ++i) c += sAllele[i] < a ? 1 : 0;
        fr.slot += c;
      }
    }
    __syncthreads();
    PP(6);
    unsigned long long h1 = 0, h2 = 0;
    const bool fits = sRowBase != ~0ull;
    for (uint32_t q = tid; q < nRow; q += WG) {
      const Frag &fr = frags[keep[q]];
      const uint32_t r = (uint32_t)fr.slot;
      h1 += t1k_pattern_mix(fr.allele, r, 0x9E3779B97F4A7C15ull);
      h2 += t1k_pattern_mix(fr.allele, r, 0xC2B2AE3D27D4EB4Full);
      if (fits) {
        t1k_row_entry e;
        e.allele_idx = (int32_t)fr.allele; e.start = fr.seqStart; e.end = fr.seqEnd;
        e.weight = rowWeight(fr.sim, P.sim, hasN);
        e.qual = __uint_as_float(q);
        e.adjust_weight = (float)(adjust * e.weight);
        P.rsRows[sRowBase + r] = e;
      }
    }
#pragma unroll
    for (int o = 32; o > 0; o >>= 1) { h1 += __shfl_down(h1, o, 64); h2 += __shfl_down(h2, o, 64); }
    if ((tid & 63) == 0) { sHash[0][tid >> 6] = h1; sHash[1][tid >> 6] = h2; }
    __syncthreads();
    if (tid == 0) {
      const uint64_t g = P.fragBase + f;
      P.rsRowPtr[g] = fits ? (unsigned long long)(P.rsRows + sRowBase) : 0ull;
      P.rsRowCount[g] = fits ? nRow : 0;
      unsigned long long t1 = 0, t2 = 0;
#pragma unroll
      for (int w = 0; w < NWAVE; ++w) { t1 += sHash[0][w]; t2 += sHash[1][w]; }
      P.rsH1[g] = t1 + 0x632BE59BD9B4E019ull * nRow;
      P.rsH2[g] = t2 + 0xA0761D6478BD642Full * nRow;
      P.rsAssigned[g] = anyKept ? 1 : 0;
    }
    __syncthreads();
    PP(7);
  }
  if (tid == 0) {
    if (sStatOvl) atomicAdd(&P.counters[22], sStatOvl);
    if (sStatRows) atomicAdd(&P.counters[9], sStatRows);
  }
#ifdef T1K_PAIR_PROFILE
  if (tid == 0) for (int i = 0; i < 8; ++i) atomicAdd(&P.counters[32 + i], (unsigned long long)tp_[i]);
#endif
}

constexpr int PAIR_WG = 256, PAIR_LJ_SLOTS = 4096;
static uint32_t pairFragCap() {
  static const uint32_t cap = [] { const char *e = getenv("T1K_PAIR_FRAGCAP"); return e ? (uint32_t)std::max(8, atoi(e)) : 8192u; }();
  return cap;
}

static int pairLaunch(t1k_ctx *ctx, t1k_rowset *rs, const uint32_t *end1, const uint32_t *end2, const uint8_t *hasN, uint32_t nFragments, uint64_t fragBase,
                      const uint8_t *dWhitelist) {
  if (!ctx->ref.bases) return t1k_fail(ctx, T1K_ERR_STATE, "mate pairing: no reference");
  if (!ctx->reads.listPtr) return t1k_fail(ctx, T1K_ERR_STATE, "mate pairing: no reads uploaded");
  T1K_HIP(ctx, hipSetDevice(ctx->device));
  int rc;
  const uint32_t n = nFragments;
  const int wgThreads = 256;
  static const int maxWg = [] { const char *e = getenv("T1K_PAIR_WGS"); return e ? std::max(64, std::min(4096, atoi(e))) : 1024; }();
  const int nWg = (int)std::min<uint32_t>(maxWg, std::max<uint32_t>(n, 1));
  auto launch = [&](unsigned grid, const PairArgs &args) { hipLaunchKernelGGL((k_pair<PAIR_WG, PAIR_LJ_SLOTS>), dim3(grid), dim3(PAIR_WG), 0, ctx->stream, args); };
  const uint32_t envFragCap = pairFragCap();
  static const uint64_t envBigCap = [] { const char *e = getenv("T1K_PAIR_BIGCAP"); return e ? (uint64_t)std::max(64, atoi(e)) : (uint64_t)(8u << 20); }();
  const uint32_t fragCap = envFragCap;
  const uint32_t A = ctx->ref.nAlleles;
  if (!rs) { ctx->nFragments = n; ctx->nRows = 0; }
  if ((rc = t1k_ensure(ctx, ctx->bEnd1, (size_t)n * 4))) return rc;
  if ((rc = t1k_ensure(ctx, ctx->bEnd2, (size_t)n * 4))) return rc;
  if ((rc = t1k_ensure(ctx, ctx->bHasN, (size_t)n))) return rc;
  if (!rs) {
    if ((rc = t1k_ensure(ctx, ctx->bRows, (size_t)ctx->prm.row_cap * sizeof(t1k_row_entry)))) return rc;
    if ((rc = t1k_ensure(ctx, ctx->bRowStart, (size_t)n * 4))) return rc;
    if ((rc = t1k_ensure(ctx, ctx->bRowCount, (size_t)n * 4))) return rc;
    if ((rc = t1k_ensure(ctx, ctx->bFragAssigned, (size_t)n))) return rc;
  }
  size_t perWg = (size_t)A * 16 + (size_t)fragCap * (sizeof(Frag) + 4);
  bool fresh = ctx->bPairScratch.bytes < (size_t)maxWg * perWg;
  if ((rc = t1k_ensure(ctx, ctx->bPairScratch, (size_t)maxWg * perWg))) return rc;
  if ((rc = t1k_ensure(ctx, ctx->bPairOverflow, (size_t)n * 8 + 16))) return rc;
  if (ctx->pairBigCap == 0) ctx->pairBigCap = envBigCap;
  if ((rc = t1k_ensure(ctx, ctx->bPairBig, (size_t)ctx->pairBigCap * (sizeof(Frag) + 4)))) return rc;
  if ((rc = t1k_ensure(ctx, ctx->bCounters, (size_t)T1K_COUNTER_WORDS * 8))) return rc;
  if (n == 0) return T1K_OK;
  T1K_HIP(ctx, hipMemcpyAsync(ctx->bEnd1.p, end1, (size_t)n * 4, hipMemcpyHostToDevice, ctx->stream));
  if (end2) T1K_HIP(ctx, hipMemcpyAsync(ctx->bEnd2.p, end2, (size_t)n * 4, hipMemcpyHostToDevice, ctx->stream));
  if (hasN) T1K_HIP(ctx, hipMemcpyAsync(ctx->bHasN.p, hasN, (size_t)n, hipMemcpyHostToDevice, ctx->stream));
  else T1K_HIP(ctx, hipMemsetAsync(ctx->bHasN.p, 0, (size_t)n, ctx->stream));
  if (fresh || ctx->pairEpoch > 0xFFFFFFFFull - 12ull * n - 2) {
    T1K_HIP(ctx, hipMemsetAsync(ctx->bPairScratch.p, 0, (size_t)maxWg * (size_t)A * 16, ctx->stream));
    ctx->pairEpoch = 0;
  }
  PairArgs p{};
  p.ref = ctx->ref;
  p.listPtr = ctx->reads.listPtr; p.listCount = ctx->reads.listCount;
  p.end1 = (const uint32_t *)ctx->bEnd1.p; p.end2 = end2 ? (const uint32_t *)ctx->bEnd2.p : nullptr; p.hasN = (const uint8_t *)ctx->bHasN.p;
  p.nFragments = n; p.sim = ctx->prm.ref_seq_similarity; p.relax = ctx->prm.relax_intron_align; p.maxAssign = ctx->prm.max_assign_cnt;
  p.hitLenRequired = ctx->prm.hit_len_required;
  p.rows = (t1k_row_entry *)ctx->bRows.p; p.rowCap = (uint64_t)ctx->prm.row_cap;
  p.rowStart = (uint32_t *)ctx->bRowStart.p; p.rowCount = (uint32_t *)ctx->bRowCount.p; p.fragAssigned = (uint8_t *)ctx->bFragAssigned.p;
  uint8_t *sc = (uint8_t *)ctx->bPairScratch.p;
  p.tab2 = (uint64_t *)sc;
  p.tabSlot = (uint64_t *)(sc + (size_t)maxWg * A * 8);
  p.frags = (Frag *)(sc + (size_t)maxWg * A * 16);
  p.fragCap = fragCap;
  p.keep = (uint32_t *)(sc + (size_t)maxWg * A * 16 + (size_t)maxWg * fragCap * sizeof(Frag));
  p.overflowList = (uint32_t *)ctx->bPairOverflow.p;
  p.counters = (unsigned long long *)ctx->bCounters.p;
  p.whitelist = dWhitelist;
  { static const int lf = getenv("T1K_PAIR_LIST") ? 1 : 0; p.listForm = lf; }
  p.direct = pairDirectOn();
  if (getenv("T1K_DEBUG_TRACE")) fprintf(stderr, "[t1k trace] pair %u fragments%s\n", n, rs ? " into the rowset" : "");
  for (int attempt = 0;; ++attempt) {
    T1K_HIP(ctx, hipMemsetAsync((char *)ctx->bCounters.p + 2 * 8, 0, 8, ctx->stream));
    T1K_HIP(ctx, hipMemsetAsync((char *)ctx->bCounters.p + 9 * 8, 0, 8, ctx->stream));
    T1K_HIP(ctx, hipMemsetAsync((char *)ctx->bCounters.p + 22 * 8, 0, 40, ctx->stream));
#ifdef T1K_PAIR_ROUTES
    T1K_HIP(ctx, hipMemsetAsync((char *)ctx->bCounters.p + 40 * 8, 0, 12 * 8, ctx->stream));
#endif
    size_t chunk = 0;
    if (rs) {
      if ((rc = t1k_rowset_chunk(rs, ctx, &chunk, &p.rsRows, &p.rsCap, &p.rsCursor))) return rc;
      p.rawKept = rs->rawKept ? 1 : 0;
      p.rsRowPtr = rs->rowPtr; p.rsRowCount = rs->rowCount; p.rsH1 = rs->h1; p.rsH2 = rs->h2; p.rsAssigned = rs->assigned; p.fragBase = fragBase;
    }
    p.epochBase = (uint32_t)ctx->pairEpoch; ctx->pairEpoch += n;
    p.only = nullptr; p.overflowList = (uint32_t *)ctx->bPairOverflow.p;
    T1K_HIP(ctx, hipEventRecord(ctx->ev[5], ctx->stream));
    launch((unsigned)nWg, p);
    {
      PairArgs q = p;
      q.only = (const uint32_t *)ctx->bPairOverflow.p; q.overflowList = nullptr;
      q.bigFrags = (Frag *)ctx->bPairBig.p; q.bigKeep = (uint32_t *)((char *)ctx->bPairBig.p + (size_t)ctx->pairBigCap * sizeof(Frag)); q.bigCap = ctx->pairBigCap;
      q.epochBase = (uint32_t)ctx->pairEpoch; ctx->pairEpoch += n;
      launch((unsigned)nWg, q);
    }
    T1K_HIP(ctx, hipEventRecord(ctx->ev[6], ctx->stream));
    if (!ctx->countersPinned) T1K_HIP(ctx, hipHostMalloc((void **)&ctx->countersPinned, (size_t)T1K_COUNTER_WORDS * 8, hipHostMallocDefault));
    T1K_HIP(ctx, hipMemcpyAsync(ctx->countersPinned, ctx->bCounters.p, 64 * 8, hipMemcpyDeviceToHost, ctx->stream));
    T1K_HIP(ctx, hipStreamSynchronize(ctx->stream));
    unsigned long long *hc = ctx->countersPinned;
    { float ms = 0; (void)hipEventElapsedTime(&ms, ctx->ev[5], ctx->ev[6]); ctx->stats.ms_pair = (attempt ? ctx->stats.ms_pair : 0) + ms; }
    if ((hc[2] & 1024ull) && attempt < 4) {
      ctx->pairBigCap = (uint64_t)((double)hc[24] * 1.25) + (getenv("T1K_PAIR_BIGCAP") ? 16 : (1u << 20));
      if ((rc = t1k_ensure(ctx, ctx->bPairBig, (size_t)ctx->pairBigCap * (sizeof(Frag) + 4)))) return rc;
      if (getenv("T1K_DEBUG_TRACE")) fprintf(stderr, "[t1k trace] pair: big arena grows to %llu entries\n", (unsigned long long)ctx->pairBigCap);
      if (!rs || !(hc[2] & ~1024ull)) continue;
    }
    if (hc[2] && rs && attempt < 4) {
      if ((rc = t1k_rowset_chunk_full(rs, ctx, chunk))) return rc;
      continue;
    }
    if (hc[2]) return t1k_fail(ctx, T1K_ERR_CAPACITY, "device arena overflow: row_cap / fragment scratch");
    if (!rs) ctx->nRows = hc[9];
    ctx->stats.rows = hc[9]; ctx->stats.pair_overlaps = hc[22];
#ifdef T1K_PAIR_ROUTES
    {
      static unsigned long long sum[12];
      static const int once = atexit([] {
        static const char *name[6] = {"hash, first launch", "HBM, first launch", "direct, first launch", "hash, second launch", "HBM, second launch", "direct, second launch"};
        for (int r = 0; r < 6; ++r) fprintf(stderr, "[t1k] pair routes (direct route %d): %-22s %12llu fragments %14llu records\n", pairDirectOn(), name[r], sum[2 * r], sum[2 * r + 1]);
      });
      (void)once;
      for (int r = 0; r < 12; ++r) __atomic_fetch_add(&sum[r], hc[40 + r], __ATOMIC_RELAXED);
    }
#endif
#ifdef T1K_PAIR_PROFILE
    fprintf(stderr, "[t1k] pair phases (ticks, thread 0 of every workgroup): tables %llu join %llu best %llu keep %llu rules %llu setreads %llu rank %llu rows+hash %llu\n", hc[32], hc[33], hc[34], hc[35], hc[36], hc[37], hc[38], hc[39]);
#endif
    return T1K_OK;
  }
}

extern "C" {

int t1k_pair_batch(t1k_ctx *ctx, const uint32_t *end1, const uint32_t *end2, const uint8_t *hasN, uint32_t nFragments) {
  if (!ctx || !end1) return t1k_fail(ctx, T1K_ERR_ARG, "t1k_pair_batch: bad arguments");
  return pairLaunch(ctx, nullptr, end1, end2, hasN, nFragments, 0, nullptr);
}

int t1k_pair_into(t1k_ctx *ctx, t1k_rowset *rs, const uint32_t *end1, const uint32_t *end2, const uint8_t *hasN, uint32_t nFragments, uint64_t fragBase) {
  if (!ctx || !rs || !end1) return t1k_fail(ctx, T1K_ERR_ARG, "t1k_pair_into: bad arguments");
  if (fragBase + nFragments > rs->nFrag) return t1k_fail(ctx, T1K_ERR_ARG, "t1k_pair_into: fragments outside the rowset");
  if (rs->device != ctx->device) return t1k_fail(ctx, T1K_ERR_ARG, "t1k_pair_into: rowset lives on another device");
  return pairLaunch(ctx, rs, end1, end2, hasN, nFragments, fragBase, rs->whitelist);
}

void t1k_pair_limits(uint32_t out[4]) {
  out[0] = ljCapacity(PAIR_LJ_SLOTS);
  out[1] = pairFragCap();
  out[2] = SORT_TILE;
  out[3] = PAIR_WG * T1K_PAIR_UNROLL;
}

uint32_t t1k_pair_direct_cap(void) { return directCapacity(PAIR_LJ_SLOTS); }

int t1k_rows_download(t1k_ctx *ctx, uint32_t *rowCounts, uint8_t *fragAssigned, t1k_row_entry *rows, uint64_t cap, uint64_t *total) {
  if (!ctx) return T1K_ERR_ARG;
  T1K_HIP(ctx, hipSetDevice(ctx->device));
  const uint32_t n = ctx->nFragments;
  std::vector<uint32_t> start(n), cnt(n);
  if (n) {
    T1K_HIP(ctx, hipMemcpy(start.data(), ctx->bRowStart.p, (size_t)n * 4, hipMemcpyDeviceToHost));
    T1K_HIP(ctx, hipMemcpy(cnt.data(), ctx->bRowCount.p, (size_t)n * 4, hipMemcpyDeviceToHost));
    if (fragAssigned) T1K_HIP(ctx, hipMemcpy(fragAssigned, ctx->bFragAssigned.p, (size_t)n, hipMemcpyDeviceToHost));
  }
  uint64_t tot = 0;
  for (uint32_t i = 0; i < n; ++i) tot += cnt[i];
  if (total) *total = tot;
  if (rowCounts) memcpy(rowCounts, cnt.data(), (size_t)n * 4);
  if (!rows) return T1K_OK;
  if (cap < tot) return t1k_fail(ctx, T1K_ERR_ARG, "row buffer too small");
  std::vector<t1k_row_entry> h(ctx->nRows);
  if (ctx->nRows) T1K_HIP(ctx, hipMemcpy(h.data(), ctx->bRows.p, ctx->nRows * sizeof(t1k_row_entry), hipMemcpyDeviceToHost));
  uint64_t w = 0;
  for (uint32_t i = 0; i < n; ++i) {
    if (cnt[i]) memcpy(rows + w, h.data() + start[i], (size_t)cnt[i] * sizeof(t1k_row_entry));
    w += cnt[i];
  }
  return T1K_OK;
}

}
```

Before: 4.060 million.

## Memoize pairing results for fragments with identical overlap-list pairs across batches

Adds a device hash table keyed by each fragment's pair of overlap-list pointers and counts (plus hasN). A probe kernel runs before the pairing kernel: a fragment whose keys match an earlier fragment copies that fragment's row pointer, count, hashes and assigned flag, and only the misses are compacted into a todo list that the pairing kernel walks. Once pairing finishes, newly computed fragments are published into the table when deferred mode is on. This avoids redoing the pair join for duplicate fragments, at the cost of an extra probe launch, a publish launch with a host sync, and roughly 24 bytes per slot of device memory.

Result: faster. 4.137 million, median of 6 (+1.9%).

```diff
diff --git a/include/t1k_gpu.h b/include/t1k_gpu.h
--- a/include/t1k_gpu.h
+++ b/include/t1k_gpu.h
@@ -92,6 +92,7 @@
 int t1k_rowset_device_bytes(t1k_rowset *rs, uint64_t *bytes, uint64_t *rowEntries);
 const char *t1k_rowset_last_error(const t1k_rowset *rs);
 int t1k_pair_into(t1k_ctx *ctx, t1k_rowset *rs, const uint32_t *end1, const uint32_t *end2, const uint8_t *hasN, uint32_t nFragments, uint64_t fragBase);
+int t1k_ctx_set_pair_memo(t1k_ctx *ctx, int publish);
 int t1k_rowset_coalesce(t1k_rowset *rs, uint64_t *nGroups, uint64_t *nEntries, uint64_t *assignedFragments);
 int t1k_rowset_coalesce_sized(t1k_rowset *rs, uint64_t *nGroups, uint64_t *nEntries, uint64_t *assignedFragments, void (*sized)(uint64_t nGroups, uint64_t nEntries, void *user), void *user);
 int t1k_rowset_groups_download(t1k_rowset *rs, uint64_t *groupPtr, t1k_group_entry *entries, uint32_t *firstFragment);
@@ -233,6 +234,7 @@
   double ms_seed, ms_chain, ms_extend, ms_select, ms_fullalign, ms_pair, ms_em, ms_total;
   uint64_t read_ends_total, pair_overlaps, dp_cells;
   double ms_load, ms_device, ms_coalesce, ms_write;
+  uint64_t pair_memo_hits, pair_memo_records;
 } t1k_stats;
 int t1k_stats_get(t1k_ctx *ctx, t1k_stats *out);
 
diff --git a/t1k_amd/capi.py b/t1k_amd/capi.py
--- a/t1k_amd/capi.py
+++ b/t1k_amd/capi.py
@@ -34,7 +34,8 @@
                                           "near_best", "dp_calls", "rows", "batches")] + \
                [(n, C.c_double) for n in ("ms_seed", "ms_chain", "ms_extend", "ms_select", "ms_fullalign", "ms_pair", "ms_em", "ms_total")] + \
                [(n, C.c_uint64) for n in ("read_ends_total", "pair_overlaps", "dp_cells")] + \
-               [(n, C.c_double) for n in ("ms_load", "ms_device", "ms_coalesce", "ms_write")]
+               [(n, C.c_double) for n in ("ms_load", "ms_device", "ms_coalesce", "ms_write")] + \
+               [(n, C.c_uint64) for n in ("pair_memo_hits", "pair_memo_records")]
 
     def as_dict(self):
         return {n: getattr(self, n) for n, _ in self._fields_}
@@ -205,6 +206,7 @@
     L.t1k_coverage_device.argtypes = [vp, C.POINTER(vp), u64p]
     L.t1k_device_memory.argtypes = [C.c_int, u64p, u64p]
     L.t1k_ctx_set_coverage_mode.argtypes = [vp, C.c_int]
+    L.t1k_ctx_set_pair_memo.argtypes = [vp, C.c_int]
     L.t1k_readset_detach.argtypes = [vp, C.POINTER(vp)]
     L.t1k_readset_take_store.argtypes = [vp, vp, C.c_int]
     L.t1k_readset_bytes.argtypes = [vp]
@@ -360,6 +362,9 @@
     def set_coverage_mode(self, deferred):
         self._check(lib().t1k_ctx_set_coverage_mode(self.h, 1 if deferred else 0), "t1k_ctx_set_coverage_mode")
 
+    def set_pair_memo(self, publish):
+        self._check(lib().t1k_ctx_set_pair_memo(self.h, 1 if publish else 0), "t1k_ctx_set_pair_memo")
+
     def detach_readset(self, slot=0):
         h = C.c_void_p()
         self._check(lib().t1k_readset_detach(self.h, C.byref(h)), "t1k_readset_detach")
diff --git a/t1k_amd/csrc/host/job.cpp b/t1k_amd/csrc/host/job.cpp
--- a/t1k_amd/csrc/host/job.cpp
+++ b/t1k_amd/csrc/host/job.cpp
@@ -517,7 +517,7 @@
             uint64_t freeNow = 0, totalNow = 0, rowsNow = 0, entriesNow = 0;
             if (t1k_device_memory(job->prm.device, &freeNow, &totalNow) == T1K_OK && t1k_rowset_device_bytes(job->rows, &rowsNow, &entriesNow) == T1K_OK && totalNow) {
               if (testHeadroom) { const uint64_t used = totalNow - std::min(freeNow, totalNow); totalNow = used + ((uint64_t)atoll(testHeadroom) << 20); freeNow = totalNow - used; }
-              const double projectedRows = (double)entriesNow / (double)sh.pairedFrags * (double)F * sizeof(t1k_row_entry) * 1.1 + 32.0 * (double)F + std::min(4e9, 0.015 * (double)totalNow);
+              const double projectedRows = (double)entriesNow / (double)sh.pairedFrags * (double)F * sizeof(t1k_row_entry) * 1.1 + (32.0 + 60.0) * (double)F + std::min(4e9, 0.015 * (double)totalNow);
               const uint64_t usedNow = totalNow - std::min(freeNow, totalNow);
               const uint64_t other = usedNow > archivedBytes + rowsNow ? usedNow - archivedBytes - rowsNow : 0;
               const double coalesceWork = 48.0 * (double)F + std::min(8e9, 0.03 * (double)totalNow);
@@ -732,6 +732,7 @@
         attached = (int)w;
       }
       if (r == T1K_OK) (void)t1k_ctx_set_coverage_mode(ctx, (W.deferred || job->analyzer) ? 1 : 0);
+      if (r == T1K_OK) (void)t1k_ctx_set_pair_memo(ctx, W.deferred ? 1 : 0);
       if (r == T1K_OK && kind == 0) {
         const uint32_t b0 = item * W.assignBatch, nb = std::min(W.assignBatch, W.nDistinct - b0);
         r = assignRange(ctx, W, b0, nb, msg);
@@ -746,6 +747,7 @@
           t1k_stats_get(ctx, &st);
           std::lock_guard<std::mutex> g(sh.m);
           job->stats.ms_pair += st.ms_pair; job->stats.pair_overlaps += st.pair_overlaps; job->stats.rows += st.rows;
+          job->stats.pair_memo_hits += st.pair_memo_hits; job->stats.pair_memo_records += st.pair_memo_records;
           sh.pairedFrags += nq;
         }
       }
@@ -976,6 +978,9 @@
   if (getenv("T1K_DEBUG_PHASES"))
     fprintf(stderr, "[t1k job] %u windows, %llu read-ends -> %llu distinct; window preparation %.1f ms (overlapped), device loop %.1f ms, coalesce + download %.1f ms (%llu groups, %llu entries)\n",
             sh.created, (unsigned long long)job->readEnds, (unsigned long long)job->distinctReadEnds, msPrep, job->msDevice, job->msCoalesce, (unsigned long long)G, (unsigned long long)N);
+  if (getenv("T1K_DEBUG_PHASES"))
+    fprintf(stderr, "[t1k job] pairing memo: %llu of %llu fragments took an earlier fragment's row (%llu list records not read, %llu read)\n",
+            (unsigned long long)job->stats.pair_memo_hits, (unsigned long long)F, (unsigned long long)job->stats.pair_memo_records, (unsigned long long)job->stats.pair_overlaps);
   if (getenv("T1K_DEBUG_PHASES") && job->covDeferred)
     fprintf(stderr, "[t1k job] coverage deferred to selection: read sets of %zu of %u windows kept (%.2f GB of device memory)\n", job->archive.size(), sh.created, archivedBytes / 1073741824.0);
   job->localDone = true;
diff --git a/t1k_amd/csrc/t1k_capi.hip b/t1k_amd/csrc/t1k_capi.hip
--- a/t1k_amd/csrc/t1k_capi.hip
+++ b/t1k_amd/csrc/t1k_capi.hip
@@ -286,7 +286,7 @@
   T1kDevBuf *all[] = {&ctx->bReadAscii, &ctx->bReadOffs, &ctx->bReadBases, &ctx->bReadN, &ctx->bReadLen, &ctx->bReadWeight, &ctx->bWgHits, &ctx->bWgGroups,
                       &ctx->bWgStage, &ctx->bWgBig, &ctx->bWgCache, &ctx->bLists, &ctx->bCand, &ctx->bExt, &ctx->bCandStart, &ctx->bCandCount, &ctx->bListPtr, &ctx->bListCount,
                       &ctx->bOvlWork, &ctx->bOvlUpload, &ctx->bDedupScratch, &ctx->bDedupBases, &ctx->bDedupN, &ctx->bDedupLen, &ctx->bDedupWeight, &ctx->bOvlStart, &ctx->bOvlCount, &ctx->bCounters, &ctx->bSlowQueue, &ctx->bSlowScratch, &ctx->bSortScratch, &ctx->bSelClass, &ctx->bEqTrace, &ctx->bSortTmp, &ctx->bJobSort, &ctx->bEnd1, &ctx->bEnd2,
-                      &ctx->bHasN, &ctx->bRows, &ctx->bRowStart, &ctx->bRowCount, &ctx->bFragAssigned, &ctx->bPairScratch, &ctx->bPairOverflow, &ctx->bPairBig, &ctx->bExtractHuge, &ctx->bEmRowPtr, &ctx->bEmEc,
+                      &ctx->bHasN, &ctx->bRows, &ctx->bRowStart, &ctx->bRowCount, &ctx->bFragAssigned, &ctx->bPairScratch, &ctx->bPairOverflow, &ctx->bPairTodo, &ctx->bPairBig, &ctx->bExtractHuge, &ctx->bEmRowPtr, &ctx->bEmEc,
                       &ctx->bEmCount, &ctx->bEmLen, &ctx->bEmX0, &ctx->bEmN, &ctx->bEmPsum, &ctx->bEmColPtr, &ctx->bEmRowOf, &ctx->bExtract, &ctx->bPileup, &ctx->bPileupIn, &ctx->spMap.buf, &ctx->spTab.keys, &ctx->spTab.vals, &ctx->spTab.work, &ctx->bSpIn,
                       &ctx->phMap.buf, &ctx->phTab.keys, &ctx->phTab.vals, &ctx->phTab.work, &ctx->bPhIn, &ctx->bPhObs, &ctx->bPhArena,
                       &ctx->supMap.buf, &ctx->supTab.keys, &ctx->supTab.vals, &ctx->supTab.work, &ctx->bSupIn,
@@ -309,7 +309,7 @@
   const struct { const char *name; T1kDevBuf *b; } all[] = {B(bReadAscii), B(bReadOffs), B(bReadBases), B(bReadN), B(bReadLen), B(bReadWeight), B(bWgHits), B(bWgGroups),
     B(bWgStage), B(bWgBig), B(bWgCache), B(bLists), B(bCand), B(bExt), B(bCandStart), B(bCandCount), B(bListPtr), B(bListCount), B(bOvlWork), B(bOvlUpload), B(bDedupScratch), B(bDedupBases), B(bDedupN),
     B(bDedupLen), B(bDedupWeight), B(bOvlStart), B(bOvlCount), B(bCounters), B(bSlowQueue), B(bSlowScratch), B(bSortScratch), B(bSelClass), B(bEqTrace), B(bSortTmp), B(bJobSort), B(bEnd1),
-    B(bEnd2), B(bHasN), B(bRows), B(bRowStart), B(bRowCount), B(bFragAssigned), B(bPairScratch), B(bPairOverflow), B(bPairBig), B(bExtractHuge), B(bEmRowPtr), B(bEmEc), B(bEmCount),
+    B(bEnd2), B(bHasN), B(bRows), B(bRowStart), B(bRowCount), B(bFragAssigned), B(bPairScratch), B(bPairOverflow), B(bPairTodo), B(bPairBig), B(bExtractHuge), B(bEmRowPtr), B(bEmEc), B(bEmCount),
     B(bEmLen), B(bEmX0), B(bEmN), B(bEmPsum), B(bEmColPtr), B(bEmRowOf), B(bExtract), B(bPileup), B(bPileupIn), B(bSpIn), B(bPhIn), B(bPhObs), B(bPhArena), B(bSupIn), B(bIndRef), B(bIndIn),
     {"bIndKeys", &ctx->indTab.keys}, {"bIndVals", &ctx->indTab.vals}, {"bIndWork", &ctx->indTab.work},
     {"bSupSites", &ctx->supMap.buf}, {"bSupKeys", &ctx->supTab.keys}, {"bSupVals", &ctx->supTab.vals}, {"bSupWork", &ctx->supTab.work},
diff --git a/t1k_amd/csrc/t1k_coalesce.hip b/t1k_amd/csrc/t1k_coalesce.hip
--- a/t1k_amd/csrc/t1k_coalesce.hip
+++ b/t1k_amd/csrc/t1k_coalesce.hip
@@ -277,6 +277,13 @@
   rs->rowCount = (uint32_t *)(rs->h2 + F); rs->assigned = (uint8_t *)(rs->rowCount + F);
   T1K_HIP(owner, hipMemsetAsync(rs->bFrag.p, 0, rs->bFrag.bytes, owner->stream));
   T1K_HIP(owner, hipMemsetAsync(rs->bCursors.p, 0, 1024 * 8, owner->stream));
+  if (const uint64_t slots = nFragments ? t1k_pair_memo_slots(nFragments) : 0) {
+    if (t1k_dev_malloc(&rs->bMemo.p, slots * 24) == hipSuccess) {
+      rs->bMemo.bytes = slots * 24;
+      rs->memo = (PairMemoEntry *)rs->bMemo.p; rs->memoSlots = slots;
+      T1K_HIP(owner, hipMemsetAsync(rs->bMemo.p, 0, rs->bMemo.bytes, owner->stream));
+    } else { rs->bMemo.p = nullptr; (void)hipGetLastError(); }
+  }
   const char *ce = getenv("T1K_ROW_CHUNK");
   rs->chunkEntries = ce ? std::max<uint64_t>(1u << 16, strtoull(ce, nullptr, 10)) : std::max<uint64_t>((uint64_t)owner->prm.row_cap, 64ull << 20);
   if (whitelist) {
@@ -299,7 +306,7 @@
 void t1k_rowset_destroy(t1k_rowset *rs) {
   if (!rs) return;
   (void)hipSetDevice(rs->device);
-  T1kDevBuf *all[] = {&rs->bFrag, &rs->bCursors, &rs->bWhitelist, &rs->bWork, &rs->bGroupPtr, &rs->bGroupEnt, &rs->bGroupFirst, &rs->bSend, &rs->bRecv, &rs->bFrag2, &rs->bAll};
+  T1kDevBuf *all[] = {&rs->bFrag, &rs->bCursors, &rs->bMemo, &rs->bWhitelist, &rs->bWork, &rs->bGroupPtr, &rs->bGroupEnt, &rs->bGroupFirst, &rs->bSend, &rs->bRecv, &rs->bFrag2, &rs->bAll};
   for (auto *b : all) if (b->p) (void)t1k_dev_free(b->p);
   for (auto &b : rs->chunks) if (b.p) (void)t1k_dev_free(b.p);
   if (rs->copyStream) (void)hipStreamDestroy(rs->copyStream);
@@ -312,7 +319,7 @@
   size_t nChunks;
   {
     std::lock_guard<std::mutex> g(rs->m);
-    uint64_t b = rs->bFrag.bytes;
+    uint64_t b = rs->bFrag.bytes + rs->bMemo.bytes;
     for (const T1kDevBuf &c : rs->chunks) if (c.p) b += c.bytes;
     *bytes = b;
     nChunks = std::min<size_t>(rs->chunks.size(), 1024);
diff --git a/t1k_amd/csrc/t1k_dev.h b/t1k_amd/csrc/t1k_dev.h
--- a/t1k_amd/csrc/t1k_dev.h
+++ b/t1k_amd/csrc/t1k_dev.h
@@ -822,6 +822,8 @@
   struct { bool on = false; t1k_route_totals kept{}; std::vector<t1k_route_rec> keptRecs, passRecs; bool passLong = false, passXlong = false; } route;
   uint64_t pairEpoch = 0;
   uint64_t pairBigCap = 0;
+  T1kDevBuf bPairTodo;
+  bool pairMemoPublish = false;
   unsigned long long *countersPinned = nullptr;
   double *emPinned = nullptr;
   size_t emPinnedN = 0;
diff --git a/t1k_amd/csrc/t1k_launch.h b/t1k_amd/csrc/t1k_launch.h
--- a/t1k_amd/csrc/t1k_launch.h
+++ b/t1k_amd/csrc/t1k_launch.h
@@ -123,6 +123,9 @@
   size_t cur = 0;
   uint64_t chunkEntries = 0;
   std::mutex m;
+  T1kDevBuf bMemo;
+  struct PairMemoEntry *memo = nullptr;
+  uint64_t memoSlots = 0;
   T1kDevBuf bWhitelist;
   const uint8_t *whitelist = nullptr;
   bool rawKept = false;
@@ -162,6 +165,8 @@
 
 int t1k_rowset_chunk(t1k_rowset *rs, t1k_ctx *ctx, size_t *chunk, t1k_row_entry **rows, uint64_t *cap, unsigned long long **cursor);
 int t1k_rowset_chunk_full(t1k_rowset *rs, t1k_ctx *ctx, size_t chunk);
+int t1k_pair_memo_on();
+uint64_t t1k_pair_memo_slots(uint64_t nFragments);
 int t1k_exclusive_sum64(t1k_ctx *ctx, const uint32_t *in, unsigned long long *out, uint32_t n);
 int t1k_exclusive_sum32(t1k_ctx *ctx, const uint32_t *in, uint32_t *out, uint64_t n);
 int t1k_exclusive_sum_u64(t1k_ctx *ctx, const unsigned long long *in, unsigned long long *out, uint64_t n);
diff --git a/t1k_amd/csrc/t1k_pair.hip b/t1k_amd/csrc/t1k_pair.hip
--- a/t1k_amd/csrc/t1k_pair.hip
+++ b/t1k_amd/csrc/t1k_pair.hip
@@ -3,6 +3,7 @@
 #include <cstring>
 #include "t1k_dev.h"
 #include "t1k_launch.h"
+#include "t1k_pair_memo.h"
 
 #ifdef T1K_PAIR_PROFILE
 #define PP(i) do { if (tid == 0) { const uint64_t tn_ = __builtin_amdgcn_s_memtime(); tp_[i] += tn_ - tl_; tl_ = tn_; } } while (0)
@@ -143,6 +144,7 @@
   int rawKept;
   unsigned long long *rsRowPtr; uint32_t *rsRowCount; unsigned long long *rsH1, *rsH2; uint8_t *rsAssigned;
   t1k_row_entry *rsRows; uint64_t rsCap; unsigned long long *rsCursor; uint64_t fragBase;
+  const uint32_t *todo;
 };
 
 struct OvlList {
@@ -262,7 +264,7 @@
 #ifdef T1K_PAIR_PROFILE
   uint64_t tp_[8] = {0, 0, 0, 0, 0, 0, 0, 0}, tl_ = __builtin_amdgcn_s_memtime();
 #endif
-  const uint32_t nItems = P.only ? (uint32_t)P.counters[23] : P.nFragments;
+  const uint32_t nItems = P.only ? (uint32_t)P.counters[23] : P.todo ? (uint32_t)P.counters[28] : P.nFragments;
   __shared__ uint32_t sItem;
   uint32_t hoNext = 0, hoLeft = 0;
   __shared__ unsigned long long sStatOvl, sStatRows;
@@ -277,7 +279,7 @@
     __syncthreads();
     const uint32_t it = sItem;
     if (it >= nItems) break;
-    const uint32_t f = P.only ? P.only[2 * it] : it;
+    const uint32_t f = P.only ? P.only[2 * it] : P.todo ? P.todo[it] : it;
     const uint64_t epoch = (uint64_t)(P.epochBase + f + 1) << 32;
     const bool paired = P.end2 != nullptr;
     const uint32_t e1 = P.end1[f];
@@ -810,6 +812,90 @@
 #endif
 }
 
+int t1k_pair_memo_on() {
+  static const int on = [] { const char *e = getenv("T1K_PAIR_MEMO"); return e && !strcmp(e, "0") ? 0 : 1; }();
+  return on;
+}
+uint64_t t1k_pair_memo_slots(uint64_t nFragments) {
+  static const long long forced = [] { const char *e = getenv("T1K_PAIR_MEMO_SLOTS"); return e ? std::max(1ll, atoll(e)) : 0ll; }();
+  if (!t1k_pair_memo_on()) return 0;
+  if (!forced) return pairMemoSlotsFor(nFragments);
+  uint64_t n = 1;
+  while (n < (uint64_t)forced) n <<= 1;
+  return n;
+}
+
+struct PairMemoArgs {
+  const unsigned long long *listPtr; const uint32_t *listCount;
+  const uint32_t *end1, *end2; const uint8_t *hasN;
+  uint32_t nFragments;
+  PairMemoEntry *tab; uint64_t nSlots;
+  uint32_t *todo;
+  unsigned long long *counters;
+  unsigned long long *rsRowPtr; uint32_t *rsRowCount; unsigned long long *rsH1, *rsH2; uint8_t *rsAssigned; uint64_t fragBase;
+  uint64_t nFrag;
+};
+
+__device__ __forceinline__ void pairMemoKeys(const PairMemoArgs &M, uint32_t f, unsigned long long &k1, unsigned long long &k2, uint32_t &recs) {
+  const uint32_t e1 = M.end1[f];
+  const uint32_t n1 = M.listCount[e1];
+  uint32_t n2 = 0;
+  unsigned long long a2 = 0;
+  if (M.end2) { const uint32_t e2 = M.end2[f]; n2 = M.listCount[e2]; a2 = M.listPtr[e2]; }
+  k1 = pairMemoKey1(M.listPtr[e1], n1, M.hasN[f] != 0);
+  k2 = pairMemoKey2(a2, n2);
+  recs = n1 + n2;
+}
+
+__global__ __launch_bounds__(256) void k_pair_memo_probe(PairMemoArgs M) {
+  __shared__ uint32_t sWave[4], sBase;
+  const int tid = threadIdx.x, lane = tid & 63, wave = tid >> 6;
+  const uint32_t f = blockIdx.x * 256u + tid;
+  const bool valid = f < M.nFragments;
+  unsigned long long v = 0;
+  uint32_t recs = 0;
+  if (valid && M.nSlots) {
+    unsigned long long k1, k2;
+    pairMemoKeys(M, f, k1, k2, recs);
+    if (recs) v = pairMemoProbe(M.tab, M.nSlots, k1, k2);
+  }
+  if (v > M.nFrag) v = 0;
+  if (v) {
+    const uint64_t g = v - 1, me = M.fragBase + f;
+    M.rsRowPtr[me] = M.rsRowPtr[g]; M.rsRowCount[me] = M.rsRowCount[g];
+    M.rsH1[me] = M.rsH1[g]; M.rsH2[me] = M.rsH2[g]; M.rsAssigned[me] = M.rsAssigned[g];
+  }
+  const bool miss = valid && !v;
+  const unsigned long long mm = __ballot(miss);
+  if (lane == 0) sWave[wave] = (uint32_t)__popcll(mm);
+  const unsigned long long hm = __ballot(v != 0);
+  unsigned long long hr = v ? recs : 0u;
+#pragma unroll
+  for (int o = 32; o > 0; o >>= 1) hr += __shfl_xor(hr, o, 64);
+  if (lane == 0 && hm) { atomicAdd(&M.counters[29], (unsigned long long)__popcll(hm)); atomicAdd(&M.counters[30], hr); }
+  __syncthreads();
+  if (tid == 0) {
+    const uint32_t tot = sWave[0] + sWave[1] + sWave[2] + sWave[3];
+    sBase = tot ? (uint32_t)atomicAdd(&M.counters[28], (unsigned long long)tot) : 0u;
+  }
+  __syncthreads();
+  if (miss) {
+    uint32_t at = sBase + (uint32_t)__popcll(mm & ((1ull << lane) - 1ull));
+    for (int w = 0; w < wave; ++w) at += sWave[w];
+    M.todo[at] = f;
+  }
+}
+
+__global__ __launch_bounds__(256) void k_pair_memo_publish(PairMemoArgs M) {
+  const uint32_t i = blockIdx.x * 256u + threadIdx.x;
+  if (i >= M.nFragments || i >= (uint32_t)M.counters[28]) return;
+  const uint32_t f = M.todo[i];
+  unsigned long long k1, k2;
+  uint32_t recs;
+  pairMemoKeys(M, f, k1, k2, recs);
+  if (recs) (void)pairMemoInsert(M.tab, M.nSlots, k1, k2, M.fragBase + f + 1);
+}
+
 constexpr int PAIR_WG = 256, PAIR_LJ_SLOTS = 4096;
 static uint32_t pairFragCap() {
   static const uint32_t cap = [] { const char *e = getenv("T1K_PAIR_FRAGCAP"); return e ? (uint32_t)std::max(8, atoi(e)) : 8192u; }();
@@ -845,6 +931,7 @@
   bool fresh = ctx->bPairScratch.bytes < (size_t)maxWg * perWg;
   if ((rc = t1k_ensure(ctx, ctx->bPairScratch, (size_t)maxWg * perWg))) return rc;
   if ((rc = t1k_ensure(ctx, ctx->bPairOverflow, (size_t)n * 8 + 16))) return rc;
+  if (rs && (rc = t1k_ensure(ctx, ctx->bPairTodo, (size_t)n * 4 + 16))) return rc;
   if (ctx->pairBigCap == 0) ctx->pairBigCap = envBigCap;
   if ((rc = t1k_ensure(ctx, ctx->bPairBig, (size_t)ctx->pairBigCap * (sizeof(Frag) + 4)))) return rc;
   if ((rc = t1k_ensure(ctx, ctx->bCounters, (size_t)T1K_COUNTER_WORDS * 8))) return rc;
@@ -876,11 +963,19 @@
   p.whitelist = dWhitelist;
   { static const int lf = getenv("T1K_PAIR_LIST") ? 1 : 0; p.listForm = lf; }
   p.direct = pairDirectOn();
+  PairMemoArgs m{};
+  if (rs) {
+    m.listPtr = p.listPtr; m.listCount = p.listCount; m.end1 = p.end1; m.end2 = p.end2; m.hasN = p.hasN; m.nFragments = n;
+    m.tab = rs->memo; m.nSlots = rs->memo ? rs->memoSlots : 0;
+    m.todo = (uint32_t *)ctx->bPairTodo.p; m.counters = p.counters;
+    m.rsRowPtr = rs->rowPtr; m.rsRowCount = rs->rowCount; m.rsH1 = rs->h1; m.rsH2 = rs->h2; m.rsAssigned = rs->assigned; m.fragBase = fragBase; m.nFrag = rs->nFrag;
+    p.todo = m.todo;
+  }
   if (getenv("T1K_DEBUG_TRACE")) fprintf(stderr, "[t1k trace] pair %u fragments%s\n", n, rs ? " into the rowset" : "");
   for (int attempt = 0;; ++attempt) {
     T1K_HIP(ctx, hipMemsetAsync((char *)ctx->bCounters.p + 2 * 8, 0, 8, ctx->stream));
     T1K_HIP(ctx, hipMemsetAsync((char *)ctx->bCounters.p + 9 * 8, 0, 8, ctx->stream));
-    T1K_HIP(ctx, hipMemsetAsync((char *)ctx->bCounters.p + 22 * 8, 0, 40, ctx->stream));
+    T1K_HIP(ctx, hipMemsetAsync((char *)ctx->bCounters.p + 22 * 8, 0, 72, ctx->stream));
 #ifdef T1K_PAIR_ROUTES
     T1K_HIP(ctx, hipMemsetAsync((char *)ctx->bCounters.p + 40 * 8, 0, 12 * 8, ctx->stream));
 #endif
@@ -893,6 +988,7 @@
     p.epochBase = (uint32_t)ctx->pairEpoch; ctx->pairEpoch += n;
     p.only = nullptr; p.overflowList = (uint32_t *)ctx->bPairOverflow.p;
     T1K_HIP(ctx, hipEventRecord(ctx->ev[5], ctx->stream));
+    if (rs) hipLaunchKernelGGL(k_pair_memo_probe, dim3((n + 255) / 256), dim3(256), 0, ctx->stream, m);
     launch((unsigned)nWg, p);
     {
       PairArgs q = p;
@@ -920,6 +1016,11 @@
     if (hc[2]) return t1k_fail(ctx, T1K_ERR_CAPACITY, "device arena overflow: row_cap / fragment scratch");
     if (!rs) ctx->nRows = hc[9];
     ctx->stats.rows = hc[9]; ctx->stats.pair_overlaps = hc[22];
+    ctx->stats.pair_memo_hits = rs ? hc[29] : 0; ctx->stats.pair_memo_records = rs ? hc[30] : 0;
+    if (rs && m.nSlots && ctx->pairMemoPublish) {
+      hipLaunchKernelGGL(k_pair_memo_publish, dim3((n + 255) / 256), dim3(256), 0, ctx->stream, m);
+      T1K_HIP(ctx, hipStreamSynchronize(ctx->stream));
+    }
 #ifdef T1K_PAIR_ROUTES
     {
       static unsigned long long sum[12];
@@ -950,6 +1051,12 @@
   if (fragBase + nFragments > rs->nFrag) return t1k_fail(ctx, T1K_ERR_ARG, "t1k_pair_into: fragments outside the rowset");
   if (rs->device != ctx->device) return t1k_fail(ctx, T1K_ERR_ARG, "t1k_pair_into: rowset lives on another device");
   return pairLaunch(ctx, rs, end1, end2, hasN, nFragments, fragBase, rs->whitelist);
+}
+
+int t1k_ctx_set_pair_memo(t1k_ctx *ctx, int publish) {
+  if (!ctx) return T1K_ERR_ARG;
+  ctx->pairMemoPublish = publish != 0;
+  return T1K_OK;
 }
 
 void t1k_pair_limits(uint32_t out[4]) {
diff --git a/t1k_amd/csrc/t1k_pair_memo.h b/t1k_amd/csrc/t1k_pair_memo.h
--- /dev/null
+++ b/t1k_amd/csrc/t1k_pair_memo.h
@@ -0,0 +1,91 @@
+#pragma once
+#include <stdint.h>
+#if defined(__HIPCC__)
+#define T1K_PM_FN __host__ __device__ __forceinline__
+#else
+#define T1K_PM_FN inline
+#endif
+
+#define PAIR_MEMO_PROBES 32u
+
+struct PairMemoEntry { unsigned long long k1, k2, val; };
+
+#if defined(__HIP_DEVICE_COMPILE__)
+#define PM_LOAD(p) __hip_atomic_load((p), __ATOMIC_RELAXED, __HIP_MEMORY_SCOPE_AGENT)
+#define PM_STORE(p, v) __hip_atomic_store((p), (v), __ATOMIC_RELAXED, __HIP_MEMORY_SCOPE_AGENT)
+#define PM_RELEASE() __builtin_amdgcn_fence(__ATOMIC_RELEASE, "agent")
+#define PM_ACQUIRE() __builtin_amdgcn_fence(__ATOMIC_ACQUIRE, "agent")
+#else
+#define PM_LOAD(p) __atomic_load_n((p), __ATOMIC_RELAXED)
+#define PM_STORE(p, v) __atomic_store_n((p), (v), __ATOMIC_RELAXED)
+#define PM_RELEASE() __atomic_thread_fence(__ATOMIC_RELEASE)
+#define PM_ACQUIRE() __atomic_thread_fence(__ATOMIC_ACQUIRE)
+#endif
+
+T1K_PM_FN unsigned long long pairMemoClaim(unsigned long long *p, unsigned long long key) {
+#if defined(__HIP_DEVICE_COMPILE__)
+  return atomicCAS(p, 0ull, key);
+#else
+  unsigned long long seen = 0ull;
+  (void)__atomic_compare_exchange_n(p, &seen, key, false, __ATOMIC_RELAXED, __ATOMIC_RELAXED);
+  return seen;
+#endif
+}
+
+T1K_PM_FN unsigned long long pairMemoKey1(unsigned long long list1, uint32_t n1, bool hasN) {
+  return (n1 ? list1 : 0ull) | (hasN ? 1ull : 0ull) | 0x8000000000000000ull;
+}
+T1K_PM_FN unsigned long long pairMemoKey2(unsigned long long list2, uint32_t n2) { return n2 ? list2 : 0ull; }
+
+T1K_PM_FN uint64_t pairMemoSlot(unsigned long long k1, unsigned long long k2, uint64_t mask) {
+  unsigned long long x = (k1 >> 4) * 0x9E3779B97F4A7C15ull ^ (k2 >> 4) * 0xC2B2AE3D27D4EB4Full ^ (k1 & 1ull);
+  x ^= x >> 29; x *= 0xD6E8FEB86659FD93ull; x ^= x >> 32;
+  return (uint64_t)x & mask;
+}
+
+T1K_PM_FN unsigned long long pairMemoProbe(PairMemoEntry *tab, uint64_t nSlots, unsigned long long k1, unsigned long long k2) {
+  if (!nSlots) return 0ull;
+  const uint64_t mask = nSlots - 1;
+  uint64_t s = pairMemoSlot(k1, k2, mask);
+  const uint32_t tries = nSlots < PAIR_MEMO_PROBES ? (uint32_t)nSlots : PAIR_MEMO_PROBES;
+  for (uint32_t t = 0; t < tries; ++t, s = (s + 1) & mask) {
+    const unsigned long long e1 = PM_LOAD(&tab[s].k1);
+    if (e1 == 0ull) return 0ull;
+    if (e1 != k1) continue;
+    const unsigned long long v = PM_LOAD(&tab[s].val);
+    if (v == 0ull) return 0ull;
+    PM_ACQUIRE();
+    if (PM_LOAD(&tab[s].k2) == k2) return v;
+  }
+  return 0ull;
+}
+
+T1K_PM_FN int pairMemoInsert(PairMemoEntry *tab, uint64_t nSlots, unsigned long long k1, unsigned long long k2, unsigned long long val) {
+  if (!nSlots) return -1;
+  const uint64_t mask = nSlots - 1;
+  uint64_t s = pairMemoSlot(k1, k2, mask);
+  const uint32_t tries = nSlots < PAIR_MEMO_PROBES ? (uint32_t)nSlots : PAIR_MEMO_PROBES;
+  for (uint32_t t = 0; t < tries; ++t, s = (s + 1) & mask) {
+    unsigned long long e1 = PM_LOAD(&tab[s].k1);
+    if (e1 == 0ull) e1 = pairMemoClaim(&tab[s].k1, k1);
+    if (e1 == 0ull) {
+      PM_STORE(&tab[s].k2, k2);
+      PM_RELEASE();
+      PM_STORE(&tab[s].val, val);
+      return 1;
+    }
+    if (e1 != k1) continue;
+    if (PM_LOAD(&tab[s].val) == 0ull) continue;
+    PM_ACQUIRE();
+    if (PM_LOAD(&tab[s].k2) == k2) return 0;
+  }
+  return -1;
+}
+
+T1K_PM_FN uint64_t pairMemoSlotsFor(uint64_t nFragments) {
+  if (!nFragments) return 0;
+  const uint64_t want = nFragments + nFragments / 4;
+  uint64_t n = 64;
+  while (n < want) n <<= 1;
+  return n;
+}
```
